# SauersML/genomic_pca

Measured on AMD Instinct MI355X. Metric: SNPs x samples / sec through rSVD at k=20; max|dPC| vs ref, higher is better.
Workload: dtype i8 (exact: int8 dosages x 4 signed 7-bit fixed-point digit planes of the skinny operand, i32 accumulate, f64 recombination; accuracy >= f32)

## Files before the change

genomic_pca_amd/_lib.py:

```python
from __future__ import annotations

import ctypes as C
import os
import subprocess

_PKG = os.path.dirname(os.path.abspath(__file__))
LIB_PATH = os.path.join(_PKG, "libgpca.so")
CSRC = os.path.join(_PKG, "csrc")

GPCA_OK = 0
GPCA_ERR_BAD_ARG = -1
GPCA_ERR_OOM = -2
GPCA_ERR_HIP = -3
GPCA_ERR_RCCL = -4
GPCA_ERR_MISSING_GENOTYPE = -5
GPCA_ERR_NOT_CONVERGED = -6
GPCA_ERR_STATE = -7
GPCA_ERR_NO_DEVICE = -8
GPCA_ERR_INVALID_GENOTYPE = -9
GPCA_UNIQUE_ID_BYTES = 128
PREC_DEFAULT = 0
PREC_I8_EXACT = 1
PREC_F32_MFMA = 2
STORE_AUTO = 0
STORE_2BIT = 1
STORE_INT8 = 2
GRM_STANDARDIZED = 0
GRM_CENTRED = 1
CFG_SIMPLE_KERNELS = 1
CFG_NO_COMPACT = 2
CFG_NO_NARROW = 4
CFG_NO_SPIN_SYNC = 8


class GpcaLibraryError(RuntimeError):
    pass


class GpcaError(RuntimeError):
    def __init__(self, status: int, message: str):
        super().__init__(f"[gpca status {status}] {message}")
        self.status = status
        self.message = message


class gpca_config(C.Structure):
    _fields_ = [("device", C.c_int32), ("precision", C.c_int32), ("storage", C.c_int32), ("digit_planes", C.c_int32),
                ("reserved", C.c_int32 * 4)]


class gpca_qc_config(C.Structure):
    _fields_ = [("min_snp_call_rate", C.c_double), ("min_snp_maf", C.c_double), ("max_snp_hwe_p_value", C.c_double)]


class gpca_kernel_timing(C.Structure):
    _fields_ = [("name", C.c_char * 32), ("launches", C.c_int64), ("total_ms", C.c_double), ("flops", C.c_double),
                ("bytes", C.c_double)]


ALLREDUCE_FN = C.CFUNCTYPE(C.c_int, C.c_void_p, C.POINTER(C.c_double), C.c_int64)
PANEL_FN = C.CFUNCTYPE(C.c_int, C.c_void_p, C.c_int64, C.c_int64, C.c_void_p, C.c_int64)
PANEL_HOST_I8 = 0
PANEL_HOST_BED = 1
PANEL_SYNTH = 2
PANEL_SYNTH16 = 3
PANEL_MAPPED_I8 = 4
PANEL_MAPPED_BED = 5
SOURCE_REGISTER = 1
SOURCE_BENCH_HOLD = 2


class gpca_panel_source(C.Structure):
    _fields_ = [("kind", C.c_int32), ("n_pop", C.c_int32), ("fill", PANEL_FN), ("user", C.c_void_p),
                ("thresh", C.c_void_p), ("seed", C.c_uint64), ("snp_offset", C.c_int64), ("host_ld", C.c_int64), ("flags", C.c_int64)]


class gpca_stream_info(C.Structure):
    _fields_ = [("panel_rows", C.c_int64), ("n_panels", C.c_int32), ("ring_slots", C.c_int32), ("n_cached", C.c_int32),
                ("staging_buffers", C.c_int32), ("zero_staging", C.c_int32), ("copy_threads", C.c_int32), ("fills", C.c_int64),
                ("fill_host_ms", C.c_double), ("fill_wait_ms", C.c_double), ("register_ms", C.c_double), ("reserved", C.c_int64 * 4)]


_H = C.c_void_p
PROTOTYPES = {
    "gpca_version": (C.c_int, []),
    "gpca_status_string": (C.c_char_p, [C.c_int]),
    "gpca_create": (C.c_int, [C.POINTER(gpca_config), C.POINTER(_H)]),
    "gpca_destroy": (C.c_int, [_H]),
    "gpca_last_error": (C.c_char_p, [_H]),
    "gpca_upload_genotypes_i8": (C.c_int, [_H, C.c_void_p, C.c_int64, C.c_int64, C.c_int64]),
    "gpca_upload_bed2bit": (C.c_int, [_H, C.c_void_p, C.c_int64, C.c_int64]),
    "gpca_synth_genotypes": (C.c_int, [_H, C.c_int64, C.c_int64, C.c_uint64, C.c_void_p, C.c_int32, C.c_int64]),
    "gpca_download_genotypes_i8": (C.c_int, [_H, C.c_void_p, C.c_int64]),
    "gpca_load_from_source": (C.c_int, [_H, C.POINTER(gpca_panel_source), C.c_int64, C.c_int64]),
    "gpca_stream_open": (C.c_int, [_H, C.POINTER(gpca_panel_source), C.c_int64, C.c_int64, C.c_int64, C.c_int32]),
    "gpca_stream_set_fused": (C.c_int, [_H, C.c_int32]),
    "gpca_stream_set_cache": (C.c_int, [_H, C.c_int64, C.POINTER(C.c_int32)]),
    "gpca_stream_get_info": (C.c_int, [_H, C.POINTER(gpca_stream_info)]),
    "gpca_get_device_memory": (C.c_int, [_H, C.POINTER(C.c_int64), C.POINTER(C.c_int64)]),
    "gpca_copy_rows": (C.c_int, [_H, _H, C.c_int64, C.c_int64]),
    "gpca_set_sample_mask": (C.c_int, [_H, C.c_void_p]),
    "gpca_set_condensed_basis": (C.c_int, [_H, C.c_void_p, C.c_void_p, C.c_int32, C.c_int64]),
    "gpca_rsvd_condensed": (C.c_int, [_H, C.c_int32, C.c_int32, C.c_int32, C.c_uint64]),
    "gpca_refine": (C.c_int, [_H, C.c_void_p, C.c_int32]),
    "gpca_dims": (C.c_int, [_H, C.POINTER(C.c_int64), C.POINTER(C.c_int64)]),
    "gpca_get_storage": (C.c_int, [_H, C.POINTER(C.c_int32), C.POINTER(C.c_int32)]),
    "gpca_snp_stats": (C.c_int, [_H, C.POINTER(gpca_qc_config), C.c_void_p, C.c_void_p, C.c_void_p]),
    "gpca_get_snp_qc_detail": (C.c_int, [_H, C.c_void_p, C.c_void_p]),
    "gpca_set_standardization": (C.c_int, [_H, C.c_void_p, C.c_void_p, C.c_void_p]),
    "gpca_get_standardization": (C.c_int, [_H, C.c_void_p, C.c_void_p, C.c_void_p]),
    "gpca_hwe_chi_squared_p_value": (C.c_double, [C.c_uint64, C.c_uint64, C.c_uint64]),
    "gpca_host_eigh_desc": (C.c_int, [C.c_void_p, C.c_int32, C.c_void_p, C.c_void_p]),
    "gpca_device_eigh_desc": (C.c_int, [_H, C.c_void_p, C.c_int32, C.c_void_p, C.c_void_p]),
    "gpca_device_orth": (C.c_int, [_H, C.c_void_p, C.c_int32, C.c_int32, C.c_void_p, C.c_void_p, C.POINTER(C.c_int32)]),
    "gpca_device_tail": (C.c_int, [_H, C.c_void_p, C.c_void_p, C.c_int32, C.c_int32, C.c_int32]),
    "gpca_standardize_block": (C.c_int, [_H, C.c_void_p, C.c_int64, C.c_void_p, C.c_int64, C.c_void_p]),
    "gpca_num_pca_snps": (C.c_int64, [_H]),
    "gpca_num_qc_samples": (C.c_int64, [_H]),
    "gpca_get_pca_snp_rows": (C.c_int, [_H, C.c_void_p]),
    "gpca_rsvd": (C.c_int, [_H, C.c_int32, C.c_int32, C.c_int32, C.c_uint64]),
    "gpca_get_scores": (C.c_int, [_H, C.c_void_p]),
    "gpca_get_scores_f64": (C.c_int, [_H, C.c_void_p]),
    "gpca_get_eigenvalues": (C.c_int, [_H, C.c_void_p]),
    "gpca_get_singular_values": (C.c_int, [_H, C.c_void_p]),
    "gpca_get_loadings": (C.c_int, [_H, C.c_void_p]),
    "gpca_transform": (C.c_int, [_H, C.c_void_p]),
    "gpca_project": (C.c_int, [_H, C.c_void_p, C.c_void_p, C.c_void_p, C.c_int32, C.c_void_p, C.c_void_p]),
    "gpca_grm": (C.c_int, [_H, C.c_int32, C.c_int64, C.c_int64, C.c_void_p, C.c_void_p]),
    "gpca_king": (C.c_int, [_H, C.c_int64, C.c_int64, C.c_void_p, C.c_void_p]),
    "gpca_ld_window": (C.c_int, [_H, C.c_int64, C.c_int64, C.c_void_p, C.c_int32, C.c_double, C.c_void_p, C.c_void_p, C.c_void_p]),
    "gpca_pcrelate_isaf": (C.c_int, [_H, C.c_void_p, C.c_int32, C.c_void_p, C.c_int64, C.c_int64, C.c_void_p, C.c_void_p]),
    "gpca_pcrelate": (C.c_int, [_H, C.c_void_p, C.c_int32, C.c_void_p, C.c_double, C.c_int64, C.c_int64, C.c_void_p, C.c_void_p]),
    "gpca_assoc_linear": (C.c_int, [_H, C.c_void_p, C.c_int32, C.c_void_p, C.c_int32, C.c_void_p, C.c_double, C.c_int64, C.c_int64, C.c_void_p,
                                    C.c_void_p, C.c_void_p]),
    "gpca_student_t_log10p": (C.c_double, [C.c_double, C.c_double]),
    "gpca_logistic_null": (C.c_int, [C.c_void_p, C.c_void_p, C.c_int32, C.c_void_p, C.c_int64, C.c_void_p, C.c_void_p, C.POINTER(C.c_int32)]),
    "gpca_assoc_logistic_score": (C.c_int, [_H, C.c_void_p, C.c_int32, C.c_void_p, C.c_int32, C.c_void_p, C.c_double, C.c_int64, C.c_int64,
                                            C.c_void_p, C.c_void_p, C.c_void_p]),
    "gpca_normal_log10p": (C.c_double, [C.c_double]),
    "gpca_assoc_logistic_spa": (C.c_int, [_H, C.c_void_p, C.c_int32, C.c_void_p, C.c_int32, C.c_void_p, C.c_double, C.c_double, C.c_int64,
                                          C.c_int64, C.c_void_p, C.c_void_p, C.c_void_p, C.c_void_p]),
    "gpca_spa_log10p": (C.c_int, [C.c_void_p, C.c_void_p, C.c_int64, C.c_double, C.POINTER(C.c_double), C.c_void_p, C.POINTER(C.c_int32)]),
    "gpca_comm_get_unique_id": (C.c_int, [C.c_void_p]),
    "gpca_comm_init": (C.c_int, [_H, C.c_int32, C.c_int32, C.c_void_p, C.c_int64]),
    "gpca_set_allreduce_hook": (C.c_int, [_H, ALLREDUCE_FN, C.c_void_p, C.c_int32, C.c_int32, C.c_int64]),
    "gpca_comm_count_ranks": (C.c_int, [_H, C.POINTER(C.c_int32)]),
    "gpca_get_timings": (C.c_int, [_H, C.POINTER(gpca_kernel_timing), C.c_int32, C.POINTER(C.c_int32)]),
    "gpca_reset_timings": (C.c_int, [_H]),
    "gpca_enable_timings": (C.c_int, [_H, C.c_int32]),
    "gpca_synchronize": (C.c_int, [_H]),
}


def build(force: bool = False) -> str:
    cmd = ["make", "-C", CSRC, "-s"] + (["-B"] if force else [])
    subprocess.check_call(cmd)
    return LIB_PATH


_lib = None


def load() -> C.CDLL:
    global _lib
    if _lib is not None:
        return _lib
    if not os.path.exists(LIB_PATH):
        raise GpcaLibraryError(
            f"{LIB_PATH} not found: build it with `python -c 'import __graft_entry__ as g; g.build()'` "
            "(hipcc --offload-arch=gfx950).  genomic_pca_amd has no CPU fallback.")
    try:
        lib = C.CDLL(LIB_PATH)
    except OSError as e:
        raise GpcaLibraryError(f"could not load {LIB_PATH}: {e}") from e
    for name, (res, args) in PROTOTYPES.items():
        try:
            fn = getattr(lib, name)
        except AttributeError as e:
            raise GpcaLibraryError(f"{LIB_PATH} does not export {name} (stale build?)") from e
        fn.restype = res
        fn.argtypes = args
    _lib = lib
    return lib
```

genomic_pca_amd/csrc/gemm_i8.hip:

```cpp
#include "gemm_i8_common.h"

namespace gpca {

template <int NSU>
struct GqnG { i32x4 g[4 * NSU]; float r, b; };
template <int NSU>
__device__ __forceinline__ void gqn_load(GqnG<NSU>& b, const int8_t* __restrict__ G, int64_t ldg, int64_t unit, int c, int h,
                                         const float* __restrict__ rv, const float* __restrict__ bv) {
    const __amdgpu_buffer_rsrc_t rg = make_rsrc8(G + unit * 32 * ldg);
    const uint32_t vo = (uint32_t)(c * ldg + 16 * h);
#pragma unroll
    for (int j = 0; j < 4 * NSU; ++j) b.g[j] = __builtin_amdgcn_raw_buffer_load_b128(rg, vo, 32u * j, 2);
    b.r = rv[unit * 32 + c]; b.b = bv[unit * 32 + c];
}
template <int NSU, int PF>
__global__ __launch_bounds__(256, 1) void k_gq_n(const int8_t* __restrict__ G, int64_t ldg, int64_t units,
                                                  const int8_t* __restrict__ Qd, const double* __restrict__ qscale,
                                                  const float* __restrict__ rv, const float* __restrict__ bv,
                                                  const float* __restrict__ sv, float* __restrict__ Tout,
                                                  float* __restrict__ cunit, double* __restrict__ apart, int scale_out, int64_t ldt) {
    const int lane = threadIdx.x & 63;
    const int wv = __builtin_amdgcn_readfirstlane(threadIdx.x >> 6);
    const int c = lane & 31, h = lane >> 5;
    const int64_t wave = (int64_t)blockIdx.x * 4 + wv, waves = (int64_t)gridDim.x * 4;
// ... 383 lines not shown
        else *dst = vv;
    }
    __builtin_amdgcn_fence(__ATOMIC_ACQ_REL, "wavefront");
    __builtin_amdgcn_sched_barrier(0);
}

struct GqdRound { int64_t unit0; int nv; int R; };

template <int NT, int R>
__device__ __forceinline__ void gqd_round(const int8_t* __restrict__ G, int64_t ldg, int64_t nstage,
                                          const int8_t* __restrict__ Qd, GqdSmem* sm, int wv, int lane, int c, int h,
                                          int64_t unit0, int nvalid, bool prologue, bool chain, GqdRound nx, uint32_t& rslot, int round_ix, uint32_t ph,
                                          int64_t rows_total, double qs, const float* __restrict__ rv,
                                          const float* __restrict__ bv, float sj, float* __restrict__ Tout, int scale_out, int64_t ldt,
                                          float* __restrict__ cunit, float& amax) {
    constexpr int S = kGqdSlots;
    static_assert(R >= 1 && R <= 4, "tiles per wave");
    auto phys = [&](uint32_t st_) -> uint32_t { const uint32_t p_ = st_ + ph; return p_ >= (uint32_t)nstage ? p_ - (uint32_t)nstage : p_; };
    const int64_t row0 = unit0 * 32;
    const i32x4 rg = gqd_rsrc(G + row0 * ldg);
    const i32x4 rgn = gqd_rsrc(G + nx.unit0 * 32 * ldg);
    const i32x4 rq = gqd_rsrc(Qd + wv * 1024);
    const uint32_t ld32 = (uint32_t)ldg;
    const uint32_t gvo_e = (uint32_t)(lane >> 3) * ld32 + 16u * (uint32_t)((lane & 7) ^ (lane >> 4));
    const uint32_t gvo_o = (uint32_t)(lane >> 3) * ld32 + 16u * (uint32_t)((lane & 7) ^ (lane >> 4) ^ 4);
    const uint32_t qvo = (uint32_t)(lane * 16);
    uint32_t toff[R];
#pragma unroll
    for (int t = 0; t < R; ++t) toff[t] = (uint32_t)(t < nvalid ? 32 * t : 0) * ld32;
    {
        const uint32_t lds_rb = (uint32_t)(uintptr_t)(__attribute__((address_space(3))) void*)&sm->rb[wv][0][0];
        i32x4 rr_ = gqd_rsrc(rv + row0), rb_ = gqd_rsrc(bv + row0);
        rr_.z = rb_.z = (int)((rows_total - row0) * 4);
        asm volatile("s_waitcnt lgkmcnt(0)" ::: "memory");
#pragma unroll
        for (int j = 0; j < (R + 1) / 2; ++j) {
            gqd_dma_dword(lds_rb + 256u * j, qvo >> 2, rr_, 256u * j);
            gqd_dma_dword(lds_rb + 512u + 256u * j, qvo >> 2, rb_, 256u * j);
        }
    }
    constexpr uint32_t QCH = kDigits * 1024;
    const uint32_t lds_q = (uint32_t)(uintptr_t)(__attribute__((address_space(3))) void*)&sm->q[0][0][0][0] + (uint32_t)wv * 1024u;
    const uint32_t lds_g = (uint32_t)(uintptr_t)(__attribute__((address_space(3))) void*)&sm->g[0][0][0] + (uint32_t)wv * (S * 4096u);
    const char* gl = reinterpret_cast<const char*>(&sm->g[wv][0][0]);
    uint32_t loff[4];
#pragma unroll
    for (int s4 = 0; s4 < 4; ++s4) loff[s4] = (uint32_t)(c * 128 + (((2 * s4 + h) ^ ((c >> 1) & 7)) * 16));

    i32x16 acc[R][kDigits];
#pragma unroll
    for (int t = 0; t < R; ++t)
#pragma unroll
        for (int d = 0; d < kDigits; ++d)
#pragma unroll
            for (int e = 0; e < 16; ++e) acc[t][d][e] = 0;

#define GQD_ISSUE_G(RSRC, SO, SLOT)                                                                       \
    {                                                                                                     \
        const uint32_t so_ = (SO);                                                                        \
        const uint32_t la_ = lds_g + (uint32_t)(SLOT) * 4096u;                                            \
        _Pragma("unroll") for (int i = 0; i < 4; ++i) gqd_dma<NT>(la_ + 1024u * i, (i & 1) ? gvo_o : gvo_e, RSRC, so_ + 8u * i * ld32); \
    }
#define GQD_ISSUE_Q(ST, QS)                                                                               \
    {                                                                                                     \
        _Pragma("unroll") for (int j = 0; j < 4; ++j)                                                     \
            gqd_dma(lds_q + (uint32_t)(((QS) * 4 + j) * kDigits) * 1024u, qvo, rq, (phys((uint32_t)(ST)) * 4u + j) * QCH); \
    }
    int64_t ist = 0;
    int it = 0;
    bool in_next = false;
    uint32_t pst = 0; int pt = 0;
#define GQD_ISSUE_NEXT(SLOT)                                                                              \
    {                                                                                                     \
        if (!in_next) {                                                                                   \
            GQD_ISSUE_G(rg, toff[it] + phys((uint32_t)ist) * 128u, SLOT)                                  \
            if (++it == R) { it = 0; if (++ist == nstage) { if (chain) in_next = true; else ist = 0; } }  \
        } else {                                                                                          \
            const uint32_t tn_ = (uint32_t)(pt < nx.nv ? 32 * pt : 0) * ld32;                             \
            GQD_ISSUE_G(rgn, tn_ + phys(pst) * 128u, SLOT)                                                \
            if (++pt == nx.R) { pt = 0; ++pst; }                                                          \
        }                                                                                                 \
    }
    if (prologue) {
        rslot = 0;
        GQD_ISSUE_NEXT(0) GQD_ISSUE_NEXT(1)
        GQD_ISSUE_Q(0, 0)
#pragma unroll
        for (int sl = S - 4; sl < S; ++sl) GQD_ISSUE_NEXT(sl)
    } else {
        ist = S / R; it = S % R;
    }
    i32x4 gcur, gnxt;

    for (int64_t st = 0; st < nstage; ++st) {
        if constexpr (R == 4) asm volatile("s_waitcnt vmcnt(16)\n\ts_barrier" ::: "memory");
        else if constexpr (R == 3) asm volatile("s_waitcnt vmcnt(12)\n\ts_barrier" ::: "memory");
        else if constexpr (R == 2) asm volatile("s_waitcnt vmcnt(8)\n\ts_barrier" ::: "memory");
        else asm volatile("s_waitcnt vmcnt(4)\n\ts_barrier" ::: "memory");
        GQD_STAGE_STAMP(round_ix, st)
        GQD_ISSUE_Q(st + 1 < nstage ? st + 1 : 0, (int)((st + 1) & 1))
        i32x4 q[4][kDigits];
#pragma unroll
        for (int s4 = 0; s4 < 4; ++s4)
#pragma unroll
            for (int d = 0; d < kDigits; ++d) q[s4][d] = sm->q[st & 1][s4][d][lane];
        if (st == 0) {
            gcur = *reinterpret_cast<const i32x4*>(gl + rslot * 4096u + loff[0]);
            gnxt = *reinterpret_cast<const i32x4*>(gl + rslot * 4096u + loff[1]);
        }
#pragma unroll
        for (int t = 0; t < R; ++t) {
            const char* ub = gl + rslot * 4096u;
            const uint32_t nslot = rslot == S - 1 ? 0u : rslot + 1u;
#pragma unroll
            for (int s4 = 0; s4 < 4; ++s4) {
                i32x4 gfar;
                if (s4 < 2) {
                    gfar = *reinterpret_cast<const i32x4*>(ub + loff[s4 + 2]);
                } else {
                    if (s4 == 2) {
                        if constexpr (R == 4) {
                            if (t == 0) gqd_wait_vm<24>(); else gqd_wait_vm<20>();
                        } else {
                            if (st < gqd_early_stages(R)) gqd_wait_young(gqd_q_young_early(R));
                            else gqd_wait_young(gqd_q_young(R, t));
                        }
                    }
                    gfar = *reinterpret_cast<const i32x4*>(gl + nslot * 4096u + loff[s4 - 2]);
                }
#pragma unroll
                for (int d = 0; d < kDigits; ++d)
                    acc[t][d] = __builtin_amdgcn_mfma_i32_32x32x32_i8(gcur, q[s4][d], acc[t][d], 0, 0, 0);
                if (s4 == 3) {
                    asm volatile("" :: "v"(gcur));
                    GQD_ISSUE_NEXT(rslot)
                }
                gcur = gnxt; gnxt = gfar;
            }
            rslot = nslot;
        }
    }
    if (!chain) asm volatile("s_waitcnt vmcnt(0)\n\ts_barrier" ::: "memory");
    GQD_STAMP(1 + 2 * round_ix)
#undef GQD_ISSUE_NEXT
#undef GQD_ISSUE_G
#undef GQD_ISSUE_Q
    float* tile = sm->tile[wv];
#pragma unroll
    for (int t = 0; t < R; ++t)
        if (t < nvalid) gq_tile_out<7, true>(acc[t], 0.f, 0.f, &sm->rb[wv][0][32 * t], &sm->rb[wv][1][32 * t], qs, sj, scale_out, tile, Tout, ldt, unit0 + t, cunit, amax, lane, nx.unit0 != unit0);
    GQD_STAMP(2 + 2 * round_ix)
}

template <int NT>
__global__ __launch_bounds__(256, 1) void k_gq_d(const int8_t* __restrict__ G, int64_t ldg, int64_t units, int64_t nstage,
                                                  const int8_t* __restrict__ Qd, const double* __restrict__ qscale,
                                                  const float* __restrict__ rv, const float* __restrict__ bv,
                                                  const float* __restrict__ sv, float* __restrict__ Tout,
                                                  float* __restrict__ cpart, double* __restrict__ apart, int scale_out, int64_t ldt,
                                                  int chain_ok, int phase_mul) {
    extern __shared__ __attribute__((aligned(16))) char gqd_smem[];
    GqdSmem* sm = reinterpret_cast<GqdSmem*>(gqd_smem);
    __builtin_assume(nstage >= 2 && (nstage & 1) == 0);
    const int lane = threadIdx.x & 63;
    const int wv = __builtin_amdgcn_readfirstlane(threadIdx.x >> 6);
    const int c = lane & 31, h = lane >> 5;
    const uint32_t ph = (uint32_t)(((int64_t)(blockIdx.x & 7) * (phase_mul & 0xffff) + (int64_t)(blockIdx.x >> 3) * (phase_mul >> 16)) % nstage);
    const int64_t u0 = (units * (int64_t)blockIdx.x) / gridDim.x;
    const int64_t u1 = (units * ((int64_t)blockIdx.x + 1)) / gridDim.x;
    float amax = 0.f;
    const float sj = sv[c];
    const double qs = qscale[c];
    asm volatile("" :: "v"(sj), "v"(qs));
    auto round_at = [&](int64_t u) -> GqdRound {
        const int64_t rem = u1 - u, take = rem < 16 ? rem : 16;
        const int64_t base = take >> 2, extra = take & 3;
        const int nv = (int)(base + (wv < extra ? 1 : 0));
        GqdRound r;
        r.nv = nv; r.R = nv ? nv : 1;
        r.unit0 = nv ? u + wv * base + (wv < extra ? wv : extra) : u;
        return r;
    };
    const bool chain_all = chain_ok && nstage > kGqdSlots;
    uint32_t rslot = 0;
    int round_ix = 0;
    GQD_STAMP(0)
    int64_t u = u0;
    while (u < u1) {
        const int64_t un = u + (u1 - u < 16 ? u1 - u : 16);
        const GqdRound cur = round_at(u);
        const bool chain = chain_all && un < u1;
        const bool prologue = !chain_all || u == u0;
        GqdRound nx = cur;
        if (chain) nx = round_at(un);
#define GPCA_GQD_ROUND(RR) gqd_round<NT, RR>(G, ldg, nstage, Qd, sm, wv, lane, c, h, cur.unit0, cur.nv, prologue, chain, nx, rslot, round_ix, ph, units * 32, qs, rv, bv, sj, Tout, scale_out, ldt, cpart, amax)
        if (cur.R == 4) GPCA_GQD_ROUND(4);
        else if (cur.R == 3) GPCA_GQD_ROUND(3);
        else if (cur.R == 2) GPCA_GQD_ROUND(2);
        else GPCA_GQD_ROUND(1);
#undef GPCA_GQD_ROUND
        u = un;
        ++round_ix;
    }
#if GPCA_STAMP
    if (threadIdx.x == 0 && blockIdx.x == 0) g_gqd_stamp_n = round_ix;
#endif
    float am_lo, am_hi; halves_pair(amax, am_lo, am_hi);
    const float am = fmaxf(am_lo, am_hi);
    if (h == 0) apart[((int64_t)blockIdx.x * 4 + wv) * 32 + c] = (double)am;
}

int launch_gq_d(hipStream_t st, const int8_t* G, int64_t ldg, const GqPlan& plan, int64_t Npad, const int8_t* Qd,
                const double* qscale, const float* r, const float* b, const float* s, float* Tout, float* cpart, double* apart,
                int scale_out, int64_t ldt, const KernelOpts& ko) {
    if (!dma_shape_ok(Npad, 256, plan.units * 32, 32) || ldg < Npad) return (int)hipErrorInvalidValue;
    const dim3 grid((unsigned)(plan.waves / 4)), blk(256);
    const int64_t nstage = Npad / 128;
    int phase = ko.gq_phase;
    if (phase < 0) phase = (nstage >= 16 && nstage <= 400) ? (int)((nstage / 8) << 16) : 0;
    hipLaunchKernelGGL((k_gq_d<1>), grid, blk, sizeof(GqdSmem), st, G, ldg, plan.units, nstage, Qd, qscale, r, b, s, Tout, cpart, apart, scale_out, ldt, ko.gq_chain, phase);
    return 0;
}

template <bool PACKED>
struct GttXG { unsigned g[16]; };

#ifndef GPCA_GTTX_AUX
#define GPCA_GTTX_AUX 2
#endif
template <bool PACKED>
__device__ __forceinline__ void gttx_load_g(GttXG<PACKED>& b, __amdgpu_buffer_rsrc_t rg, uint32_t gvo, uint32_t row_off, uint32_t ldr) {
#pragma unroll
    for (int i = 0; i < 16; ++i) b.g[i] = (unsigned)__builtin_amdgcn_raw_buffer_load_b32(rg, gvo, row_off + (uint32_t)i * ldr, PACKED ? 0 : GPCA_GTTX_AUX);
}
template <bool PACKED, int ABL = 0>
__device__ __forceinline__ void gttx_decode_step(const GttXG<PACKED>& bn, Gtt2Ops& on, unsigned (&x)[4], unsigned (&y)[4], int m, unsigned bsh) {
    const int w = m >> 2, ph = m & 3;
    if (ABL & 1) { on.bt[ph][w] = (int)bn.g[4 * w + ph]; return; }
    if (PACKED) {
        if (ph == 0) x[w] = ((bn.g[4 * w] >> bsh) & 0xffu) | (((bn.g[4 * w + 1] >> bsh) & 0xffu) << 8) |
                            (((bn.g[4 * w + 2] >> bsh) & 0xffu) << 16) | ((bn.g[4 * w + 3] >> bsh) << 24);
        if (ph == 1) { on.bt[0][w] = (int)(x[w] & 0x03030303u); on.bt[1][w] = (int)((x[w] >> 2) & 0x03030303u); }
        if (ph == 2) on.bt[2][w] = (int)((x[w] >> 4) & 0x03030303u);
        if (ph == 3) on.bt[3][w] = (int)((x[w] >> 6) & 0x03030303u);
    } else {
        const int r0 = (int)bn.g[4 * w], r1 = (int)bn.g[4 * w + 1], r2 = (int)bn.g[4 * w + 2], r3 = (int)bn.g[4 * w + 3];
        if (ph == 0) { x[w] = (unsigned)permb(r1, r0, 0x05010400u); y[w] = (unsigned)permb(r1, r0, 0x07030602u); }
        if (ph == 1) { x[w] = x[w]; }
        if (ph == 2) {
            const int y0 = permb(r3, r2, 0x05010400u);
            on.bt[0][w] = permb(y0, (int)x[w], 0x05040100u); on.bt[1][w] = permb(y0, (int)x[w], 0x07060302u);
        }
        if (ph == 3) {
            const int y1 = permb(r3, r2, 0x07030602u);
            on.bt[2][w] = permb(y1, (int)y[w], 0x05040100u); on.bt[3][w] = permb(y1, (int)y[w], 0x07060302u);
        }
    }
}
template <bool PACKED>
__device__ __forceinline__ void gttx_decode(const GttXG<PACKED>& b, Gtt2Ops& o, unsigned bsh) {
    unsigned x[4], y[4];
#pragma unroll
    for (int m = 0; m < 16; ++m) gttx_decode_step<PACKED>(b, o, x, y, m, bsh);
}
struct GttXT { i32x4 t[kDigits]; };
template <bool PACKED, int ND = kDigits, int ABL = 0, bool ZERO = false>
__device__ __forceinline__ void gttx_phase(const GttXT& tc, const Gtt2Ops& oc, i32x16 (&acc)[4][kDigits],
                                           const GttXG<PACKED>& gn, Gtt2Ops& on, GttXT& tn, const i32x4* lds_next, unsigned bsh) {
    unsigned x[4], y[4];
    const i32x16 zero16 = {0, 0, 0, 0, 0, 0, 0, 0, 0, 0, 0, 0, 0, 0, 0, 0};
#pragma unroll
    for (int d = 0; d < kDigits; ++d)
#pragma unroll
        for (int t = 0; t < 4; ++t) {
            if (ABL & 8) { if (d < ND) { if (ZERO) acc[t][d] = zero16; acc[t][d][0] ^= tc.t[d][t] ^ oc.bt[t][d]; } }
            else if (d < ND) acc[t][d] = __builtin_amdgcn_mfma_i32_32x32x32_i8(tc.t[d], oc.bt[t], ZERO ? zero16 : acc[t][d], 0, 0, 0);
            const int m = d * 4 + t;
            if (m < ND) tn.t[m] = lds_next[m * 64];
            gttx_decode_step<PACKED, ABL>(gn, on, x, y, m, bsh);
            __builtin_amdgcn_sched_barrier(0);
        }
}

template <int NT>
__device__ __forceinline__ void gtd_issue_g(const uint8_t* gp, int64_t ldr, int64_t blk, int64_t kblocks, uint32_t lds_slot, uint32_t gvo) {
    const int64_t ub = blk < kblocks ? blk : 0;
    const i32x4 rg = gqd_rsrc(gp + ub * 32 * ldr);
    asm volatile("s_waitcnt lgkmcnt(0)" ::: "memory");
#pragma unroll
    for (int i = 0; i < 4; ++i) gqd_dma<NT>(lds_slot + 1024u * i, gvo, rg, 8u * i * (uint32_t)ldr);
}
__device__ __forceinline__ void gtd_issue_t(const int8_t* tp, int64_t st, int64_t nstage, uint32_t lds_t_slot, uint32_t tvo) {
    constexpr uint32_t TKB = kDigits * 1024;
    const int64_t us = st < nstage ? st : 0;
    const i32x4 rt = gqd_rsrc(tp + us * 4 * TKB);
#pragma unroll
    for (int j = 0; j < 4; ++j) gqd_dma<0>(lds_t_slot + (uint32_t)(j * kDigits) * 1024u, tvo, rt, j * TKB);
}
__device__ __forceinline__ void gtd_read_g(GttXG<false>& b, const char* unit) {
#pragma unroll
    for (int i = 0; i < 16; ++i) b.g[i] = *reinterpret_cast<const unsigned*>(unit + i * 128);
}

#if GPCA_STAMP
__device__ unsigned long long g_gtd_stamp[2 * 4096];
#endif
__device__ __forceinline__ int64_t k2_virtual_wg(int xcd_remap) {
    int64_t vb = blockIdx.x;
    if (xcd_remap) {
        const int64_t q = gridDim.x / 8, r = gridDim.x % 8, x = blockIdx.x % 8;
        vb = x * q + (x < r ? x : r) + blockIdx.x / 8;
    }
    return vb;
}

struct GtdTask { const uint8_t* gp; const int8_t* tp; int64_t kblocks; int64_t n0; int64_t slice; bool live; };

template <int BITS>
__device__ __forceinline__ void gtt_tiles_out(const i32x16 (&acc)[4][kDigits], double* __restrict__ Ypart, int64_t slice, int64_t Npad, int64_t n0,
                                              char* stage = nullptr, int piece_stride = 1024) {
    __builtin_amdgcn_sched_barrier(0);
    unsigned all = ~0u;
    asm volatile("" : "+s"(all));
    const int lane = (int)__builtin_amdgcn_mbcnt_hi(all, __builtin_amdgcn_mbcnt_lo(all, 0u));
    const int c = lane & 31, h = lane >> 5;
#ifndef GPCA_YPART_DIRECT
    if (stage) {
        double* ybase = Ypart + (slice * Npad + n0) * 32;
#pragma unroll
        for (int t = 0; t < 4; ++t) {
#pragma unroll
            for (int half = 0; half < 2; ++half) {
#pragma unroll
                for (int q = 0; q < 2; ++q)
#pragma unroll
                    for (int ip = 0; ip < 2; ++ip) {
                        const int e = 8 * half + 4 * q + 2 * ip;
                        double2 o;
                        o.x = combine_digits<BITS>(acc[t], e); o.y = combine_digits<BITS>(acc[t], e + 1);
                        const int ch = 4 * q + 2 * h + ip;
                        *reinterpret_cast<double2*>(stage + (c >> 3) * piece_stride + (c & 7) * 128 + ((ch ^ (c & 7)) << 4)) = o;
                    }
                __builtin_amdgcn_fence(__ATOMIC_ACQ_REL, "wavefront");
#pragma unroll
                for (int i = 0; i < 4; ++i) {
                    const int line = (lane >> 3) + 8 * i, ch = lane & 7;
                    const double2 v = *reinterpret_cast<const double2*>(stage + i * piece_stride + (lane >> 3) * 128 + ((ch ^ (line & 7)) << 4));
                    typedef double d2v __attribute__((ext_vector_type(2)));
                    const d2v vv = {v.x, v.y};
                    __builtin_nontemporal_store(vv, reinterpret_cast<d2v*>(ybase + (4 * line + t) * 32 + 16 * half + 2 * ch));
                }
                __builtin_amdgcn_fence(__ATOMIC_ACQ_REL, "wavefront");
                __builtin_amdgcn_sched_barrier(0);
            }
        }
        return;
    }
#endif
    double* yp = Ypart + (slice * Npad + n0 + 4 * c) * 32 + 4 * h;
#pragma unroll
    for (int t = 0; t < 4; ++t) {
#pragma unroll
        for (int e = 0; e < 16; e += 2) {
            const int j = acc_row(0, e, 0);
            double2 o;
            o.x = combine_digits<BITS>(acc[t], e); o.y = combine_digits<BITS>(acc[t], e + 1);
            *reinterpret_cast<double2*>(yp + t * 32 + j) = o;
            if (e == 6) __builtin_amdgcn_sched_barrier(0);
        }
        __builtin_amdgcn_sched_barrier(0);
    }
}

struct K2Walk {
    int64_t wch, g, wch_step, g_step, ngroups;
    int ntask;
    __device__ __forceinline__ void init(int64_t vwg, int64_t T, int64_t ngroups_, int tasks_per_wg, int strided) {
        ngroups = ngroups_;
        const int64_t t_first = strided ? vwg : vwg * tasks_per_wg, t_step = strided ? (int64_t)gridDim.x : 1;
        ntask = 0;
        if (t_first < T) { const int64_t left = (T - 1 - t_first) / t_step + 1; ntask = (int)(left < tasks_per_wg ? left : tasks_per_wg); }
        wch = t_first / ngroups; g = t_first - wch * ngroups;
        wch_step = t_step / ngroups; g_step = t_step - wch_step * ngroups;
    }
    __device__ __forceinline__ void advance() { wch += wch_step; g += g_step; if (g >= ngroups) { g -= ngroups; ++wch; } }
};

template <int NT, int ABL = 0>
__global__ __launch_bounds__(256, 1) void k_gtt_d(const uint8_t* __restrict__ Gb, int64_t ldr, int64_t Npad,
                                                   const int8_t* __restrict__ Td, double* __restrict__ Ypart,
                                                   int64_t S, int64_t C, int64_t ngroups, int W, int tasks_per_wg, int strided, int xcd_remap) {
    extern __shared__ __attribute__((aligned(16))) char gqd_smem[];
    GqdSmem* sm = reinterpret_cast<GqdSmem*>(gqd_smem);
    const int lane = threadIdx.x & 63;
    const int wv = __builtin_amdgcn_readfirstlane(threadIdx.x >> 6);
    const int c = lane & 31, h = lane >> 5;
#if GPCA_STAMP
    if (threadIdx.x == 0 && blockIdx.x < 4096) g_gtd_stamp[2 * blockIdx.x] = __builtin_amdgcn_s_memrealtime();
#endif
    constexpr uint32_t TKB = kDigits * 1024;
    K2Walk cw;
    cw.init(k2_virtual_wg(xcd_remap), (int64_t)W * ngroups, ngroups, tasks_per_wg, strided);
    const int ntask = cw.ntask;
    if (ntask == 0) return;
    auto task_of = [&](const K2Walk& w) -> GtdTask {
        const int64_t s0 = w.wch * C, s1 = (s0 + C < S) ? s0 + C : S;
        GtdTask k;
        k.n0 = (w.g * 4 + wv) * 128;
        k.live = k.n0 < Npad;
        if (!k.live) k.n0 = 0;
        k.gp = Gb + (s0 * 128) * ldr + k.n0;
        k.tp = Td + (s0 * 4) * TKB + wv * 1024;
        k.kblocks = (s1 - s0) * 4;
        k.slice = w.wch;
        return k;
    };

    const uint32_t gvo = (uint32_t)(lane >> 3) * (uint32_t)ldr + 16u * (uint32_t)(lane & 7);
    const uint32_t tvo = (uint32_t)(lane * 16);
    const uint32_t lds_t = (uint32_t)(uintptr_t)(__attribute__((address_space(3))) void*)&sm->q[0][0][0][0] + (uint32_t)wv * 1024u;
    const uint32_t lds_g = (uint32_t)(uintptr_t)(__attribute__((address_space(3))) void*)&sm->g[0][0][0] + (uint32_t)wv * (kGqdSlots * 4096u);
    const char* gl = reinterpret_cast<const char*>(&sm->g[wv][0][0]) + (16 * h) * 128 + 4 * c;
    i32x4 (*tds)[4][kDigits][64] = sm->q;

    K2Walk gw = cw, tw = cw;
    int gi = 0; GtdTask gk = task_of(gw); int64_t gblk = 0;
    int ti = 0; GtdTask tk = gk; int64_t tst = 0;
    auto issue_g = [&](uint32_t slot) {
        const i32x4 rg = gqd_rsrc(gk.gp + gblk * 32 * ldr);
        asm volatile("s_waitcnt lgkmcnt(0)" ::: "memory");
#pragma unroll
        for (int i = 0; i < 4; ++i) gqd_dma<NT>(lds_g + slot * 4096u + 1024u * i, gvo, rg, 8u * i * (uint32_t)ldr);
        if (++gblk == gk.kblocks) { gblk = 0; if (gi + 1 < ntask) { ++gi; gw.advance(); gk = task_of(gw); } }
    };
    auto issue_t = [&](uint32_t tslot) {
        const i32x4 rt = gqd_rsrc(tk.tp + tst * 4 * TKB);
#pragma unroll
        for (int j = 0; j < 4; ++j) gqd_dma<0>(lds_t + tslot * 4u * TKB + (uint32_t)(j * kDigits) * 1024u, tvo, rt, j * TKB);
        if (++tst == (tk.kblocks >> 2)) { tst = 0; if (ti + 1 < ntask) { ++ti; tw.advance(); tk = task_of(tw); } }
    };

    i32x16 acc[4][kDigits];
    GttXG<false> GA, GB;
    Gtt2Ops OA, OB;
    GttXT TA, TB;
    issue_g(0); issue_g(1);
    issue_t(0);
    issue_g(2); issue_g(3); issue_g(4); issue_g(5);
    issue_t(1);
    asm volatile("s_waitcnt vmcnt(20)\n\ts_barrier" ::: "memory");
    gtd_read_g(GA, gl);
    gtd_read_g(GB, gl + 4096);
#pragma unroll
    for (int d = 0; d < kDigits; ++d) TA.t[d] = tds[0][0][d][lane];
    gttx_decode<false>(GA, OA, 0u);
    asm volatile("" :: "v"(GB.g[15]));
    issue_g(0);
    uint32_t s1 = 1;
    uint32_t slot = 0;

#define GTD_PHASE(TC, OC, GN, ON, TN, GR, WV, TSLOT, TBLK, ZERO)                                           \
    {                                                                                                    \
        const uint32_t s2_ = s1 == kGqdSlots - 1 ? 0u : s1 + 1u;                                         \
        gqd_wait_vm<WV>();                                                                               \
        gtd_read_g(GR, gl + s2_ * 4096u);                                                                \
        __builtin_amdgcn_sched_barrier(0);                                                               \
        gttx_phase<false, kDigits, ABL, ZERO>(TC, OC, acc, GN, ON, TN, &tds[(TSLOT)][(TBLK)][0][lane], 0u); \
        __builtin_amdgcn_sched_barrier(0);                                                               \
        if (!(ABL & 4)) issue_g(s1);                                                                     \
        s1 = s2_;                                                                                        \
    }
#define GTD_STAGE(ZERO)                                                                                  \
    {                                                                                                    \
        GTD_PHASE(TA, OA, GB, OB, TB, GA, 20, slot, 1, ZERO)                                             \
        GTD_PHASE(TB, OB, GA, OA, TA, GB, 20, slot, 2, false)                                            \
        GTD_PHASE(TA, OA, GB, OB, TB, GA, 20, slot, 3, false)                                            \
        asm volatile("s_waitcnt vmcnt(16)\n\ts_barrier" ::: "memory");    \
        if (!(ABL & 2)) issue_t(slot);                                                                   \
        GTD_PHASE(TB, OB, GA, OA, TA, GB, 24, slot ^ 1u, 0, false)                                       \
        slot ^= 1u;                                                                                      \
    }
    for (int i = 0; i < ntask; ++i) {
        if (i) cw.advance();
        const GtdTask k = task_of(cw);
        const int64_t nstage = k.kblocks >> 2;
        GTD_STAGE(true)
        for (int64_t st = 1; st < nstage; ++st) GTD_STAGE(false)
        if (k.live && !((ABL & 16) && acc[0][0][0] != 0x7fffffff)) gtt_tiles_out<7>(acc, Ypart, k.slice, Npad, k.n0, reinterpret_cast<char*>(&sm->tile[wv][0]));
    }
#undef GTD_STAGE
#undef GTD_PHASE
    asm volatile("s_waitcnt vmcnt(0)" ::: "memory");
#if GPCA_STAMP
    if (threadIdx.x == 0 && blockIdx.x < 4096) g_gtd_stamp[2 * blockIdx.x + 1] = __builtin_amdgcn_s_memrealtime();
#endif
}

struct GtpStage { i32x4 t[4][kDigits][64]; char g[4][4096]; };
struct GtpSmem { GtpStage stg[4]; };

template <int ND>
__device__ __forceinline__ void gtp_segment(const uint8_t* __restrict__ G2, int64_t ld2, int64_t Npad, const int8_t* __restrict__ Td,
                                            double* __restrict__ Ypart, GtpSmem* sm, int wv, int lane, int c, int h,
                                            int64_t g, int64_t s0, int64_t nstage, int64_t slice) {
    const int64_t n0 = (g * 4 + wv) * 128;
    const int64_t m_begin = s0 * 128;

    i32x16 acc[4][kDigits];
#pragma unroll
    for (int t = 0; t < 4; ++t)
#pragma unroll
        for (int d = 0; d < kDigits; ++d)
#pragma unroll
            for (int e = 0; e < 16; ++e) acc[t][d][e] = 0;

    constexpr uint32_t TKB = kDigits * 1024;
    const uint8_t* gp = G2 + m_begin * ld2 + g * 128;
    const int8_t* tp = Td + (m_begin >> 5) * TKB + wv * 1024;
    const uint32_t gvo = (uint32_t)(8 * wv + (lane >> 3)) * (uint32_t)ld2 + 16u * (uint32_t)(lane & 7);
    const uint32_t tvo = (uint32_t)(lane * 16);
    const uint32_t lds0 = (uint32_t)(uintptr_t)(__attribute__((address_space(3))) void*)&sm->stg[0];
    const unsigned bsh = 8u * (unsigned)(c & 3);
    const uint32_t rdo = (uint32_t)((16 * h) * 128 + 32 * wv + (c & ~3));

    auto issue_stage = [&](int64_t st, uint32_t slot) {
        const int64_t us = st < nstage ? st : 0;
        const i32x4 rg = gqd_rsrc(gp + us * 128 * ld2);
        const i32x4 rt = gqd_rsrc(tp + us * 4 * TKB);
        const uint32_t base = lds0 + slot * (uint32_t)sizeof(GtpStage);
#pragma unroll
        for (int bb = 0; bb < 4; ++bb)
            gqd_dma<0>(base + 4u * TKB + (uint32_t)bb * 4096u + (uint32_t)wv * 1024u, gvo, rg, (uint32_t)(32 * bb) * (uint32_t)ld2);
#pragma unroll
        for (int j = 0; j < 4; ++j)
            gqd_dma<0>(base + (uint32_t)(j * kDigits) * 1024u + (uint32_t)wv * 1024u, tvo, rt, j * TKB);
    };
    auto read_g = [&](GttXG<true>& b, uint32_t slot, int bb) {
        const char* unit = &sm->stg[slot].g[bb][0] + rdo;
#pragma unroll
        for (int i = 0; i < 16; ++i) b.g[i] = *reinterpret_cast<const unsigned*>(unit + i * 128);
    };

    GttXG<true> GA, GB;
    Gtt2Ops OA, OB;
    GttXT TA, TB;
    issue_stage(0, 0); issue_stage(1, 1); issue_stage(2, 2);
    asm volatile("s_waitcnt vmcnt(8)\n\ts_barrier" ::: "memory");
    issue_stage(3, 3);
    read_g(GA, 0, 0);
    read_g(GB, 0, 1);
#pragma unroll
    for (int d = 0; d < ND; ++d) TA.t[d] = sm->stg[0].t[0][d][lane];
    gttx_decode<true>(GA, OA, bsh);

#define GTP_PHASE(TC, OC, GN, ON, TN, GR, TSLOT, TBLK, RS, RB)                                             \
    {                                                                                                    \
        read_g(GR, (RS), (RB));                                                                          \
        __builtin_amdgcn_sched_barrier(0);                                                               \
        gttx_phase<true, ND>(TC, OC, acc, GN, ON, TN, &sm->stg[(TSLOT)].t[(TBLK)][0][lane], bsh);            \
        __builtin_amdgcn_sched_barrier(0);                                                               \
    }
    for (int64_t st = 0; st < nstage; ++st) {
        const uint32_t q0 = (uint32_t)(st & 3), qn = (uint32_t)((st + 1) & 3);
        if (st > 0) {
            asm volatile("s_waitcnt vmcnt(8) lgkmcnt(0)\n\ts_barrier" ::: "memory");
            issue_stage(st + 3, (uint32_t)((st + 3) & 3));
        }
        GTP_PHASE(TA, OA, GB, OB, TB, GA, q0, 1, q0, 2)
        GTP_PHASE(TB, OB, GA, OA, TA, GB, q0, 2, q0, 3)
        GTP_PHASE(TA, OA, GB, OB, TB, GA, q0, 3, qn, 0)
        GTP_PHASE(TB, OB, GA, OA, TA, GB, qn, 0, qn, 1)
    }
#undef GTP_PHASE
    asm volatile("s_waitcnt vmcnt(0)\n\ts_barrier" ::: "memory");
    gtt_tiles_out<ND == 3 ? 8 : 7>(acc, Ypart, slice, Npad, n0, &sm->stg[3].g[0][1024 * wv], (int)sizeof(sm->stg[3].g[0]));
}

template <int ND>
__global__ __launch_bounds__(256, 1) void k_gtt_p(const uint8_t* __restrict__ G2, int64_t ld2, int64_t Npad,
                                                   const int8_t* __restrict__ Td, double* __restrict__ Ypart,
                                                   int64_t S, int64_t C, int64_t ngroups, int W, int tasks_per_wg, int strided, int xcd_remap) {
    extern __shared__ __attribute__((aligned(16))) char gqd_smem[];
    GtpSmem* sm = reinterpret_cast<GtpSmem*>(gqd_smem);
    const int lane = threadIdx.x & 63;
    const int wv = __builtin_amdgcn_readfirstlane(threadIdx.x >> 6);
    const int c = lane & 31, h = lane >> 5;
    K2Walk cw;
    cw.init(k2_virtual_wg(xcd_remap), (int64_t)W * ngroups, ngroups, tasks_per_wg, strided);
    for (int i = 0; i < cw.ntask; ++i) {
        if (i) cw.advance();
        const int64_t s0 = cw.wch * C, s1 = (s0 + C < S) ? s0 + C : S;
        gtp_segment<ND>(G2, ld2, Npad, Td, Ypart, sm, wv, lane, c, h, cw.g, s0, s1 - s0, cw.wch);
    }
}

int launch_gtt_p(hipStream_t st, const uint8_t* G2, int64_t ld2, int64_t Mpad, int64_t Npad, const int8_t* Td, double* Ypart,
                 const Gtt8Plan& plan, int nd, const KernelOpts& ko) {
    if (plan.tasks_per_wg < 1 || plan.S * 128 != Mpad || !dma_shape_ok(Npad, kSamplePad2bit, Mpad, kGQRowsPerWave) || ld2 * 4 < Npad) return (int)hipErrorInvalidValue;
    const int remap = ko.gtt_xcd;
    if (nd == 3) hipLaunchKernelGGL(k_gtt_p<3>, dim3((unsigned)plan.grid), dim3(256), sizeof(GtpSmem), st, G2, ld2, Npad, Td, Ypart, plan.S, plan.C, plan.ngroups, plan.W, plan.tasks_per_wg, plan.strided, remap);
    else hipLaunchKernelGGL(k_gtt_p<kDigits>, dim3((unsigned)plan.grid), dim3(256), sizeof(GtpSmem), st, G2, ld2, Npad, Td, Ypart, plan.S, plan.C, plan.ngroups, plan.W, plan.tasks_per_wg, plan.strided, remap);
    return 0;
}

int launch_gtt_d(hipStream_t st, const int8_t* G, int64_t ldg, int64_t Mpad, int64_t Npad, const int8_t* Td, double* Ypart,
                 const Gtt8Plan& plan, const KernelOpts& ko) {
    if (plan.tasks_per_wg < 1 || plan.S * 128 != Mpad || !dma_shape_ok(Npad, 256, Mpad, kGQRowsPerWave) || ldg < Npad) return (int)hipErrorInvalidValue;
    const dim3 grid((unsigned)plan.grid), blk(256);
    const int remap = ko.gtt_xcd;
    hipLaunchKernelGGL((k_gtt_d<1>), grid, blk, sizeof(GqdSmem), st, (const uint8_t*)G, ldg, Npad, Td, Ypart, plan.S, plan.C, plan.ngroups, plan.W, plan.tasks_per_wg, plan.strided, remap);
    return 0;
}

int init_device_kernels_i8() {
    int e = 0;
#define GPCA_OPT_IN(KERNEL, BYTES) \
    if (e == 0) e = (int)hipFuncSetAttribute(reinterpret_cast<const void*>(KERNEL), hipFuncAttributeMaxDynamicSharedMemorySize, (int)(BYTES));
    GPCA_OPT_IN((k_gq_d<1>), sizeof(GqdSmem))
    GPCA_OPT_IN((k_gtt_p<kDigits>), sizeof(GtpSmem)) GPCA_OPT_IN((k_gtt_p<3>), sizeof(GtpSmem))
    GPCA_OPT_IN((k_gtt_d<1>), sizeof(GqdSmem))
#undef GPCA_OPT_IN
    return e;
}

}
```

genomic_pca_amd/csrc/gpca_api.cpp:

```cpp
#include "gpca_internal.h"

using namespace gpca;

RcclApi g_rccl;
thread_local std::string g_last_global_err;

static thread_local uint64_t g_tls_err_gen = 0;
static thread_local std::string g_tls_err;
static std::atomic<uint64_t> g_next_gen{1};
int fail(gpca_handle* h, int code, const std::string& msg) {
    if (h) { h->err = msg; g_tls_err_gen = h->gen; g_tls_err = msg; } else g_last_global_err = msg;
    return code;
}

void fold_timings(gpca_handle* h) {
    for (auto& r : h->recs) {
        float ms = 0.f;
        if (hipEventSynchronize(r.b) == hipSuccess && hipEventElapsedTime(&ms, r.a, r.b) == hipSuccess) {
            size_t i = 0;
            for (; i < h->agg.size(); ++i) if (r.name == h->agg[i].name) break;
            if (i == h->agg.size()) { gpca_kernel_timing t{}; snprintf(t.name, sizeof t.name, "%s", r.name.c_str()); h->agg.push_back(t); }
            h->agg[i].launches++; h->agg[i].total_ms += ms; h->agg[i].flops += r.flops; h->agg[i].bytes += r.bytes;
        }
        h->ev_pool.push_back(r.a); h->ev_pool.push_back(r.b);
    }
    h->recs.clear();
}

extern "C" int gpca_version(void) { return GPCA_VERSION; }

extern "C" const char* gpca_status_string(int s) {
    switch (s) {
        case GPCA_OK: return "ok";
        case GPCA_ERR_BAD_ARG: return "bad argument";
        case GPCA_ERR_OOM: return "out of device memory";
        case GPCA_ERR_HIP: return "HIP runtime error";
        case GPCA_ERR_RCCL: return "RCCL error";
        case GPCA_ERR_MISSING_GENOTYPE: return "missing genotype in a PCA SNP";
        case GPCA_ERR_NOT_CONVERGED: return "sketch lost rank";
        case GPCA_ERR_STATE: return "call out of order";
        case GPCA_ERR_NO_DEVICE: return "no HIP device";
        case GPCA_ERR_INVALID_GENOTYPE: return "genotype outside {0,1,2} in a PCA SNP";
        default: return "unknown status";
    }
}

extern "C" const char* gpca_last_error(gpca_handle* h) {
    if (!h) return g_last_global_err.c_str();
    if (g_tls_err_gen == h->gen) return g_tls_err.c_str();
    return h->err.c_str();
}

extern "C" int gpca_create(const gpca_config* cfg, gpca_handle** out) {
    if (!out) return fail(nullptr, GPCA_ERR_BAD_ARG, "gpca_create: out is NULL");
    *out = nullptr;
    int ndev = 0;
    if (hipGetDeviceCount(&ndev) != hipSuccess || ndev <= 0)
        return fail(nullptr, GPCA_ERR_NO_DEVICE, "gpca_create: no HIP device visible (this engine has no CPU fallback)");
    gpca_handle* h = new gpca_handle();
    h->gen = g_next_gen.fetch_add(1, std::memory_order_relaxed);
    int dev = cfg ? cfg->device : -1;
    if (dev < 0) { if (hipGetDevice(&dev) != hipSuccess) dev = 0; }
    if (dev >= ndev) { delete h; return fail(nullptr, GPCA_ERR_BAD_ARG, "gpca_create: device ordinal out of range"); }
    h->device = dev;
    h->precision = (!cfg || cfg->precision == GPCA_PREC_DEFAULT) ? GPCA_PREC_I8_EXACT : cfg->precision;
    h->storage_cfg = cfg ? cfg->storage : GPCA_STORE_AUTO;
    if (h->storage_cfg != GPCA_STORE_AUTO && h->storage_cfg != GPCA_STORE_INT8 && h->storage_cfg != GPCA_STORE_2BIT) { delete h; return fail(nullptr, GPCA_ERR_BAD_ARG, "gpca_create: unknown storage mode"); }
    if (h->precision != GPCA_PREC_F32_MFMA && h->precision != GPCA_PREC_I8_EXACT) { delete h; return fail(nullptr, GPCA_ERR_BAD_ARG, "gpca_create: unknown precision mode"); }
    h->storage = h->storage_cfg == GPCA_STORE_2BIT ? GPCA_STORE_2BIT : GPCA_STORE_INT8;
    {
        const int dp = cfg ? cfg->digit_planes : 0;
        if (dp != 0 && dp != 3 && dp != 4) { delete h; return fail(nullptr, GPCA_ERR_BAD_ARG, "gpca_create: digit_planes must be 0, 3 or 4"); }
        if (dp == 3 && !(h->precision == GPCA_PREC_I8_EXACT && h->storage_cfg == GPCA_STORE_2BIT)) { delete h; return fail(nullptr, GPCA_ERR_BAD_ARG, "gpca_create: digit_planes = 3 is implemented for GPCA_PREC_I8_EXACT with GPCA_STORE_2BIT"); }
        h->nd_cfg = dp;
        h->nd = dp == 3 ? 3 : ((dp == 0 && h->precision == GPCA_PREC_I8_EXACT && h->storage == GPCA_STORE_2BIT) ? 3 : 4);
    }
    {
        const int32_t flags = cfg ? cfg->reserved[0] : 0, gqw = cfg ? cfg->reserved[1] : 0, gtw = cfg ? cfg->reserved[2] : 0;
        if ((flags & ~GPCA_CFG_ALL) != 0 || gqw < 0 || gtw < 0 || (cfg && cfg->reserved[3] != 0)) { delete h; return fail(nullptr, GPCA_ERR_BAD_ARG, "gpca_create: unknown bits in gpca_config.reserved"); }
        h->simple_kernels = (flags & GPCA_CFG_SIMPLE_KERNELS) != 0;
        h->compact_ok = (flags & GPCA_CFG_NO_COMPACT) == 0;
        h->narrow_ok = (flags & GPCA_CFG_NO_NARROW) == 0;
        h->spin_sync = (flags & GPCA_CFG_NO_SPIN_SYNC) == 0;
        if (gqw) h->gq_waves_target = std::max(4, (int)gqw);
        if (gtw) h->gtt_waves_target = std::max(4, (int)gtw);
    }
    if (hipSetDevice(dev) != hipSuccess || hipStreamCreateWithFlags(&h->st, hipStreamNonBlocking) != hipSuccess) {
        delete h; return fail(nullptr, GPCA_ERR_HIP, "gpca_create: hipSetDevice/hipStreamCreate failed");
    }
    hipDeviceProp_t prop;
    if (hipGetDeviceProperties(&prop, dev) == hipSuccess) {
        if (strncmp(prop.gcnArchName, "gfx950", 6) != 0) {
            std::string m = std::string("gpca_create: device is ") + prop.gcnArchName + ", this library only carries gfx950 code";
            (void)hipStreamDestroy(h->st); delete h; return fail(nullptr, GPCA_ERR_NO_DEVICE, m);
        }
    }
    int e = init_device_kernels_i8();
    if (e == 0) e = init_device_kernels_common();
    if (e == 0) e = init_device_kernels_eig();
    if (e != 0) {
        std::string m = std::string("gpca_create: cannot reserve the LDS the DMA kernels need (hipFuncSetAttribute: ") + hipGetErrorString((hipError_t)e) + ")";
        (void)hipStreamDestroy(h->st); delete h; return fail(nullptr, GPCA_ERR_HIP, m);
    }
    *out = h;
    return GPCA_OK;
}

void drop_child(gpca_handle* h) {
    h->child_valid = false; h->rsvd_on_child = false;
    if (!h->child) return;
    gpca_handle* c = h->child;
    h->child = nullptr;
    c->d_row_ids = nullptr;
    if (h->timing_on || !c->agg.empty() || !c->recs.empty()) {
        (void)hipStreamSynchronize(h->st);
        fold_timings(c);
        for (const gpca_kernel_timing& t : c->agg) {
            size_t i = 0;
            for (; i < h->agg.size(); ++i) if (strcmp(h->agg[i].name, t.name) == 0) break;
            if (i == h->agg.size()) h->agg.push_back(t);
            else { h->agg[i].launches += t.launches; h->agg[i].total_ms += t.total_ms; h->agg[i].flops += t.flops; h->agg[i].bytes += t.bytes; }
        }
    }
    (void)gpca_destroy(c);
}

extern "C" int gpca_destroy(gpca_handle* h) {
    if (!h) return GPCA_OK;
    { LOCK(h);
      (void)hipSetDevice(h->device);
      (void)hipStreamSynchronize(h->st);
      drop_child(h);
      stream_close(h);
      for (auto& r : h->recs) { (void)hipEventDestroy(r.a); (void)hipEventDestroy(r.b); }
      for (auto e : h->ev_pool) (void)hipEventDestroy(e);
      if (h->ev_status) (void)hipEventDestroy(h->ev_status);
      if (h->comm && g_rccl.CommDestroy) g_rccl.CommDestroy(h->comm);
      free_stats(h); free_ws(h); dfree(h->dG); dfree(h->dG2);
      for (auto* ln : h->lanes_free) {
          (void)hipStreamDestroy(ln->st); (void)hipEventDestroy(ln->dep); dfree(ln->d_rows); dfree(ln->d_cols); dfree(ln->d_out); dfree(ln->d_err); delete ln;
      }
      h->lanes_free.clear(); h->lanes_total = 0;
      dfree(h->d_status); if (h->h_status) { (void)hipHostFree(h->h_status); h->h_status = nullptr; }
      if (!h->is_child) (void)hipStreamDestroy(h->st);
    }
    { std::lock_guard<std::mutex> lk(h->pull_mu); }
    delete h;
    return GPCA_OK;
}

extern "C" int gpca_synchronize(gpca_handle* h) {
    if (!h) return GPCA_ERR_BAD_ARG;
    LOCK(h);
    if (h->sm.st_fill) HIPCHK(hipStreamSynchronize(h->sm.st_fill));
    HIPCHK(hipStreamSynchronize(h->st));
    return GPCA_OK;
}

int alloc_stats(gpca_handle* h) {
    const size_t M = (size_t)h->Mpad;
    if (h->d_mu && h->cap_stats_pad >= h->Mpad) return GPCA_OK;
    if (h->d_mu) free_stats(h);
    h->cap_stats_pad = h->Mpad;
    HIPCHK(hipMalloc((void**)&h->d_mu, M * 4)); HIPCHK(hipMalloc((void**)&h->d_sigma, M * 4));
    HIPCHK(hipMalloc((void**)&h->d_r, M * 4)); HIPCHK(hipMalloc((void**)&h->d_b, M * 4));
    HIPCHK(hipMalloc((void**)&h->d_keep, M)); HIPCHK(hipMalloc((void**)&h->d_reason, M));
    HIPCHK(hipMalloc((void**)&h->d_counts, M * 16)); HIPCHK(hipMalloc((void**)&h->d_flags, 16));
    HIPCHK(hipMemsetAsync(h->d_counts, 0, M * 16, h->st)); HIPCHK(hipMemsetAsync(h->d_r, 0, M * 4, h->st)); HIPCHK(hipMemsetAsync(h->d_b, 0, M * 4, h->st));
    HIPCHK(hipMemsetAsync(h->d_mu, 0, M * 4, h->st)); HIPCHK(hipMemsetAsync(h->d_sigma, 0, M * 4, h->st)); HIPCHK(hipMemsetAsync(h->d_keep, 0, M, h->st));
    return GPCA_OK;
}

int refresh_pca_rows(gpca_handle* h) {
    std::vector<uint8_t> keep((size_t)h->M);
    HIPCHK(hipMemcpy(keep.data(), h->d_keep, (size_t)h->M, hipMemcpyDeviceToHost));
    h->pca_rows.clear();
    for (int64_t i = 0; i < h->M; ++i) if (keep[(size_t)i]) h->pca_rows.push_back(i);
    h->n_pca = (int64_t)h->pca_rows.size();
    dfree(h->d_pca_rows);
    if (h->n_pca) {
        HIPCHK(hipMalloc((void**)&h->d_pca_rows, (size_t)h->n_pca * 8));
        HIPCHK(hipMemcpy(h->d_pca_rows, h->pca_rows.data(), (size_t)h->n_pca * 8, hipMemcpyHostToDevice));
    }
    return GPCA_OK;
}

extern "C" int gpca_snp_stats(gpca_handle* h, const gpca_qc_config* qc, float* mu, float* sigma, uint8_t* keep) {
    if (!h) return GPCA_ERR_BAD_ARG;
    LOCK(h);
    if (!have_genotypes(h)) return fail(h, GPCA_ERR_STATE, "gpca_snp_stats: no genotypes resident and no panel stream open");
    HIPCHK(hipSetDevice(h->device));
    CHK(alloc_stats(h));
    QcParams q{0.0, 0.0, 1.0};
    if (qc) { q.min_call_rate = qc->min_snp_call_rate; q.min_maf = qc->min_snp_maf; q.max_hwe_p = qc->max_snp_hwe_p_value; }
    HIPCHK(hipMemsetAsync(h->d_flags, 0, 16, h->st));
    {
        ScopedTimer t(h, "snp_stats", 0.0, (double)h->M * (double)h->N);
        CHK(for_each_panel(h, [&](const PanelView& pv) -> int {
            const int64_t o = pv.row0;
            if (h->storage == GPCA_STORE_2BIT)
                launch_snp_stats_2bit(h->st, pv.g2, pv.rows, h->N, h->ld2, q, h->d_mu + o, h->d_sigma + o, h->d_r + o, h->d_b + o, h->d_keep + o,
                                      h->d_reason + o, h->d_counts + 4 * o, h->d_flags);
            else
                launch_snp_stats(h->st, pv.g8, pv.rows, h->N, h->ld8, q, h->d_mu + o, h->d_sigma + o, h->d_r + o, h->d_b + o, h->d_keep + o,
                                 h->d_reason + o, h->d_counts + 4 * o, h->d_flags);
            HIPCHK(hipGetLastError());
            return GPCA_OK;
        }));
    }
    HIPCHK(hipMemcpyAsync(&h->flags, h->d_flags, 4, hipMemcpyDeviceToHost, h->st));
    HIPCHK(hipStreamSynchronize(h->st));
    if (h->sm.on && h->sm.fl.d_flags) CHK(finish_pack_flags(h, h->sm.fl.d_flags, h->sm.st_fill));
    h->flags |= h->pack_flags;
    CHK(refresh_pca_rows(h));
    h->have_stats = true; h->have_rsvd = false; h->rmax_valid = false; drop_child(h);
    if (mu) HIPCHK(hipMemcpy(mu, h->d_mu, (size_t)h->M * 4, hipMemcpyDeviceToHost));
    if (sigma) HIPCHK(hipMemcpy(sigma, h->d_sigma, (size_t)h->M * 4, hipMemcpyDeviceToHost));
    if (keep) HIPCHK(hipMemcpy(keep, h->d_keep, (size_t)h->M, hipMemcpyDeviceToHost));
    return GPCA_OK;
}

extern "C" int gpca_get_snp_qc_detail(gpca_handle* h, uint32_t* counts, uint8_t* reason) {
    if (!h) return GPCA_ERR_BAD_ARG;
    LOCK(h);
    if (!h->have_stats) return fail(h, GPCA_ERR_STATE, "gpca_get_snp_qc_detail: run gpca_snp_stats first");
    if (counts) HIPCHK(hipMemcpy(counts, h->d_counts, (size_t)h->M * 16, hipMemcpyDeviceToHost));
    if (reason) HIPCHK(hipMemcpy(reason, h->d_reason, (size_t)h->M, hipMemcpyDeviceToHost));
    return GPCA_OK;
}

extern "C" int gpca_get_standardization(gpca_handle* h, float* mu, float* sigma, uint8_t* keep) {
    if (!h) return GPCA_ERR_BAD_ARG;
    LOCK(h);
    if (!h->have_stats) return fail(h, GPCA_ERR_STATE, "gpca_get_standardization: run gpca_snp_stats or gpca_set_standardization first");
    HIPCHK(hipStreamSynchronize(h->st));
    if (mu) HIPCHK(hipMemcpy(mu, h->d_mu, (size_t)h->M * 4, hipMemcpyDeviceToHost));
// ... 327 lines not shown
```

genomic_pca_amd/csrc/gpca_internal.h:

```cpp
#pragma once
#include "../../include/gpca.h"
#include "kernels.h"

#include <dlfcn.h>
#include <hip/hip_runtime.h>

#include <algorithm>
#include <atomic>
#include <chrono>
#include <condition_variable>
#include <deque>
#include <thread>
#include <cmath>
#include <cstdio>
#include <cstdlib>
#include <cstring>
#include <map>
#include <mutex>
#include <string>
#include <vector>

using namespace gpca;

typedef struct ncclComm* ncclComm_t;
typedef struct { char internal[128]; } ncclUniqueId_t;
typedef int (*pfn_ncclGetUniqueId)(ncclUniqueId_t*);
typedef int (*pfn_ncclCommInitRank)(ncclComm_t*, int, ncclUniqueId_t, int);
typedef int (*pfn_ncclAllReduce)(const void*, void*, size_t, int, int, ncclComm_t, hipStream_t);
typedef int (*pfn_ncclCommDestroy)(ncclComm_t);
typedef const char* (*pfn_ncclGetErrorString)(int);
struct RcclApi {
    void* lib = nullptr;
    pfn_ncclGetUniqueId GetUniqueId = nullptr;
    pfn_ncclCommInitRank CommInitRank = nullptr;
    pfn_ncclAllReduce AllReduce = nullptr;
    pfn_ncclCommDestroy CommDestroy = nullptr;
    pfn_ncclGetErrorString GetErrorString = nullptr;
    bool load() {
        if (lib) return true;
        const char* names[] = {"librccl.so.1", "librccl.so", "/opt/rocm/lib/librccl.so.1"};
        for (const char* n : names) { lib = dlopen(n, RTLD_NOW | RTLD_LOCAL); if (lib) break; }
        if (!lib) return false;
        GetUniqueId = (pfn_ncclGetUniqueId)dlsym(lib, "ncclGetUniqueId");
        CommInitRank = (pfn_ncclCommInitRank)dlsym(lib, "ncclCommInitRank");
        AllReduce = (pfn_ncclAllReduce)dlsym(lib, "ncclAllReduce");
        CommDestroy = (pfn_ncclCommDestroy)dlsym(lib, "ncclCommDestroy");
        GetErrorString = (pfn_ncclGetErrorString)dlsym(lib, "ncclGetErrorString");
        return GetUniqueId && CommInitRank && AllReduce && CommDestroy;
    }
};
extern RcclApi g_rccl;
enum { kNcclFloat64 = 8, kNcclSum = 0 };

struct TimingRec { std::string name; hipEvent_t a, b; double flops, bytes; };

struct PanelView { const int8_t* g8; const uint8_t* g2; int64_t row0, rows, rows_pad; int index; };

struct Filler {
    gpca_panel_source src{};
    int64_t chunk_rows = 0;
    int64_t stage_ld = 0;
    uint32_t* d_thresh = nullptr;
    int8_t* d_scratch8 = nullptr;
    uint8_t* d_raw = nullptr;
    unsigned* d_flags = nullptr;
    bool open = false;
    bool host = false, mapped = false, registered = false;
    const uint8_t* map_base = nullptr; int64_t map_ld = 0; size_t reg_bytes = 0;
    int device = 0, copy_threads = 1;
    int n_stage = 0;
    std::vector<void*> h_stage;
    std::vector<hipEvent_t> ev_stage;
    enum { kFree = 0, kReady = 1, kInFlight = 2 };
    std::vector<int> st_state, st_rc;
    std::vector<int64_t> st_row0;
    std::deque<std::pair<int64_t, int64_t>> jobs;
    uint64_t posted = 0, produced = 0, consumed = 0;
    bool busy = false, quit = false;
    std::mutex m; std::condition_variable cv; std::thread worker;
    int64_t fills = 0; double fill_host_ms = 0.0, fill_wait_ms = 0.0, register_ms = 0.0;
    std::map<void*, int64_t> held;
};

struct StreamState {
    bool on = false;
    Filler fl;
    int64_t panel_rows = 0;
    int n_panels = 0, ring = 0;
    std::vector<void*> slot;
    std::vector<hipEvent_t> ev_filled, ev_free;
    std::vector<char> free_pending;
    hipStream_t st_fill = nullptr;
    int64_t seq = 0;
    int fused = 1;
    std::vector<void*> cache;
    std::vector<hipEvent_t> ev_cache;
    std::vector<char> cache_filled;
};

struct gpca_handle {
    std::recursive_mutex mu;
    KernelOpts ko;
    StreamState sm;
    int device = 0;
    int precision = GPCA_PREC_I8_EXACT;
    int storage = GPCA_STORE_INT8;
    int storage_cfg = GPCA_STORE_AUTO;
    int nd_cfg = 0;
    int auto_pin = 0;
    hipStream_t st = nullptr;
    std::string err;

    int64_t M = 0, N = 0, ldg = 0, Mpad = 0;
    int64_t ld8 = 0;
    int64_t cap_rows_pad = 0;
    int64_t cap_stats_pad = 0;
    int8_t* dG = nullptr;
    uint8_t* dG2 = nullptr;
    int64_t ld2 = 0;
    uint32_t pack_flags = 0;

    bool have_stats = false;
    float *d_mu = nullptr, *d_sigma = nullptr, *d_r = nullptr, *d_b = nullptr;
    uint8_t *d_keep = nullptr, *d_reason = nullptr;
    uint32_t *d_counts = nullptr, *d_flags = nullptr;
    int64_t n_pca = 0;
    std::vector<int64_t> pca_rows;
    int64_t* d_pca_rows = nullptr;
    uint32_t flags = 0;

    int k = 0, l = 0, L = 0;
    bool have_rsvd = false;
    float *dQ = nullptr, *dT = nullptr, *dTb = nullptr, *dYpart = nullptr, *d_cpart = nullptr, *d_s32 = nullptr;
    double* h_pin = nullptr;
    int spin_sync = 1;
    int* d_cholflag = nullptr;
    double *d_scratch64 = nullptr, *dY = nullptr, *d_c = nullptr, *d_part64 = nullptr, *dW = nullptr, *dZ = nullptr, *d_s64 = nullptr;
    double* d_tr64 = nullptr; size_t cap_tr64 = 0;
    double* d_scores64 = nullptr; float* d_scores32 = nullptr; float* d_load32 = nullptr; int* d_sign = nullptr;
    double* d_eigres = nullptr;
    double* d_cand_val = nullptr; int64_t* d_cand_idx = nullptr;
    size_t cap_Q = 0, cap_T = 0, cap_Tb = 0, cap_Ypart = 0, cap_cpart = 0, cap_Y = 0, cap_part64 = 0, cap_scores = 0, cap_load = 0;
    std::vector<double> eig, sv;
    GttPlan plan{};
    GqPlan gqplan{};
    Gtt8Plan plan8{};
    int8_t *dQd = nullptr, *dTd = nullptr;
    bool c_fold_pending = false;
    double* d_apart = nullptr; size_t cap_apart = 0; bool apart_valid = false; int64_t apart_parts = 0;
    const double* apart_src[4] = {nullptr, nullptr, nullptr, nullptr};
    float* d_rmax = nullptr; bool rmax_valid = false;
    double* d_amax_run = nullptr;
    double* d_yint = nullptr; size_t cap_yint = 0;
    uint8_t* d_smask = nullptr;
    int64_t n_smask = 0;
    float* d_cw = nullptr; int32_t* d_cfeat0 = nullptr; int c_cmax = 0; int64_t c_R = 0; int c_B = 0;
    int64_t *d_cblk_row0 = nullptr, *d_cblk_row1 = nullptr; int32_t *d_cblk_feat0 = nullptr, *d_cblk_c = nullptr;
    double* dP = nullptr; size_t cap_P = 0;
    float* d_lqr = nullptr; size_t cap_lqr = 0;
    float *d_ones = nullptr, *d_zeros = nullptr; size_t cap_ones = 0, cap_zeros = 0;
    bool loadings_valid = true;
    double* d_status = nullptr;
    double* h_status = nullptr;
    hipEvent_t ev_status = nullptr;
    std::string status_own;
    struct PullLane {
        hipStream_t st = nullptr;
        hipEvent_t dep = nullptr;
        int64_t *d_rows = nullptr, *d_cols = nullptr; float* d_out = nullptr; unsigned long long* d_err = nullptr;
        size_t cap_rows = 0, cap_cols = 0, cap_out = 0;
    };
    std::mutex pull_mu;
    std::condition_variable pull_cv;
    std::vector<PullLane*> lanes_free;
    int lanes_total = 0;
    std::atomic<int> pulls_in_flight{0};
    double *dYpart64 = nullptr, *d_qscale = nullptr, *d_qinv = nullptr, *d_tscale = nullptr, *d_tinv = nullptr;
    size_t cap_Qd = 0, cap_Td = 0, cap_Ypart64 = 0;
    int nd = 4;
    uint64_t gen = 0;
    int simple_kernels = 0;
    int narrow_ok = 1;
    int gq_waves_target = 1024, gtt_waves_target = 2048;

    gpca_handle* child = nullptr;
    bool child_valid = false, rsvd_on_child = false;
    bool is_child = false;
    const int64_t* d_row_ids = nullptr;
    int compact_ok = 1;

    int world = 1, rank = 0;
    int64_t snp_offset = 0;
    ncclComm_t comm = nullptr;
    gpca_allreduce_fn hook = nullptr;
    void* hook_user = nullptr;
    std::vector<double> hook_buf;

    bool timing_on = false;
    int timing_every = 1;
    int64_t timing_calls = 0;
    bool timing_skip = false;
    int open_timers = 0;
    std::vector<TimingRec> recs;
    std::vector<hipEvent_t> ev_pool;
    std::vector<gpca_kernel_timing> agg;
};
constexpr size_t kMaxTimingRecs = 32768;
#define LOCK(h) std::lock_guard<std::recursive_mutex> lock_guard_(h->mu); (void)hipSetDevice(h->device); drain_pulls(h)
#define LOCK_SHARED(h) std::lock_guard<std::recursive_mutex> lock_guard_(h->mu); (void)hipSetDevice(h->device)
constexpr int kMaxPullLanes = 16;
inline void drain_pulls(gpca_handle* h) {
    if (h->pulls_in_flight.load(std::memory_order_acquire) == 0) return;
    std::unique_lock<std::mutex> lk(h->pull_mu);
    h->pull_cv.wait(lk, [&] { return h->pulls_in_flight.load(std::memory_order_acquire) == 0; });
}

extern thread_local std::string g_last_global_err;
int fail(gpca_handle* h, int code, const std::string& msg);
#define HIPCHK(call)                                                                                   \
    do {                                                                                               \
        hipError_t e_ = (call);                                                                        \
        if (e_ != hipSuccess) {                                                                        \
            char buf_[512];                                                                            \
            snprintf(buf_, sizeof buf_, "%s failed: %s (%s:%d)", #call, hipGetErrorString(e_), __FILE__, __LINE__); \
            return fail(h, e_ == hipErrorOutOfMemory ? GPCA_ERR_OOM : GPCA_ERR_HIP, buf_);             \
        }                                                                                              \
    } while (0)
#define CHK(x) do { int rc_ = (x); if (rc_ != GPCA_OK) return rc_; } while (0)

template <typename T>
inline int ensure(gpca_handle* h, T*& p, size_t& cap, size_t need_elems) {
    if (cap >= need_elems && p) return GPCA_OK;
    if (p) { HIPCHK(hipFree(p)); p = nullptr; cap = 0; }
    HIPCHK(hipMalloc((void**)&p, need_elems * sizeof(T)));
    cap = need_elems;
    return GPCA_OK;
}
template <typename T>
inline void dfree(T*& p) { if (p) { (void)hipFree(p); p = nullptr; } }
template <typename T>
inline hipError_t dalloc(T*& p, size_t elems) { return hipMalloc((void**)&p, std::max<size_t>(elems, 1) * sizeof(T)); }
inline int preflight_device_memory(gpca_handle* h, const char* name, const char* what, double need_bytes) {
    size_t fr = 0, tot = 0;
    HIPCHK(hipMemGetInfo(&fr, &tot));
    if (need_bytes > (double)fr) {
        char buf[256];
        snprintf(buf, sizeof buf, "%s: %s %.3g GB of device memory, %.3g GB are free: ask for fewer rows", name, what, need_bytes * 1e-9, (double)fr * 1e-9);
        return fail(h, GPCA_ERR_OOM, buf);
    }
    return GPCA_OK;
}

inline hipError_t malloc_genotypes(const gpca_handle*, void** p, size_t bytes) { return hipMalloc(p, bytes); }

inline int64_t round_up(int64_t x, int64_t m) { return (x + m - 1) / m * m; }
static_assert(gpca::kMaxSketchCols == 128, "kernels.h");
constexpr int kMaxSketch = gpca::kMaxSketchCols;

void fold_timings(gpca_handle* h);
struct ScopedTimer {
    gpca_handle* h; bool on; size_t idx = 0; hipStream_t st;
    ScopedTimer(gpca_handle* h_, const char* name, double flops, double bytes, hipStream_t st_ = nullptr, bool enable = true)
        : h(h_), on(h_->timing_on && !h_->timing_skip && enable), st(st_ ? st_ : h_->st) {
        if (!on) return;
        if (h->recs.size() >= kMaxTimingRecs && h->open_timers == 0) fold_timings(h);
        TimingRec r; r.name = name; r.flops = flops; r.bytes = bytes; r.a = r.b = nullptr;
        for (hipEvent_t* e : {&r.a, &r.b}) {
            if (!h->ev_pool.empty()) { *e = h->ev_pool.back(); h->ev_pool.pop_back(); }
            else if (hipEventCreateWithFlags(e, hipEventDisableSystemFence) != hipSuccess) { on = false; return; }
        }
        (void)hipEventRecord(r.a, st);
        h->recs.push_back(r); idx = h->recs.size() - 1; h->open_timers++;
    }
    ~ScopedTimer() { if (on) { (void)hipEventRecord(h->recs[idx].b, st); h->open_timers--; } }
};


inline bool have_genotypes(const gpca_handle* h) { return h->dG || h->dG2 || h->sm.on; }
inline bool multi_rank(const gpca_handle* h) { return h->world > 1 || h->hook != nullptr; }
constexpr size_t kPlaneBytesPerBlock = (size_t)gpca::kDigits * 1024;
void free_stats(gpca_handle* h);
int alloc_stats(gpca_handle* h);
int refresh_pca_rows(gpca_handle* h);
void free_eigensnp(gpca_handle* h);
void free_ws(gpca_handle* h);
void stream_close(gpca_handle* h);
int finish_pack_flags(gpca_handle* h, unsigned* d_flags, hipStream_t st);
int filler_fill(gpca_handle* h, Filler& f, int64_t row0, int64_t rows, void* dst, hipStream_t st);
void filler_post(Filler& f, int64_t row0, int64_t rows);
void filler_cancel(Filler& f);
int allreduce_f64(gpca_handle* h, double* dbuf, int64_t count);
hipError_t stream_wait(gpca_handle* h);
int agree_status(gpca_handle* h, int local_rc, const char* where);
int agree_status_begin(gpca_handle* h, int local_rc);
int agree_status_end(gpca_handle* h, int local_rc, const char* where);
void status_histogram(double* slots16, int local_rc);
int status_verdict(gpca_handle* h, const double* v, int local_rc, const std::string& own, const char* where);
void drop_child(gpca_handle* h);
struct XBuf {
    double* p = nullptr; bool pinned = false;
    hipError_t alloc(size_t n) {
        if (hipMalloc((void**)&p, std::max<size_t>(n, 1) * 8) == hipSuccess) return hipSuccess;
        (void)hipGetLastError();
        p = nullptr; pinned = true;
        return hipHostMalloc((void**)&p, std::max<size_t>(n, 1) * 8, hipHostMallocDefault);
    }
    ~XBuf() { if (p) { if (pinned) (void)hipHostFree(p); else (void)hipFree(p); } }
};
#define LOCAL(x) do { if (lrc == GPCA_OK) lrc = (x); if (lrc != GPCA_OK && !mr) return lrc; } while (0)
int exchange_with_status(gpca_handle* h, const char* fn, double* buf, size_t n, int& lrc, double* tail, size_t ntail = 16);
inline void set_row_bit(std::vector<uint32_t>& mask, int64_t i) { mask[(size_t)(i >> 5)] |= 1u << (i & 31); }
int64_t kept_row_mask(const std::vector<uint8_t>& keep, int64_t Mpad, std::vector<uint32_t>& mask);
int check_genotype_flag(gpca_handle* h, const char* fn, const char* whose, const unsigned* d_bad);
struct PanelRows { const void* G; int64_t ldr; };
inline PanelRows panel_rows(const gpca_handle* h, const PanelView& pv) {
    return h->storage == GPCA_STORE_2BIT ? PanelRows{pv.g2, h->ld2} : PanelRows{pv.g8, h->ld8};
}
inline PanelView resident_view(const gpca_handle* h) { return PanelView{h->dG, h->dG2, 0, h->M, h->Mpad, 0}; }
int asc_check_call(gpca_handle* h, const std::string& f, bool cols_ok, const std::string& cols_rule, const double* Y, const double* C, int Pc,
                   const char* out_err, int64_t row0, int64_t row1, double max_vif, const char* late_err = nullptr);
void asc_sample_set(const uint8_t* include, int64_t N, std::vector<int64_t>& S, std::vector<unsigned>* incw);
int asc_standardise(const double* C, int Pc, const std::vector<int64_t>& S, double* X, std::string& msg);
int asc_cholesky(const double* X, int P, int64_t ns, const double* w, bool (*accept)(double d, double diag), std::vector<double>& A,
                 std::string& msg);
void asc_solve_lt(const std::vector<double>& A, int P, int64_t ns, const double* X, const double* w, double* out);
int asc_check_genotypes(gpca_handle* h, const std::string& f, const unsigned long long* d_bad, hipStream_t st);
struct AscOutput { double* host; const double* dev; int64_t elems; };
int asc_copy_outputs(gpca_handle* h, hipStream_t st, std::initializer_list<AscOutput> outs);

template <class F>
inline int for_each_panel_walk(gpca_handle* h, F&& fn) {
    StreamState& sm = h->sm;
    const bool packed = h->storage == GPCA_STORE_2BIT;
    const int64_t row_bytes = packed ? h->ld2 : h->ld8;
    for (int p = 0; p < sm.n_panels; ++p) {
// ... 49 lines not shown
```

genomic_pca_amd/csrc/gpca_rsvd.cpp:

```cpp
#include "gpca_internal.h"

using namespace gpca;

static void tred2(int n, double* V, double* d, double* e) {
    for (int j = 0; j < n; ++j) d[j] = V[(n - 1) * n + j];
    for (int i = n - 1; i > 0; --i) {
        double scale = 0.0, h = 0.0;
        for (int k = 0; k < i; ++k) scale += std::fabs(d[k]);
        if (scale == 0.0) {
            e[i] = d[i - 1];
            for (int j = 0; j < i; ++j) { d[j] = V[(i - 1) * n + j]; V[i * n + j] = 0.0; V[j * n + i] = 0.0; }
        } else {
            for (int k = 0; k < i; ++k) { d[k] /= scale; h += d[k] * d[k]; }
            double f = d[i - 1];
            double g = std::sqrt(h);
            if (f > 0) g = -g;
            e[i] = scale * g; h -= f * g; d[i - 1] = f - g;
            for (int j = 0; j < i; ++j) e[j] = 0.0;
            for (int j = 0; j < i; ++j) {
                f = d[j]; V[j * n + i] = f; g = e[j] + V[j * n + j] * f;
                for (int k = j + 1; k <= i - 1; ++k) { g += V[k * n + j] * d[k]; e[k] += V[k * n + j] * f; }
                e[j] = g;
            }
            f = 0.0;
            for (int j = 0; j < i; ++j) { e[j] /= h; f += e[j] * d[j]; }
            const double hh = f / (h + h);
            for (int j = 0; j < i; ++j) e[j] -= hh * d[j];
            for (int j = 0; j < i; ++j) {
                f = d[j]; g = e[j];
                for (int k = j; k <= i - 1; ++k) V[k * n + j] -= (f * e[k] + g * d[k]);
                d[j] = V[(i - 1) * n + j]; V[i * n + j] = 0.0;
            }
        }
        d[i] = h;
    }
    for (int i = 0; i < n - 1; ++i) {
        V[(n - 1) * n + i] = V[i * n + i]; V[i * n + i] = 1.0;
        const double h = d[i + 1];
        if (h != 0.0) {
            for (int k = 0; k <= i; ++k) d[k] = V[k * n + (i + 1)] / h;
            for (int j = 0; j <= i; ++j) {
                double g = 0.0;
                for (int k = 0; k <= i; ++k) g += V[k * n + (i + 1)] * V[k * n + j];
                for (int k = 0; k <= i; ++k) V[k * n + j] -= g * d[k];
            }
        }
        for (int k = 0; k <= i; ++k) V[k * n + (i + 1)] = 0.0;
    }
    for (int j = 0; j < n; ++j) { d[j] = V[(n - 1) * n + j]; V[(n - 1) * n + j] = 0.0; }
    V[(n - 1) * n + (n - 1)] = 1.0; e[0] = 0.0;
}
static void tql2(int n, double* V, double* d, double* e) {
    for (int i = 1; i < n; ++i) e[i - 1] = e[i];
    e[n - 1] = 0.0;
    double f = 0.0, tst1 = 0.0;
    const double eps = 2.220446049250313e-16;
    for (int l = 0; l < n; ++l) {
        tst1 = std::max(tst1, std::fabs(d[l]) + std::fabs(e[l]));
        int m = l;
        while (m < n - 1 && std::fabs(e[m]) > eps * tst1) ++m;
        if (m > l) {
            int iter = 0;
            do {
                ++iter;
                double g = d[l];
                double p = (d[l + 1] - g) / (2.0 * e[l]);
                double r = std::hypot(p, 1.0);
                if (p < 0) r = -r;
                d[l] = e[l] / (p + r); d[l + 1] = e[l] * (p + r);
                const double dl1 = d[l + 1];
                double h = g - d[l];
                for (int i = l + 2; i < n; ++i) d[i] -= h;
                f += h;
                p = d[m];
                double c = 1.0, c2 = c, c3 = c, s = 0.0, s2 = 0.0;
                const double el1 = e[l + 1];
                for (int i = m - 1; i >= l; --i) {
                    c3 = c2; c2 = c; s2 = s;
                    g = c * e[i]; h = c * p;
                    r = std::hypot(p, e[i]);
                    e[i + 1] = s * r; s = e[i] / r; c = p / r;
                    p = c * d[i] - s * g;
                    d[i + 1] = h + s * (c * g + s * d[i]);
                    for (int k = 0; k < n; ++k) {
                        h = V[k * n + i + 1];
                        V[k * n + i + 1] = s * V[k * n + i] + c * h;
                        V[k * n + i] = c * V[k * n + i] - s * h;
                    }
                }
                p = -s * s2 * c3 * el1 * e[l] / dl1;
                e[l] = s * p; d[l] = c * p;
            } while (std::fabs(e[l]) > eps * tst1 && iter < 200);
        }
        d[l] += f; e[l] = 0.0;
    }
}
static void host_eigh_desc(std::vector<double>& A, std::vector<double>& V, std::vector<double>& w, int n) {
    std::vector<double> e((size_t)n);
    V = A;
    if (n == 1) { w[0] = A[0]; V[0] = 1.0; return; }
    tred2(n, V.data(), w.data(), e.data());
    tql2(n, V.data(), w.data(), e.data());
    for (int i = 0; i < n - 1; ++i) {
        int m = i;
        for (int j = i + 1; j < n; ++j) if (w[j] > w[m]) m = j;
        if (m != i) { std::swap(w[i], w[m]); for (int k = 0; k < n; ++k) std::swap(V[k * n + i], V[k * n + m]); }
    }
}
extern "C" int gpca_host_eigh_desc(const double* a_sym, int32_t n, double* w, double* v) {
    if (!a_sym || !w || !v || n < 1 || n > kMaxSketch) return GPCA_ERR_BAD_ARG;
    std::vector<double> A(a_sym, a_sym + (size_t)n * n), V((size_t)n * n), W((size_t)n);
    host_eigh_desc(A, V, W, n);
    std::copy(W.begin(), W.end(), w); std::copy(V.begin(), V.end(), v);
    return GPCA_OK;
}

extern "C" int gpca_device_eigh_desc(gpca_handle* h, const double* a_sym, int32_t n, double* w, double* v) {
    if (!h || !a_sym || !w || !v || n < 1 || n > kMaxSketch) return GPCA_ERR_BAD_ARG;
    LOCK(h);
    const int L = n <= 32 ? 32 : (n <= 64 ? 64 : kMaxSketch);
    double *dA = nullptr, *dZz = nullptr, *dR = nullptr, *dV = nullptr;
    std::vector<double> A((size_t)L * L, 0.0), R((size_t)kEigResCount);
    for (int a = 0; a < n; ++a) for (int c = 0; c < n; ++c) A[(size_t)a * L + c] = a_sym[(size_t)a * n + c];
    int rc = GPCA_OK;
    auto run = [&]() -> int {
        HIPCHK(hipMalloc((void**)&dA, A.size() * 8)); HIPCHK(hipMalloc((void**)&dZz, 2 * (size_t)L * n * 8));
        HIPCHK(hipMalloc((void**)&dR, R.size() * 8)); HIPCHK(hipMalloc((void**)&dV, (size_t)n * n * 8));
        HIPCHK(hipMemcpyAsync(dA, A.data(), A.size() * 8, hipMemcpyHostToDevice, h->st));
        launch_small_eigh(h->st, dA, 0, n, L, n, 1, 1.0, nullptr, dZz, dR, dV);
        HIPCHK(hipGetLastError());
        HIPCHK(hipMemcpyAsync(R.data(), dR, R.size() * 8, hipMemcpyDeviceToHost, h->st));
        HIPCHK(hipMemcpyAsync(v, dV, (size_t)n * n * 8, hipMemcpyDeviceToHost, h->st));
        HIPCHK(hipStreamSynchronize(h->st));
        return GPCA_OK;
    };
    rc = run();
    dfree(dA); dfree(dZz); dfree(dR); dfree(dV);
    if (rc != GPCA_OK) return rc;
    std::copy(R.begin() + kEigResW, R.begin() + kEigResW + n, w);
    if (R[kEigResFlag + 1] != 0.0) return fail(h, GPCA_ERR_NOT_CONVERGED, "gpca_device_eigh_desc: the QL sweeps hit their cap");
    return GPCA_OK;
}

static int stage_sum_c(gpca_handle* h, int64_t parts) {
    launch_sum_partials_f32(h->st, h->d_cpart, parts, h->L, h->d_c, h->d_scratch64);
    HIPCHK(hipGetLastError());
    return GPCA_OK;
}


static inline bool narrow_shape(const gpca_handle* h) {
    return h->narrow_ok && h->precision == GPCA_PREC_I8_EXACT && h->storage == GPCA_STORE_INT8 && h->N <= kNarrowSamples;
}
static inline bool k2_batched(const gpca_handle* h) {
    return !narrow_shape(h) && !h->simple_kernels;
}
static inline Gtt8Plan k2_plan(const gpca_handle* h, int64_t rows_pad) {
    return narrow_shape(h) ? gtt8_plan_narrow(rows_pad, h->N, std::min(h->gtt_waves_target, 1024)) :
           k2_batched(h) ? gtt8_plan_batched(rows_pad, h->ldg, h->gtt_waves_target) : gtt8_plan(rows_pad, h->ldg, h->gtt_waves_target);
}

static inline GqPlan k1_plan(const gpca_handle* h, int64_t rows_pad) { return gq_plan(rows_pad, h->gq_waves_target); }

static int k2_panel(gpca_handle* h, const PanelView& pv, const int8_t* Td_half, const Gtt8Plan& plan) {
    const int8_t* Td = Td_half + (size_t)(pv.row0 >> 5) * kPlaneBytesPerBlock;
    const bool packed = h->storage == GPCA_STORE_2BIT;
    if (narrow_shape(h)) launch_gtt_n(h->st, pv.g8, h->ld8, pv.rows_pad, h->ldg, Td, h->dYpart64, plan);
    else if (h->simple_kernels) {
        if (packed) launch_gtt_2bit(h->st, pv.g2, h->ld2, pv.rows_pad, h->ldg, Td, h->dYpart64, plan, h->nd);
        else launch_gtt_i8(h->st, pv.g8, h->ld8, pv.rows_pad, h->ldg, Td, h->dYpart64, plan, h->ko);
    } else if (packed) {
        const int e = launch_gtt_p(h->st, pv.g2, h->ld2, pv.rows_pad, h->ldg, Td, h->dYpart64, plan, h->nd, h->ko);
        if (e != 0) return fail(h, GPCA_ERR_HIP, "k_gtt_p launch failed (hip error " + std::to_string(e) + ")");
    } else {
        const int e = launch_gtt_d(h->st, pv.g8, h->ld8, pv.rows_pad, h->ldg, Td, h->dYpart64, plan, h->ko);
        if (e != 0) return fail(h, GPCA_ERR_HIP, "k_gtt_d launch failed (hip error " + std::to_string(e) + ")");
    }
    HIPCHK(hipGetLastError());
    return GPCA_OK;
}

static int stage_AtT_local(gpca_handle* h, bool planes_ready = false) {
    const double elems = (double)h->M * (double)h->N;
    if (h->precision == GPCA_PREC_I8_EXACT) {
        const int L = h->L, halves = L / 32;
        const size_t td_half = (size_t)h->Mpad * 32 * kDigits;
        for (int hf = 0; hf < halves && !planes_ready; ++hf) {
            const float* Th = h->dT + 32 * hf;
            double* tsc = h->d_tscale + 32 * hf; double* tin = h->d_tinv + 32 * hf;
            if (h->c_fold_pending) launch_quantize_f32_cfold(h->st, Th, h->Mpad, h->Mpad, tin, h->dTd + hf * td_half, 0, h->nd, L, h->d_scratch64 + (size_t)hf * kPostK1Scratch,
                                                             post_k1_slices(h->Mpad / 32), h->d_c + 32 * hf);
            else if (h->apart_valid) launch_quantize_f32_premax(h->st, Th, h->Mpad, h->Mpad, h->apart_src[hf], h->apart_parts, tsc, tin, h->dTd + hf * td_half, 0, h->nd, L);
            else launch_quantize_f32(h->st, Th, h->Mpad, h->Mpad, h->d_part64, tsc, tin, h->dTd + hf * td_half, 0, h->nd, L);
            HIPCHK(hipGetLastError());
        }
        h->apart_valid = false; h->c_fold_pending = false;
        const bool streamed = h->sm.on;
        const size_t yint_half = (size_t)h->N * 32;
        {
            const double by = h->storage == GPCA_STORE_2BIT ? elems / 4 : elems;
            ScopedTimer sweep(h, "gemm_GtT", 2.0 * elems * h->l, by * halves, nullptr, streamed);
            CHK(for_each_panel(h, [&](const PanelView& pv) -> int {
                const Gtt8Plan plan = streamed ? k2_plan(h, pv.rows_pad) : h->plan8;
                for (int hf = 0; hf < halves; ++hf) {
                    {
                        ScopedTimer t(h, "gemm_GtT", 2.0 * elems * h->l / halves, by, nullptr, !streamed);
                        CHK(k2_panel(h, pv, h->dTd + hf * td_half, plan));
                    }
                    if (streamed) launch_accum_y_i8(h->st, h->dYpart64, plan.W, h->ldg, h->N, h->d_yint + hf * yint_half, pv.index == 0);
                    else launch_reduce_y_i8(h->st, h->dYpart64, plan.W, h->ldg, h->N, h->d_c + 32 * hf, h->d_tscale + 32 * hf, h->dY + 32 * hf, L);
                    HIPCHK(hipGetLastError());
                }
                return GPCA_OK;
            }));
        }
        if (streamed)
            for (int hf = 0; hf < halves; ++hf) {
                launch_finish_y_i8(h->st, h->d_yint + hf * yint_half, h->N, h->d_c + 32 * hf, h->d_tscale + 32 * hf, h->dY + 32 * hf, L);
                HIPCHK(hipGetLastError());
            }
        return GPCA_OK;
    }
    {
        const bool packed = h->storage == GPCA_STORE_2BIT;
        ScopedTimer t(h, "gemm_GtT", 2.0 * elems * h->l, packed ? elems / 4 : elems);
        launch_gtt_f32(h->st, packed ? (const void*)h->dG2 : (const void*)h->dG, packed, packed ? h->ld2 : h->ld8, h->Mpad, h->ldg, h->dTb, h->L, h->dYpart, h->plan);
    }
    HIPCHK(hipGetLastError());
    launch_reduce_y(h->st, h->dYpart, h->plan.W, h->ldg, h->N, h->L, h->d_c, h->dY);
    HIPCHK(hipGetLastError());
    return GPCA_OK;
}

static int stage_AQ(gpca_handle* h, int scale_out) {
    const double elems = (double)h->M * (double)h->N;
    if (h->precision == GPCA_PREC_I8_EXACT) {
        const int L = h->L, halves = L / 32;
        const bool packed = h->storage == GPCA_STORE_2BIT, streamed = h->sm.on;
        const size_t qhalf = (size_t)h->ldg * 32 * kDigits;
        const size_t chalf = (size_t)h->Mpad;
        const size_t ahalf = (size_t)h->gqplan.waves * 32;
        if (streamed && scale_out) HIPCHK(hipMemsetAsync(h->d_amax_run, 0, kMaxSketch * 8, h->st));
        {
            const double by = packed ? elems / 4 : elems;
            ScopedTimer sweep(h, "gemm_GQ", 2.0 * elems * h->l, by * halves, nullptr, streamed);
            CHK(for_each_panel(h, [&](const PanelView& pv) -> int {
                const GqPlan plan = streamed ? k1_plan(h, pv.rows_pad) : h->gqplan;
                for (int hf = 0; hf < halves; ++hf) {
                    const int8_t* Qd = h->dQd + hf * qhalf;
                    const double* qsc = h->d_qscale + 32 * hf;
                    const float* s32 = h->d_s32 + 32 * hf;
                    const float* rr = h->d_r + pv.row0; const float* bb = h->d_b + pv.row0;
                    float* Th = h->dT + (size_t)pv.row0 * L + 32 * hf;
                    float* cp = h->d_cpart + hf * chalf + (size_t)pv.row0;
                    double* ap = h->d_apart + hf * ahalf;
                    ScopedTimer t(h, "gemm_GQ", 2.0 * elems * h->l / halves, by, nullptr, !streamed);
                    if (packed) launch_gq_2bit(h->st, pv.g2, h->ld2, plan, h->ldg, Qd, qsc, rr, bb, s32, Th, cp, ap, scale_out, h->nd, L);
                    else if (narrow_shape(h)) {
                        const int e = launch_gq_n(h->st, pv.g8, h->ld8, plan, h->N, Qd, qsc, rr, bb, s32, Th, cp, ap, scale_out, L);
                        if (e != 0) return fail(h, GPCA_ERR_HIP, "k_gq_n launch failed (hip error " + std::to_string(e) + ")");
                    }
                    else if (!h->simple_kernels) {
                        const int e = launch_gq_d(h->st, pv.g8, h->ld8, plan, h->ldg, Qd, qsc, rr, bb, s32, Th, cp, ap, scale_out, L, h->ko);
                        if (e != 0) return fail(h, GPCA_ERR_HIP, "k_gq_d launch failed (hip error " + std::to_string(e) + ")");
                    }
                    else launch_gq_i8(h->st, pv.g8, h->ld8, plan, h->N, Qd, qsc, rr, bb, s32, Th, cp, scale_out, L, h->ko);
                    HIPCHK(hipGetLastError());
                    if (streamed && scale_out && (packed || !h->simple_kernels || narrow_shape(h))) {
                        launch_absmax_fold(h->st, ap, plan.waves, h->d_amax_run + 32 * hf);
                        HIPCHK(hipGetLastError());
                    }
                }
                return GPCA_OK;
            }));
        }
        h->apart_valid = scale_out != 0 && (packed || !h->simple_kernels || narrow_shape(h));
        h->c_fold_pending = scale_out != 0 && !streamed && h->apart_valid;
        if (scale_out)
            for (int hf = 0; hf < halves; ++hf) {
                if (h->c_fold_pending)
                    launch_post_k1(h->st, h->d_cpart + hf * chalf, h->Mpad / 32, h->d_scratch64 + (size_t)hf * kPostK1Scratch, h->d_apart + hf * ahalf, h->gqplan.waves,
                                   h->d_tscale + 32 * hf, h->d_tinv + 32 * hf, h->nd);
                else launch_sum_partials_f32(h->st, h->d_cpart + hf * chalf, h->Mpad / 32, 32, h->d_c + 32 * hf, h->d_scratch64);
                HIPCHK(hipGetLastError());
            }
        for (int hf = 0; hf < kMaxSketch / 32; ++hf) h->apart_src[hf] = streamed ? h->d_amax_run + 32 * hf : h->d_apart + hf * ahalf;
        h->apart_parts = streamed ? 1 : h->gqplan.waves;
        return GPCA_OK;
    }
    {
        const bool packed = h->storage == GPCA_STORE_2BIT;
        ScopedTimer t(h, "gemm_GQ", 2.0 * elems * h->l, packed ? elems / 4 : elems);
        launch_gq_f32(h->st, packed ? (const void*)h->dG2 : (const void*)h->dG, packed, packed ? h->ld2 : h->ld8, h->gqplan, h->ldg, h->dQ, h->L, h->d_r, h->d_b,
                      h->d_s32, h->dT, scale_out ? h->dTb : nullptr, h->d_cpart);
    }
    HIPCHK(hipGetLastError());
    if (scale_out) CHK(stage_sum_c(h, h->gqplan.waves));
    return GPCA_OK;
}

static int stage_power_fused(gpca_handle* h) {
    const double elems = (double)h->M * (double)h->N;
    const int L = h->L, halves = L / 32;
    const bool packed = h->storage == GPCA_STORE_2BIT;
    const size_t qhalf = (size_t)h->ldg * 32 * kDigits, chalf = (size_t)h->Mpad, ahalf = (size_t)h->gqplan.waves * 32;
    const size_t td_half = (size_t)h->Mpad * 32 * kDigits, yint_half = (size_t)h->N * 32;
    {
        const double by = packed ? elems / 4 : elems;
        ScopedTimer sweep(h, "gemm_fused", 4.0 * elems * h->l, by * halves);
        CHK(for_each_panel(h, [&](const PanelView& pv) -> int {
            const GqPlan plan1 = k1_plan(h, pv.rows_pad);
            const Gtt8Plan plan2 = k2_plan(h, pv.rows_pad);
            const float* rr = h->d_r + pv.row0; const float* bb = h->d_b + pv.row0;
            for (int hf = 0; hf < halves; ++hf) {
                const int8_t* Qd = h->dQd + hf * qhalf;
                float* Th = h->dT + (size_t)pv.row0 * L + 32 * hf;
                float* cp = h->d_cpart + hf * chalf + (size_t)pv.row0;
                double* ap = h->d_apart + hf * ahalf;
                if (packed) launch_gq_2bit(h->st, pv.g2, h->ld2, plan1, h->ldg, Qd, h->d_qscale + 32 * hf, rr, bb, h->d_s32 + 32 * hf, Th, cp, ap, 1, h->nd, L);
                else if (narrow_shape(h)) {
                    const int e = launch_gq_n(h->st, pv.g8, h->ld8, plan1, h->N, Qd, h->d_qscale + 32 * hf, rr, bb, h->d_s32 + 32 * hf, Th, cp, ap, 1, L);
                    if (e != 0) return fail(h, GPCA_ERR_HIP, "k_gq_n launch failed (hip error " + std::to_string(e) + ")");
                }
                else {
                    const int e = launch_gq_d(h->st, pv.g8, h->ld8, plan1, h->ldg, Qd, h->d_qscale + 32 * hf, rr, bb, h->d_s32 + 32 * hf, Th, cp, ap, 1, L, h->ko);
                    if (e != 0) return fail(h, GPCA_ERR_HIP, "k_gq_d launch failed (hip error " + std::to_string(e) + ")");
                }
                HIPCHK(hipGetLastError());
                launch_quantize_f32_premax(h->st, Th, pv.rows_pad, pv.rows_pad, ap, plan1.waves, h->d_tscale + 32 * hf, h->d_tinv + 32 * hf,
                                           h->dTd + hf * td_half + (size_t)(pv.row0 >> 5) * kPlaneBytesPerBlock, 0, h->nd, L);
                HIPCHK(hipGetLastError());
            }
            for (int hf = 0; hf < halves; ++hf) {
                CHK(k2_panel(h, pv, h->dTd + hf * td_half, plan2));
                launch_accum_y_scaled(h->st, h->dYpart64, plan2.W, h->ldg, h->N, h->d_tscale + 32 * hf, h->d_yint + hf * yint_half, pv.index == 0);
                HIPCHK(hipGetLastError());
            }
            return GPCA_OK;
        }));
    }
    for (int hf = 0; hf < halves; ++hf) {
        launch_sum_partials_f32(h->st, h->d_cpart + hf * chalf, h->Mpad / 32, 32, h->d_c + 32 * hf, h->d_scratch64);
        HIPCHK(hipGetLastError());
        launch_finish_y_sum(h->st, h->d_yint + hf * yint_half, h->N, h->d_c + 32 * hf, h->dY + 32 * hf, L);
        HIPCHK(hipGetLastError());
    }
    h->apart_valid = false;
    return GPCA_OK;
}

static int stage_orth(gpca_handle* h, int rounds = 2) {
    const int L = h->L, l = h->l;
    if (h->d_smask) {
        launch_mask_rows(h->st, h->dY, h->N, L, h->d_smask);
        HIPCHK(hipGetLastError());
    }
    for (int round = 0; round < rounds; ++round) {
        const int64_t parts = gram_num_parts(h->N);
        launch_gram_f64(h->st, h->dY, h->N, L, h->d_part64);
        HIPCHK(hipGetLastError());
        if (L == 32 && parts <= 64) launch_chol_inv_fold(h->st, h->d_part64, (int)parts, l, L, h->dZ, h->d_cholflag);
        else {
            launch_sum_partials_f64(h->st, h->d_part64, parts, (int64_t)L * L, h->dW, h->d_scratch64);
            HIPCHK(hipGetLastError());
            const int e = launch_chol_inv(h->st, h->dW, l, L, h->dZ, h->d_cholflag);
            if (e != 0) return fail(h, GPCA_ERR_HIP, "CholeskyQR: the factorisation was not launched (hip error " + std::to_string(e) + ")");
        }
        HIPCHK(hipGetLastError());
        if (round + 1 < rounds) launch_apply_right_inplace(h->st, h->dY, h->N, L, h->dZ, nullptr, h->ldg);
        else launch_apply_right_tail(h->st, h->dY, h->N, L, h->dZ, h->dQ, h->ldg, h->d_part64, h->d_part64 + tail_num_parts(h->ldg) * L);
        HIPCHK(hipGetLastError());
    }
    const bool i8 = h->precision == GPCA_PREC_I8_EXACT;
    const int64_t tparts = tail_num_parts(h->ldg);
    const double* csum_part = h->d_part64;
    const double* amax_part = h->d_part64 + tparts * L;
    if (i8 && tparts <= kFinishQFoldMax) {
        for (int hf = 0; hf < L / 32; ++hf) {
            launch_quantize_f64_finishq(h->st, h->dY + 32 * hf, h->N, h->ldg, h->dQd + (size_t)hf * h->ldg * 32 * kDigits, h->storage == GPCA_STORE_2BIT ? 1 : 0, h->nd, L,
                                        csum_part + 32 * hf, amax_part + 32 * hf, tparts, L, h->d_s64 + 32 * hf, h->d_s32 + 32 * hf, h->d_qscale + 32 * hf, h->d_qinv + 32 * hf);
            HIPCHK(hipGetLastError());
        }
        return GPCA_OK;
    }
    launch_finish_q(h->st, csum_part, amax_part, tparts, L, h->d_s64, h->d_s32, i8 ? h->d_qscale : nullptr, i8 ? h->d_qinv : nullptr, h->nd);
    HIPCHK(hipGetLastError());
    if (i8) {
        for (int hf = 0; hf < L / 32; ++hf) {
            launch_quantize_f64_prescaled(h->st, h->dY + 32 * hf, h->N, h->ldg, h->d_qinv + 32 * hf, h->dQd + (size_t)hf * h->ldg * 32 * kDigits,
                                          h->storage == GPCA_STORE_2BIT ? 1 : 0, h->nd, L);
            HIPCHK(hipGetLastError());
        }
    }
    return GPCA_OK;
}

static int ensure_workspace(gpca_handle* h) {
    const int L = h->L;
    const int64_t Npad = h->ldg, M = h->M, N = h->N;
    const int64_t gemm_rows = h->sm.on ? h->sm.panel_rows : h->Mpad;
    h->plan = gtt_plan(h->Mpad, Npad, L, h->gtt_waves_target);
    h->gqplan = k1_plan(h, gemm_rows);
    CHK(ensure(h, h->dQ, h->cap_Q, (size_t)Npad * L));
    CHK(ensure(h, h->dT, h->cap_T, (size_t)h->Mpad * L));
    if (h->precision == GPCA_PREC_F32_MFMA) CHK(ensure(h, h->dTb, h->cap_Tb, (size_t)h->Mpad * L));
    if (h->Mpad > M) HIPCHK(hipMemsetAsync(h->dT + (size_t)M * L, 0, (size_t)(h->Mpad - M) * L * 4, h->st));
    if (h->precision == GPCA_PREC_F32_MFMA) CHK(ensure(h, h->dYpart, h->cap_Ypart, (size_t)h->plan.W * (size_t)Npad * L));
    const int64_t cparts = cpart_capacity(h->gqplan.waves, h->Mpad, L);
    CHK(ensure(h, h->d_cpart, h->cap_cpart, (size_t)cparts));
    CHK(ensure(h, h->dY, h->cap_Y, (size_t)N * L + 16));
    const int64_t p64 = part64_capacity(M, h->Mpad, N, Npad, L);
    CHK(ensure(h, h->d_part64, h->cap_part64, (size_t)p64));
    if (!h->d_c) {
        constexpr size_t LL = (size_t)kMaxSketch * kMaxSketch;
        HIPCHK(hipMalloc((void**)&h->d_c, kMaxSketch * 8)); HIPCHK(hipMalloc((void**)&h->d_s64, kMaxSketch * 8));
        HIPCHK(hipMalloc((void**)&h->d_s32, kMaxSketch * 4)); HIPCHK(hipMalloc((void**)&h->dW, (LL + 16) * 8));
        HIPCHK(hipMalloc((void**)&h->dZ, 2 * LL * 8));
        HIPCHK(hipHostMalloc((void**)&h->h_pin, (3 * LL + 16) * 8, hipHostMallocDefault)); HIPCHK(hipMalloc((void**)&h->d_sign, kMaxSketch * 4));
        HIPCHK(hipMalloc((void**)&h->d_scratch64, (size_t)sum_scratch_capacity(kMaxSketch) * 8));
        HIPCHK(hipMalloc((void**)&h->d_eigres, kEigResCount * 8));
        HIPCHK(hipMalloc((void**)&h->d_cand_val, (size_t)scores_cand_capacity() * 8)); HIPCHK(hipMalloc((void**)&h->d_cand_idx, (size_t)scores_cand_capacity() * 8));
        HIPCHK(hipMalloc((void**)&h->d_cholflag, 4));
    }
    if (h->precision == GPCA_PREC_I8_EXACT) {
        h->plan8 = k2_plan(h, gemm_rows);
        CHK(ensure(h, h->dQd, h->cap_Qd, (size_t)Npad * 32 * kDigits * (size_t)(L / 32)));
        CHK(ensure(h, h->dTd, h->cap_Td, (size_t)h->Mpad * 32 * kDigits * (size_t)(L / 32)));
        int64_t yslices = h->plan8.W;
        if (h->sm.on && h->M % h->sm.panel_rows) yslices = std::max<int64_t>(yslices, k2_plan(h, round_up(h->M % h->sm.panel_rows, kGQRowsPerWave)).W);
        CHK(ensure(h, h->dYpart64, h->cap_Ypart64, (size_t)yslices * (size_t)Npad * 32));
        CHK(ensure(h, h->d_apart, h->cap_apart, (size_t)h->gqplan.waves * 32 * (size_t)(L / 32)));
        if (h->sm.on) CHK(ensure(h, h->d_yint, h->cap_yint, (size_t)N * 32 * (size_t)(L / 32)));
        if (!h->d_qscale) {
            HIPCHK(hipMalloc((void**)&h->d_qscale, kMaxSketch * 8)); HIPCHK(hipMalloc((void**)&h->d_qinv, kMaxSketch * 8));
            HIPCHK(hipMalloc((void**)&h->d_tscale, kMaxSketch * 8)); HIPCHK(hipMalloc((void**)&h->d_tinv, kMaxSketch * 8));
            HIPCHK(hipMalloc((void**)&h->d_amax_run, kMaxSketch * 8));
            HIPCHK(hipMalloc((void**)&h->d_rmax, 4));
        }
    }
    size_t cap2 = h->cap_scores;
    CHK(ensure(h, h->d_scores64, h->cap_scores, (size_t)N * h->k));
    CHK(ensure(h, h->d_scores32, cap2, (size_t)N * h->k));
    CHK(ensure(h, h->d_load32, h->cap_load, (size_t)std::max<int64_t>(h->n_pca, 1) * h->k));
    return GPCA_OK;
}

static int rsvd_preflight(gpca_handle* h, int32_t k, int32_t oversample, int32_t power_iters) {
    if (!have_genotypes(h)) return fail(h, GPCA_ERR_STATE, "gpca_rsvd: no genotypes resident and no panel stream open");
    if (!h->have_stats) return fail(h, GPCA_ERR_STATE, "gpca_rsvd: run gpca_snp_stats or gpca_set_standardization first");
    if (k <= 0) return fail(h, GPCA_ERR_BAD_ARG, "Number of components (-k) must be > 0.");
    if (oversample < 0 || power_iters < 0) return fail(h, GPCA_ERR_BAD_ARG, "gpca_rsvd: negative oversample/power_iters");
    if (h->N < 2) return fail(h, GPCA_ERR_BAD_ARG, "PCA requires at least 2 samples.");
    if (!multi_rank(h) && h->n_pca == 0) return fail(h, GPCA_ERR_BAD_ARG, "PCA requires at least 1 variant (feature), found 0.");
    const int l = k + oversample;
    if (l > kMaxSketch) return fail(h, GPCA_ERR_BAD_ARG, "gpca_rsvd: k + oversample must be <= 128");
    if (l > 64 && h->precision != GPCA_PREC_I8_EXACT)
        return fail(h, GPCA_ERR_BAD_ARG, "gpca_rsvd: sketches wider than 64 columns (k + oversample > 64) run on GPCA_PREC_I8_EXACT; GPCA_PREC_F32_MFMA holds up to 64");
    if (l > h->N || (!multi_rank(h) && l > h->n_pca)) return fail(h, GPCA_ERR_BAD_ARG, "gpca_rsvd: k + oversample exceeds min(samples, PCA SNPs)");
    if (h->flags & 1u) return fail(h, GPCA_ERR_MISSING_GENOTYPE,
        "Unexpected missing genotype (-127i8) in a PCA SNP. This should have been filtered by QC.");
    if (h->flags & 2u) return fail(h, GPCA_ERR_INVALID_GENOTYPE, "a PCA SNP holds a dosage outside {0,1,2}");
    if (h->sm.on && h->precision != GPCA_PREC_I8_EXACT) return fail(h, GPCA_ERR_STATE, "gpca_rsvd: streamed panels need GPCA_PREC_I8_EXACT");
    if (h->precision == GPCA_PREC_I8_EXACT && h->N > ((int64_t)1 << 22))
        return fail(h, GPCA_ERR_BAD_ARG, "gpca_rsvd: the exact-integer path holds up to 4 194 304 samples per matrix (i32 accumulators); use GPCA_PREC_F32_MFMA beyond");
    HIPCHK(hipSetDevice(h->device));
    h->k = k; h->l = l; h->L = l <= 32 ? 32 : (l <= 64 ? 64 : kMaxSketch);
    h->have_rsvd = false;
    CHK(ensure_workspace(h));
    HIPCHK(hipMemsetAsync(h->d_cholflag, 0, 4, h->st));
    return GPCA_OK;
}

static int enqueue_small_eigh(gpca_handle* h, const double* src, int nslices, int zmode, double denom) {
    launch_small_eigh(h->st, src, nslices, h->l, h->L, h->k, zmode, denom, h->d_cholflag, h->dZ, h->d_eigres, nullptr);
    HIPCHK(hipGetLastError());
    return GPCA_OK;
}
static int enqueue_scores_loadings(gpca_handle* h, const float* Xload, bool loadings) {
    const int L = h->L, k = h->k;
    const size_t zk = (size_t)L * k;
    if (L <= 64) {
        launch_scores(h->st, h->dY, h->N, L, h->dZ, k, h->d_scores64, h->d_cand_val, h->d_cand_idx);
        HIPCHK(hipGetLastError());
        launch_scores_sign(h->st, h->d_scores64, h->d_scores32, h->N, k, h->d_cand_val, h->d_cand_idx, scores_num_parts(h->N), h->d_sign);
        HIPCHK(hipGetLastError());
        if (loadings) launch_rightmul_gather_f32(h->st, Xload, h->d_pca_rows, h->n_pca, L, h->dZ + zk, k, h->d_load32, h->d_sign);
    } else {
        launch_rightmul_f64(h->st, h->dY, h->N, L, h->dZ, k, h->d_scores64, (float*)nullptr);
        HIPCHK(hipGetLastError());
        launch_col_sign(h->st, h->d_scores64, h->N, k, h->d_sign);
        launch_scale_cols(h->st, h->d_scores64, h->d_scores32, h->N, k, h->d_sign);
        HIPCHK(hipGetLastError());
        if (loadings) {
            launch_scale_cols(h->st, h->dZ + zk, (float*)nullptr, L, k, h->d_sign);
            launch_rightmul_gather_f32(h->st, Xload, h->d_pca_rows, h->n_pca, L, h->dZ + zk, k, h->d_load32);
        }
    }
    HIPCHK(hipGetLastError());
    return GPCA_OK;
}
static int finish_small_eigh(gpca_handle* h, bool take) {
    double* res = h->h_pin;
    HIPCHK(hipMemcpyAsync(res, h->d_eigres, sizeof(double) * kEigResCount, hipMemcpyDeviceToHost, h->st));
    HIPCHK(stream_wait(h));
    if (!take) return GPCA_OK;
    static_assert(kEigNotConverged == GPCA_ERR_NOT_CONVERGED, "eig_result.h restates the status code");
    const EigVerdict verdict = eig_result_verdict(res, h->l);
    if (verdict.status != 0) return fail(h, verdict.status, verdict.msg);
    h->sv.assign(res + kEigResSv, res + kEigResSv + h->l);
    h->eig.assign(res + kEigResEig, res + kEigResEig + h->k);
    return GPCA_OK;
}

static int call_tail(gpca_handle* h, int zmode, double denom, const float* Xload, int lrc) {
    const bool mr = multi_rank(h);
    const int L = h->L;
    const double* gsrc = h->dW; int gslices = 0;
    auto gram = [&]() -> int {
        const int64_t rows = zmode == 0 ? h->M : h->N;
        const int64_t parts = gram_num_parts(rows);
        if (zmode == 0) launch_gram_f32(h->st, h->dT, rows, L, h->d_part64);
        else launch_gram_f64(h->st, h->dY, rows, L, h->d_part64);
        HIPCHK(hipGetLastError());
        if (mr) launch_sum_partials_f64(h->st, h->d_part64, parts, (int64_t)L * L, h->dW, h->d_scratch64);
        else launch_sum_partials_f64_stage1(h->st, h->d_part64, parts, (int64_t)L * L, h->d_scratch64, &gsrc, &gslices);
        HIPCHK(hipGetLastError());
        return GPCA_OK;
    };
    LOCAL(gram());
    if (mr) {
        h->status_own = h->err;
        status_histogram(h->h_status, lrc);
        if (hipMemcpyAsync(h->dW + (size_t)L * L, h->h_status, 16 * sizeof(double), hipMemcpyHostToDevice, h->st) != hipSuccess && lrc == GPCA_OK)
            lrc = fail(h, GPCA_ERR_HIP, "gpca_rsvd: status copy failed");
        const int xrc = allreduce_f64(h, h->dW, (int64_t)L * L + 16);
        if (xrc != GPCA_OK) return xrc;
    }
    auto tail = [&]() -> int {
        CHK(enqueue_small_eigh(h, gsrc, gslices, zmode, denom));
        return enqueue_scores_loadings(h, Xload, true);
    };
    LOCAL(tail());
    if (mr && hipMemcpyAsync(h->h_status + 16, h->dW + (size_t)L * L, 16 * sizeof(double), hipMemcpyDeviceToHost, h->st) != hipSuccess)
        return lrc != GPCA_OK ? lrc : fail(h, GPCA_ERR_HIP, "gpca_rsvd: status fetch failed");
    {
        const int frc = finish_small_eigh(h, lrc == GPCA_OK);
        if (lrc == GPCA_OK) lrc = frc;
    }
    if (mr) {
        const std::string own_now = h->err;
        const int agreed = status_verdict(h, h->h_status + 16, lrc, h->status_own, "gpca_rsvd (after the last exchange)");
        if (agreed != GPCA_OK) return agreed;
        h->err = own_now;
    }
    return lrc;
}

static bool wants_child(gpca_handle* h, int32_t k, int32_t oversample) {
    if (!h->compact_ok || h->is_child || h->sm.on || multi_rank(h) || h->d_smask || !h->have_stats || (!h->dG && !h->dG2)) return false;
    if (h->n_pca < 1 || k + oversample > h->n_pca) return false;
    if ((h->flags & 3u) != 0) return false;
    const int64_t npad = round_up(h->n_pca, kGQRowsPerWave), dropped = h->Mpad - npad;
    const int64_t pitch = h->storage == GPCA_STORE_2BIT ? h->ld2 : h->ld8;
    if (dropped < 32768 || dropped * pitch < ((int64_t)8 << 20)) return false;
    return 2 * npad <= h->Mpad;
}
static int ensure_child(gpca_handle* h) {
    if (h->child && h->child_valid) return GPCA_OK;
    drop_child(h);
    const bool packed = h->storage == GPCA_STORE_2BIT;
    const int64_t n = h->n_pca, npad = round_up(n, kGQRowsPerWave), pitch = packed ? h->ld2 : h->ld8;
    size_t free_b = 0, total_b = 0;
    HIPCHK(hipMemGetInfo(&free_b, &total_b));
    const double need = (double)npad * (double)pitch + (double)npad * 1024.0 + (double)h->ldg * 8192.0 + 1073741824.0;
    if (need > (double)free_b) return GPCA_ERR_OOM;
    gpca_handle* c = new gpca_handle();
    c->is_child = true; c->compact_ok = 0;
    c->device = h->device; c->precision = h->precision; c->storage = h->storage; c->nd = h->nd; c->ko = h->ko;
    c->st = h->st;
    c->simple_kernels = h->simple_kernels; c->narrow_ok = h->narrow_ok; c->spin_sync = h->spin_sync;
    c->gq_waves_target = h->gq_waves_target; c->gtt_waves_target = h->gtt_waves_target;
    c->timing_on = h->timing_on;
    c->M = n; c->N = h->N; c->Mpad = npad; c->ldg = h->ldg; c->ld8 = h->ld8; c->ld2 = h->ld2; c->cap_rows_pad = npad; c->pack_flags = h->pack_flags;
    h->child = c;
    auto build = [&]() -> int {
        gpca_handle* hh = h;
        (void)hh;
        if (packed) { HIPCHK(malloc_genotypes(h, (void**)&c->dG2, (size_t)npad * (size_t)pitch)); }
        else { HIPCHK(malloc_genotypes(h, (void**)&c->dG, (size_t)npad * (size_t)pitch)); }
        char* gdst = packed ? (char*)c->dG2 : (char*)c->dG;
        if (npad > n) HIPCHK(hipMemsetAsync(gdst + (size_t)n * pitch, 0, (size_t)(npad - n) * pitch, h->st));
        launch_gather_rows(h->st, packed ? (const void*)h->dG2 : (const void*)h->dG, pitch, h->d_pca_rows, n, gdst);
        HIPCHK(hipGetLastError());
        {
            gpca_handle* h = c;
            CHK(alloc_stats(h));
        }
        launch_gather_elems(h->st, h->d_mu, 4, h->d_pca_rows, n, c->d_mu); launch_gather_elems(h->st, h->d_sigma, 4, h->d_pca_rows, n, c->d_sigma);
        launch_gather_elems(h->st, h->d_r, 4, h->d_pca_rows, n, c->d_r); launch_gather_elems(h->st, h->d_b, 4, h->d_pca_rows, n, c->d_b);
        launch_gather_elems(h->st, h->d_counts, 16, h->d_pca_rows, n, c->d_counts);
        HIPCHK(hipGetLastError());
        HIPCHK(hipMemsetAsync(c->d_keep, 1, (size_t)n, h->st)); HIPCHK(hipMemsetAsync(c->d_reason, 0, (size_t)npad, h->st));
        c->pca_rows.resize((size_t)n);
        for (int64_t i = 0; i < n; ++i) c->pca_rows[(size_t)i] = i;
        c->n_pca = n;
        HIPCHK(hipMalloc((void**)&c->d_pca_rows, (size_t)n * 8));
        HIPCHK(hipMemcpyAsync(c->d_pca_rows, c->pca_rows.data(), (size_t)n * 8, hipMemcpyHostToDevice, h->st));
        HIPCHK(hipStreamSynchronize(h->st));
        c->d_row_ids = h->d_pca_rows;
        c->snp_offset = h->snp_offset;
        c->flags = 0; c->have_stats = true;
        return GPCA_OK;
    };
    const int rc = build();
    if (rc != GPCA_OK) { const std::string keep = c->err.empty() ? h->err : c->err; drop_child(h); h->err = keep; return rc; }
    h->child_valid = true;
    return GPCA_OK;
}

extern "C" int gpca_rsvd(gpca_handle* h, int32_t k, int32_t oversample, int32_t power_iters, uint64_t seed) {
    if (!h) return GPCA_ERR_BAD_ARG;
    LOCK(h);
    h->rsvd_on_child = false;
    struct SkipGuard { gpca_handle* h; ~SkipGuard() { h->timing_skip = false; } } skip_guard{h};
    if (!h->is_child) h->timing_skip = h->timing_on && h->timing_every > 1 && (h->timing_calls++ % h->timing_every) != 0;
    if (wants_child(h, k, oversample) && ensure_child(h) == GPCA_OK) {
        gpca_handle* c = h->child;
        c->timing_on = h->timing_on; c->timing_skip = h->timing_skip;
        const int rc = gpca_rsvd(c, k, oversample, power_iters, seed);
        if (rc != GPCA_OK) { h->err = c->err; h->have_rsvd = false; return rc; }
        h->k = c->k; h->l = c->l; h->L = c->L; h->eig = c->eig; h->sv = c->sv;
        h->have_rsvd = true; h->loadings_valid = true; h->rsvd_on_child = true;
        return GPCA_OK;
    }
    const bool mr = multi_rank(h);
    const int pre = rsvd_preflight(h, k, oversample, power_iters);
    if (!mr) { if (pre != GPCA_OK) return pre; }
    else {
        CHK(agree_status_begin(h, pre));
        if (pre != GPCA_OK) return agree_status_end(h, pre, "gpca_rsvd (before the sketch)");
    }
    bool agreement_pending = mr;
    int lrc = GPCA_OK;
    const int l = h->l, L = h->L;
#define EXCHANGE(buf, count) do { \
        if (agreement_pending) { \
            agreement_pending = false; \
            const int arc_ = agree_status_end(h, GPCA_OK, "gpca_rsvd (before the sketch)"); \
            if (arc_ != GPCA_OK) { (void)hipStreamSynchronize(h->st); return arc_; }    \
        } \
        const int xrc_ = allreduce_f64(h, (buf), (count)); if (xrc_ != GPCA_OK) return xrc_; } while (0)
    auto omega = [&]() -> int {
        ScopedTimer t(h, "omega", 0.0, (double)h->M * L * 4.0);
        if (h->precision == GPCA_PREC_I8_EXACT) {
            if (!h->rmax_valid) {
                HIPCHK(hipMemsetAsync(h->d_rmax, 0, 4, h->st));
                launch_max_f32(h->st, h->d_r, h->Mpad, h->d_rmax);
                HIPCHK(hipGetLastError());
                h->rmax_valid = true;
            }
            launch_omega_planes(h->st, h->M, h->Mpad, l, L, h->snp_offset, seed, h->d_r, h->d_b, h->d_cpart, h->dTd, h->d_rmax, h->d_tscale, h->d_tinv, h->nd, h->d_row_ids);
            h->apart_valid = false;
        } else launch_omega(h->st, h->M, h->Mpad, l, L, h->snp_offset, seed, h->d_r, h->d_b, h->dTb, h->d_cpart, nullptr, 1, h->d_row_ids);
        HIPCHK(hipGetLastError());
        return GPCA_OK;
    };
    LOCAL(omega());
    LOCAL(stage_sum_c(h, omega_num_parts(h->Mpad)));
    LOCAL(stage_AtT_local(h, h->precision == GPCA_PREC_I8_EXACT));
    EXCHANGE(h->dY, h->N * (int64_t)L);
    LOCAL(stage_orth(h, power_iters == 0 ? 2 : 1));
    const bool fused = h->sm.on && h->sm.fused && (h->storage == GPCA_STORE_2BIT || !h->simple_kernels || narrow_shape(h));
    for (int it = 0; it < power_iters; ++it) {
        if (fused) LOCAL(stage_power_fused(h));
        else { LOCAL(stage_AQ(h, 1)); LOCAL(stage_AtT_local(h)); }
        EXCHANGE(h->dY, h->N * (int64_t)L);
        LOCAL(stage_orth(h, it + 1 == power_iters ? 2 : 1));
    }
    LOCAL(stage_AQ(h, 0));
    const double n_eff = h->d_smask ? (double)h->n_smask : (double)h->N;
    lrc = call_tail(h, 0, n_eff - 1.0, h->dT, lrc);
    if (lrc != GPCA_OK) return lrc;
#undef EXCHANGE
    h->have_rsvd = true; h->loadings_valid = true;
    return GPCA_OK;
}

#define NEED_RSVD(name) \
    if (!h || !out) return GPCA_ERR_BAD_ARG; \
    LOCK(h); \
    if (!h->have_rsvd) return fail(h, GPCA_ERR_STATE, name ": run gpca_rsvd first")
#define ON_CHILD(call) \
    if (h->rsvd_on_child && h->child) { const int rc_ = (call); if (rc_ != GPCA_OK) h->err = h->child->err; return rc_; }

extern "C" int gpca_get_scores(gpca_handle* h, float* out) {
    NEED_RSVD("gpca_get_scores");
    ON_CHILD(gpca_get_scores(h->child, out));
    HIPCHK(hipMemcpy(out, h->d_scores32, (size_t)h->N * h->k * 4, hipMemcpyDeviceToHost));
    return GPCA_OK;
}
extern "C" int gpca_get_scores_f64(gpca_handle* h, double* out) {
    NEED_RSVD("gpca_get_scores_f64");
    ON_CHILD(gpca_get_scores_f64(h->child, out));
    HIPCHK(hipMemcpy(out, h->d_scores64, (size_t)h->N * h->k * 8, hipMemcpyDeviceToHost));
    return GPCA_OK;
}
extern "C" int gpca_get_eigenvalues(gpca_handle* h, double* out) {
    NEED_RSVD("gpca_get_eigenvalues");
    std::copy(h->eig.begin(), h->eig.end(), out);
    return GPCA_OK;
}
extern "C" int gpca_get_singular_values(gpca_handle* h, double* out) {
    NEED_RSVD("gpca_get_singular_values");
    std::copy(h->sv.begin(), h->sv.end(), out);
    return GPCA_OK;
}
extern "C" int gpca_get_loadings(gpca_handle* h, float* out) {
    NEED_RSVD("gpca_get_loadings");
    ON_CHILD(gpca_get_loadings(h->child, out));
    if (!h->loadings_valid) return fail(h, GPCA_ERR_STATE, "gpca_get_loadings: the last call (gpca_rsvd_condensed) produced sample scores only");
    if (h->n_pca) HIPCHK(hipMemcpy(out, h->d_load32, (size_t)h->n_pca * h->k * 4, hipMemcpyDeviceToHost));
    return GPCA_OK;
}

extern "C" int gpca_transform(gpca_handle* h, double* out) {
    NEED_RSVD("gpca_transform");
    ON_CHILD(gpca_transform(h->child, out));
    if (!h->loadings_valid) return fail(h, GPCA_ERR_STATE, "gpca_transform: the last call (gpca_rsvd_condensed) produced sample scores only");
    HIPCHK(hipSetDevice(h->device));
    const int L = h->L, k = h->k;
    const bool mr = multi_rank(h);
    int lrc = GPCA_OK;
    auto prep = [&]() -> int {
// ... 236 lines not shown
```

genomic_pca_amd/csrc/kernels.h:

```cpp
#pragma once
#include <hip/hip_runtime.h>
#include <stdint.h>
#include "eig_result.h"
#include "plan_math.h"

namespace gpca {

struct QcParams { double min_call_rate, min_maf, max_hwe_p; };

struct KernelOpts {
    int gq_phase = -1;
    int gq_chain = 1;
    int gtt_xcd = 1;
};
int init_device_kernels_i8();
int init_device_kernels_common();
int init_device_kernels_eig();

void launch_small_eigh(hipStream_t st, const double* src, int nslices, int n, int L, int k, int zmode, double denom, const int* cholflag,
                       double* Z, double* res, double* Vout);

template <class T>
__host__ __device__ inline constexpr T acc_row(T row0, int e, int h) { return row0 + (e & 3) + 8 * (e >> 2) + 4 * h; }

__host__ __device__ inline int64_t blocked_t_index(int64_t row, int col, int LT) {
    const int64_t group = row >> 4;
    const int w = (int)(row & 15), lt = col >> 5, cc = col & 31;
    return ((group * LT + lt) * 64 + ((w & 1) * 32 + cc)) * 8 + (w >> 1);
}
__host__ __device__ inline int64_t blocked_q_index(int64_t n, int col, int LT) {
    const int64_t chunk = n >> 5;
    const int w = (int)(n & 31), lt = col >> 5, cc = col & 31;
    return ((chunk * LT + lt) * 64 + ((w >> 4) * 32 + cc)) * 16 + (w & 15);
}

void launch_synth(hipStream_t st, int8_t* G, int64_t M, int64_t N, int64_t ld, int64_t snp_offset,
                  uint64_t seed, const uint32_t* d_thresh, int P);
void launch_synth16(hipStream_t st, void* G, int packed, int64_t rows, int64_t N, int64_t ld, int64_t snp0, uint64_t seed,
                    const uint32_t* d_thresh16, int P);
void launch_bed_decode(hipStream_t st, const uint8_t* bed, int64_t bytes_per_row, int8_t* G, int64_t M,
                       int64_t N, int64_t ld);
void launch_snp_stats(hipStream_t st, const int8_t* G, int64_t M, int64_t N, int64_t ld, QcParams qc,
                      float* mu, float* sigma, float* r, float* b, uint8_t* keep, uint8_t* reason,
                      uint32_t* counts, uint32_t* flags);
void launch_set_scale(hipStream_t st, int64_t M, const float* mu, const float* sigma, const uint8_t* keep,
                      float* r, float* b);
void launch_standardize_block(hipStream_t st, const int8_t* G, int64_t ld, const float* mu,
                              const float* sigma, const int64_t* rows, int64_t ns, const int64_t* cols,
                              int64_t nj, float* out, unsigned long long* err_idx);

void launch_omega(hipStream_t st, int64_t M, int64_t Mpad, int l, int L, int64_t snp_offset, uint64_t seed,
                  const float* r, const float* b, float* Tb, float* cpart, double* apart, int blocked = 1, const int64_t* row_ids = nullptr);
void launch_gather_rows(hipStream_t st, const void* src, int64_t pitch, const int64_t* ids, int64_t n, void* dst);
void launch_gather_elems(hipStream_t st, const void* src, int elem_bytes, const int64_t* ids, int64_t n, void* dst);

void launch_omega_planes(hipStream_t st, int64_t M, int64_t Mpad, int l, int L, int64_t snp_offset, uint64_t seed, const float* r,
                         const float* b, float* cpart, int8_t* Td, const float* rmax, double* tscale, double* tinv, int nd,
                         const int64_t* row_ids = nullptr);
void launch_max_f32(hipStream_t st, const float* r, int64_t n, float* out);

void launch_gq_f32(hipStream_t st, const void* G, int packed, int64_t ldr, const GqPlan& plan, int64_t Npad, const float* Qb,
                   int L, const float* r, const float* b, const float* s, float* Tout, float* Tb, float* cpart);
void launch_gtt_f32(hipStream_t st, const void* G, int packed, int64_t ldr, int64_t Mpad, int64_t Npad, const float* Tb,
                    int L, float* Ypart, const GttPlan& plan);
void launch_reduce_y(hipStream_t st, const float* Ypart, int W, int64_t Npad, int64_t N, int L, const double* c,
                     double* Y);

void launch_sum_partials_f32(hipStream_t st, const float* part, int64_t P, int64_t E, double* out, double* scratch);
void launch_sum_partials_f64(hipStream_t st, const double* part, int64_t P, int64_t E, double* out, double* scratch);
#ifdef __HIPCC__
template <typename T>
__device__ __forceinline__ void sum_partials_body(const T* __restrict__ part, int64_t P, int64_t E, double* __restrict__ out, int S, int bx, int by,
                                                  double (*red)[64]) {
    const int lane = threadIdx.x & 63, wv = threadIdx.x >> 6;
    const int64_t e = (int64_t)bx * 64 + lane;
    const int64_t per = (P + S - 1) / S;
    const int64_t p0 = by * per, p1 = (p0 + per < P) ? p0 + per : P;
    double a0 = 0.0, a1 = 0.0, a2 = 0.0, a3 = 0.0;
    if (e < E) {
        int64_t p = p0 + wv;
        for (; p + 12 < p1; p += 16) {
            a0 += (double)part[p * E + e]; a1 += (double)part[(p + 4) * E + e];
            a2 += (double)part[(p + 8) * E + e]; a3 += (double)part[(p + 12) * E + e];
        }
        for (; p < p1; p += 4) a0 += (double)part[p * E + e];
    }
    red[wv][lane] = (a0 + a1) + (a2 + a3);
    __syncthreads();
    if (wv == 0 && e < E) out[(int64_t)by * E + e] = ((red[0][lane] + red[1][lane]) + red[2][lane]) + red[3][lane];
}
#endif
void launch_sum_partials_f64_stage1(hipStream_t st, const double* part, int64_t P, int64_t E, double* scratch, const double** src, int* slices);
void launch_gram_f64(hipStream_t st, const double* X, int64_t rows, int L, double* part);
void launch_gram_f32(hipStream_t st, const float* X, int64_t rows, int L, double* part);
constexpr double kDigitScale = 0.49 * 268435456.0;
constexpr double kDigitScale3 = 0.49 * 16777216.0;
inline double digit_scale(int nd) { return nd == 3 ? kDigitScale3 : kDigitScale; }
void launch_apply_right_tail(hipStream_t st, double* X, int64_t rows, int L, const double* Z, float* Qout, int64_t rows_pad,
                             double* csum_part, double* amax_part);
void launch_finish_q(hipStream_t st, const double* csum_part, const double* amax_part, int64_t P, int L, double* s64, float* s32,
                     double* scale, double* inv, int nd = 4);
int launch_chol_inv(hipStream_t st, const double* W, int n, int ld, double* Z, int* flag);
void launch_chol_inv_fold(hipStream_t st, const double* part, int P, int n, int ld, double* Z, int* flag);
void launch_apply_right_inplace(hipStream_t st, double* X, int64_t rows, int L, const double* Z, float* Qb,
                                int64_t rows_pad);
void launch_rightmul_f64(hipStream_t st, const double* X, int64_t rows, int L, const double* Z, int K, double* out64,
                         float* out32);
void launch_rightmul_gather_f32(hipStream_t st, const float* X, const int64_t* row_ids, int64_t nrows, int L,
                                const double* Z, int K, float* out32, const int* sign = nullptr);
void launch_scores(hipStream_t st, const double* X, int64_t rows, int L, const double* Z, int K, double* out64, double* cand_val, int64_t* cand_idx);
void launch_scores_sign(hipStream_t st, double* out64, float* out32, int64_t rows, int K, const double* cand_val, const int64_t* cand_idx,
                        int64_t parts, int* sign);
void launch_colsum_f64(hipStream_t st, const double* X, int64_t rows, int L, double* part);
void launch_col_sign(hipStream_t st, const double* X, int64_t rows, int K, int* sign);
void launch_scale_cols(hipStream_t st, double* X64, float* X32, int64_t rows, int K, const int* sign);
void launch_f64_to_f32(hipStream_t st, const double* in, float* out, int64_t n);
void launch_fill_f32(hipStream_t st, float* p, int64_t n, float v);
void launch_expand_loadings(hipStream_t st, const float* load, const int64_t* rows, int64_t n_pca, int k, int L, float* Tp);
void launch_scale_rows(hipStream_t st, const float* X, int64_t M, int64_t Mpad, int L, const float* r, const float* b,
                       float* Tb, float* cpart, int blocked = 1);


void launch_bd_expand(hipStream_t st, const float* W, const int32_t* feat0, int cmax, const double* P, int64_t M, int L, float* out);
void launch_bd_reduce(hipStream_t st, const float* W, const int32_t* feat0, int cmax, const float* T, int L, const int64_t* blk_row0,
                      const int64_t* blk_row1, const int32_t* blk_feat0, const int32_t* blk_c, int B, double* P);
void launch_rightmul_inplace_f32(hipStream_t st, float* X, int64_t rows, int L, const double* Z);
void launch_mask_rows(hipStream_t st, double* Y, int64_t N, int L, const uint8_t* mask);
void launch_f32_to_f64(hipStream_t st, const float* in, double* out, int64_t n);

constexpr int kDigits = 4;
void launch_gq_i8(hipStream_t st, const int8_t* G, int64_t ldg, const GqPlan& plan, int64_t N, const int8_t* Qd,
                  const double* qscale, const float* r, const float* b, const float* s, float* Tout, float* cpart,
                  int scale_out, int64_t ldt = 32, const KernelOpts& ko = KernelOpts());
void launch_gtt_i8(hipStream_t st, const int8_t* G, int64_t ldg, int64_t Mpad, int64_t Npad, const int8_t* Td,
                   double* Ypart, const Gtt8Plan& plan, const KernelOpts& ko = KernelOpts());
void launch_gtt_n(hipStream_t st, const int8_t* G, int64_t ldg, int64_t Mpad, int64_t Npad, const int8_t* Td, double* Ypart,
                  const Gtt8Plan& plan);
int launch_gq_n(hipStream_t st, const int8_t* G, int64_t ldg, const GqPlan& plan, int64_t N, const int8_t* Qd,
                const double* qscale, const float* r, const float* b, const float* s, float* Tout, float* cpart, double* apart,
                int scale_out, int64_t ldt = 32);
void launch_reduce_y_i8(hipStream_t st, const double* Ypart, int W, int64_t Npad, int64_t N, const double* c,
                        const double* tscale, double* Y, int64_t ldy = 32);
void launch_accum_y_i8(hipStream_t st, const double* Ypart, int W, int64_t Npad, int64_t N, double* Yint, int first);
void launch_finish_y_i8(hipStream_t st, const double* Yint, int64_t N, const double* c, const double* tscale, double* Y, int64_t ldy = 32);
void launch_absmax_fold(hipStream_t st, const double* apart, int64_t P, double* run);
void launch_accum_y_scaled(hipStream_t st, const double* Ypart, int W, int64_t Npad, int64_t N, const double* tscale, double* Yacc, int first);
void launch_finish_y_sum(hipStream_t st, const double* Yacc, int64_t N, const double* c, double* Y, int64_t ldy = 32);
void launch_quantize_f32(hipStream_t st, const float* X, int64_t rows, int64_t rows_pad, double* part, double* scale,
                         double* inv, int8_t* Xd, int layout = 0, int nd = 4, int64_t ldx = 32);
void launch_quantize_f64(hipStream_t st, const double* X, int64_t rows, int64_t rows_pad, double* part, double* scale,
                         double* inv, int8_t* Xd, int layout = 0, int nd = 4, int64_t ldx = 32);

constexpr int64_t kSamplePad2bit = 1024;
void launch_bed_to_codes(hipStream_t st, const uint8_t* bed, int64_t bpr, uint8_t* G2, int64_t M, int64_t N, int64_t ld2);
void launch_pack_i8(hipStream_t st, const int8_t* G8, int64_t ld8, uint8_t* G2, int64_t rows, int64_t N, int64_t ld2,
                    unsigned* flags);
void launch_snp_stats_2bit(hipStream_t st, const uint8_t* G2, int64_t M, int64_t N, int64_t ld2, QcParams qc, float* mu,
                           float* sigma, float* r, float* b, uint8_t* keep, uint8_t* reason, uint32_t* counts, uint32_t* flags);
void launch_standardize_block_2bit(hipStream_t st, const uint8_t* G2, int64_t ld2, const float* mu, const float* sigma,
                                   const int64_t* rows, int64_t ns, const int64_t* cols, int64_t nj, float* out,
                                   unsigned long long* err_idx);
void launch_gq_2bit(hipStream_t st, const uint8_t* G2, int64_t ld2, const GqPlan& plan, int64_t Npad, const int8_t* Qd,
                    const double* qscale, const float* r, const float* b, const float* s, float* Tout, float* cpart,
                    double* apart, int scale_out, int nd = 4, int64_t ldt = 32);
void launch_quantize_f64_prescaled(hipStream_t st, const double* X, int64_t rows, int64_t rows_pad, const double* inv, int8_t* Xd, int layout, int nd = 4, int64_t ldx = 32);
void launch_quantize_f64_finishq(hipStream_t st, const double* X, int64_t rows, int64_t rows_pad, int8_t* Xd, int layout, int nd, int64_t ldx,
                                 const double* csum_part, const double* amax_part, int64_t P, int ldp, double* s64, float* s32, double* scale, double* inv);
void launch_quantize_f32_premax(hipStream_t st, const float* X, int64_t rows, int64_t rows_pad, const double* apart, int64_t P,
                                double* scale, double* inv, int8_t* Xd, int layout, int nd = 4, int64_t ldx = 32);
void launch_post_k1(hipStream_t st, const float* cpart, int64_t units, double* cscratch, const double* apart, int64_t P, double* scale, double* inv, int nd);
void launch_quantize_f32_cfold(hipStream_t st, const float* X, int64_t rows, int64_t rows_pad, const double* inv, int8_t* Xd, int layout, int nd,
                               int64_t ldx, const double* cscratch, int cslices, double* c);
int launch_gtt_p(hipStream_t st, const uint8_t* G2, int64_t ld2, int64_t Mpad, int64_t Npad, const int8_t* Td, double* Ypart,
                 const Gtt8Plan& plan, int nd = 4, const KernelOpts& ko = KernelOpts());
int launch_gtt_d(hipStream_t st, const int8_t* G, int64_t ldg, int64_t Mpad, int64_t Npad, const int8_t* Td, double* Ypart,
                 const Gtt8Plan& plan, const KernelOpts& ko = KernelOpts());
int launch_gq_d(hipStream_t st, const int8_t* G, int64_t ldg, const GqPlan& plan, int64_t Npad, const int8_t* Qd,
                const double* qscale, const float* r, const float* b, const float* s, float* Tout, float* cpart, double* apart,
                int scale_out, int64_t ldt = 32, const KernelOpts& ko = KernelOpts());
void launch_gtt_2bit(hipStream_t st, const uint8_t* G2, int64_t ld2, int64_t Mpad, int64_t Npad, const int8_t* Td,
                     double* Ypart, const Gtt8Plan& plan, int nd = 4);


void launch_project(hipStream_t st, const void* G, int packed, int64_t ldr, int64_t Mpad, int64_t Npad, const int8_t* Ta, const int8_t* Tb,
                    const uint32_t* rmask, double* Ypa, double* Ypb, unsigned* cnt, unsigned* bad, const PrjPlan& plan, int nd, int lazy_b);
void launch_project_correct(hipStream_t st, const double* Yint_b, int64_t N, const double* tscale_b, const unsigned* cnt, int64_t n_model,
                            double* Y, int64_t ldy);
void launch_project_colmax(hipStream_t st, const float* X, int64_t rows, int L, unsigned long long* out);
void launch_project_used(hipStream_t st, const unsigned* cnt, int64_t N, double n_model, double* used);

constexpr int kGrmDigits = 6;
constexpr int kGrmFlushRows = 4096;
constexpr int kGrmTabBytes = 4 * kGrmDigits * 32;
void launch_grm(hipStream_t st, const void* G, int packed, int64_t ldr, int64_t rows_pad, const int8_t* tab, const uint32_t* kmask,
                const int2* tiles, int64_t ntiles, int64_t row0, int64_t row1, int64_t N, double* R, int* Q, int first);
void launch_grm_vec(hipStream_t st, const void* G, int packed, int64_t ldr, int64_t rows, int64_t Npad, const uint8_t* keep,
                    const int64_t* qc, const int64_t* qe, double* Up, double* Vp, unsigned* cnt, unsigned* bad);
void launch_grm_vec_fold(hipStream_t st, const double* Up, const double* Vp, int64_t rows, int64_t Npad, double* u, double* v);
void launch_grm_finish(hipStream_t st, const double* R, const int* Q, const double* u, const double* v, const unsigned* cnt, double S,
                       double beta, double K, int64_t row0, int64_t row1, double* out, double* npairs);

void launch_king(hipStream_t st, const void* G, int packed, int64_t ldr, int64_t rows_pad, const uint32_t* kmask, const int2* tiles,
                 int64_t ntiles, int64_t row0, int64_t row1, int64_t N, double* R, int64_t E, int first);
void launch_king_vec(hipStream_t st, const void* G, int packed, int64_t ldr, int64_t rows, int64_t Npad, const uint8_t* keep,
                     unsigned* het, unsigned* miss, unsigned* bad);
void launch_king_vec_f64(hipStream_t st, const unsigned* het, const unsigned* miss, int64_t Npad, double* het_f, double* miss_f);
void launch_king_finish(hipStream_t st, const double* R, int64_t E, const double* het, const double* miss, double K, int64_t row0,
                        int64_t row1, double* kin, int* counts);

void launch_ld(hipStream_t st, const void* G, int packed, int64_t ldr, const int64_t* krows, int64_t K, int64_t N, int64_t row0,
               int64_t row1, const int64_t* win_end, int wmax, int weff, int* W);
void launch_ld_vec(hipStream_t st, const void* G, int packed, int64_t ldr, const int64_t* krows, int64_t N, int64_t row0, int64_t hi,
                   unsigned* stat, unsigned long long* bad);
void launch_ld_finish(hipStream_t st, const int* W, const unsigned* stat, int64_t N, int64_t row0, int64_t row1, const int64_t* win_end,
                      int wmax, double threshold, double* r2, int* counts, unsigned long long* above);

void launch_pcrelate_beta(hipStream_t st, const void* G, int packed, int64_t ldr, const int64_t* krows, int64_t K, int64_t N,
                          const uint8_t* train, const double* Hw, int P, float* betaG, float* beta_rm, unsigned long long* bad);
void launch_pcrelate_isaf(hipStream_t st, const float* betaG, const float* X, int P, int64_t N, int64_t row0, int64_t row1, float* mu);
void launch_pcrelate_inv(hipStream_t st, const void* G, int packed, int64_t ldr, const int64_t* krows, int64_t K, int64_t N,
                         const float* betaG, const float* X, int P, float tau, unsigned* inv);
int launch_pcrelate(hipStream_t st, const void* G, int packed, int64_t ldr, const int64_t* krows, int64_t K, int64_t N, const float* betaG,
                    const float* X, int P, float tau, const int2* tiles, int64_t ntiles, int64_t row0, int64_t row1, double* R, int* Q, int64_t E);
void launch_pcrelate_finish(hipStream_t st, const double* R, const int* Q, const unsigned* inv, int64_t K, int64_t E, int64_t row0,
                            int64_t row1, double* kin, int* nsnp);

int launch_assoc(hipStream_t st, const void* G, int packed, int64_t ldr, const int64_t* krows, int64_t N, const float* Bt,
                 const unsigned* incw, int L, int64_t row0, int64_t row1, double* xb, unsigned* sums, unsigned long long* bad);
void launch_assoc_finish(hipStream_t st, const double* xb, const unsigned* sums, const double* yy, int T, int L, double df, double max_vif,
                         int64_t rows, double* stats, double* info);

int launch_assoc_score_count(hipStream_t st, const void* G, int packed, int64_t ldr, const int64_t* krows, int64_t N, const unsigned* incw,
                             int64_t row0, int64_t row1, unsigned* sums, unsigned long long* bad);
int launch_assoc_score(hipStream_t st, const void* G, int packed, int64_t ldr, const int64_t* krows, int64_t N, const float* Bt,
                       const unsigned* incw, int T, int L, int64_t row0, int64_t row1, const unsigned* sums, double* dv);
void launch_assoc_score_finish(hipStream_t st, const double* dv, const unsigned* sums, int T, int Pc, double max_vif, int64_t rows,
                               double* stats, double* ua, double* info);

void launch_assoc_spa_flag(hipStream_t st, const double* stats, const double* dv, int T, int Pc, int64_t item0, int64_t nitems, double spa_z,
                           double* out, int* list, unsigned* count);
int launch_assoc_spa(hipStream_t st, const void* G, int packed, int64_t ldr, const int64_t* krows, int64_t N, const unsigned* incw,
                     const unsigned* sums, const double* dv, const double* Z, const double* mu, int T, int Pc, int64_t row0, int64_t item0,
                     const int* list, const unsigned* count, double* gws, double* out);

}
```

genomic_pca_amd/csrc/plan_math.h:

```cpp
#pragma once
#include <stdint.h>
#include <algorithm>
#include <initializer_list>
#include <vector>

namespace gpca {

constexpr int64_t kSamplePad = 256;
constexpr int kGQRowsPerWave = 128;
constexpr int kMaxSketchCols = 128;

inline int64_t omega_num_parts(int64_t Mpad) { return (Mpad + 63) / 64; }

constexpr int kSumSlicesMax = 64, kSumSlicesMaxNarrow = 256;
inline int sum_slices(int64_t P, int64_t E) {
    const int64_t cap = E <= 64 ? kSumSlicesMaxNarrow : kSumSlicesMax;
    int64_t s = (P + 63) / 64;
    return (int)(s < 1 ? 1 : (s > cap ? cap : s));
}
inline int64_t sum_scratch_need(int64_t E) { return (E <= 64 ? (int64_t)kSumSlicesMaxNarrow : (int64_t)kSumSlicesMax) * E; }
constexpr int64_t kPostK1Scratch = 256 * 32;
inline int post_k1_slices(int64_t units) { return sum_slices(units, 32); }
inline int64_t sum_scratch_capacity(int Lmax) {
    const int64_t E = (int64_t)Lmax * Lmax;
    const int64_t need = std::max(sum_scratch_need(64), sum_scratch_need(E));
    return std::max<int64_t>(need, (int64_t)(Lmax / 32) * kPostK1Scratch);
}

inline int64_t gram_rows_per_block(int64_t rows) {
    if (rows <= 262144) {
        int64_t parts = rows / 256;
        parts = parts < 32 ? 32 : (parts > 64 ? 64 : parts);
        const int64_t q = (rows + parts - 1) / parts;
        return q < 32 ? 32 : (q + 31) / 32 * 32;
    }
    int64_t r = (rows + 1023) / 1024;
    r = (r + 31) / 32 * 32;
    return r < 32 ? 32 : (r > 2048 ? 2048 : r);
}
inline int64_t gram_num_parts(int64_t rows) { const int64_t rpb = gram_rows_per_block(rows); return (rows + rpb - 1) / rpb; }
inline int64_t gram_max_parts(int64_t rows) {
    if (rows <= 262144) return 64;
    return std::max<int64_t>(1024, (rows + 2047) / 2048);
}

constexpr int kTailRows = 64;
inline int64_t tail_num_parts(int64_t rows_pad) { return (rows_pad + kTailRows - 1) / kTailRows; }
constexpr int64_t kFinishQFoldMax = 512;

constexpr int kScoreParts = 48;
inline int64_t scores_num_parts(int64_t rows) { const int64_t c = (rows + 255) / 256; return c < kScoreParts ? (c < 1 ? 1 : c) : kScoreParts; }
constexpr int kColsumRowsPerBlock = 256;
inline int64_t colsum_num_parts(int64_t rows) { return (rows + kColsumRowsPerBlock - 1) / kColsumRowsPerBlock; }
constexpr int kAbsmaxRowsPerBlock = 1024;
inline int64_t absmax_num_parts(int64_t rows) { return (rows + kAbsmaxRowsPerBlock - 1) / kAbsmaxRowsPerBlock; }

struct GqPlan { int64_t units; int64_t waves; };
inline GqPlan gq_plan(int64_t Mpad, int waves_target) {
    GqPlan p;
    p.units = Mpad / 32;
    int64_t w = waves_target < 4 ? 4 : waves_target;
    if (w > p.units) w = p.units;
    w = (w + 3) / 4 * 4;
    p.waves = w;
    return p;
}
struct GttPlan { int64_t nblocks_n; int W; int64_t rows_per_wave; int64_t grid; };
inline GttPlan gtt_plan(int64_t Mpad, int64_t Npad, int L, int target_waves) {
    GttPlan p;
    p.nblocks_n = Npad / kSamplePad;
    int64_t W = target_waves / p.nblocks_n;
    if (W < 1) W = 1;
    const int64_t maxW = Mpad / 32;
    if (W > maxW) W = maxW;
    int64_t rpw = (Mpad + W - 1) / W;
    rpw = (rpw + 31) / 32 * 32;
    W = (Mpad + rpw - 1) / rpw;
    p.W = (int)W;
    p.rows_per_wave = rpw;
    const int64_t ngroups = (p.nblocks_n + 3) / 4;
    p.grid = ngroups * W;
    (void)L;
    return p;
}
struct Gtt8Plan { int64_t nblocks_n; int W; int64_t rows_per_wave; int64_t grid; int tasks_per_wg; int64_t S; int64_t ngroups; int strided; int64_t C; };
inline Gtt8Plan gtt8_plan(int64_t Mpad, int64_t Npad, int target_waves) {
    Gtt8Plan p{};
    p.nblocks_n = Npad / 128;
    int64_t W = target_waves / p.nblocks_n;
    if (W < 1) W = 1;
    const int64_t minW = (Mpad + ((int64_t)1 << 22) - 1) >> 22;
    if (W < minW) W = minW;
    const int64_t maxW = Mpad / 128;
    if (W > maxW) W = maxW;
    int64_t rpw = (Mpad + W - 1) / W;
    rpw = (rpw + 127) / 128 * 128;
    W = (Mpad + rpw - 1) / rpw;
    p.W = (int)W;
    p.rows_per_wave = rpw;
    p.grid = ((p.nblocks_n + 3) / 4) * W;
    return p;
}
inline Gtt8Plan gtt8_plan_batched(int64_t Mpad, int64_t Npad, int target_waves) {
    Gtt8Plan p{};
    p.nblocks_n = Npad / 128;
    p.ngroups = (p.nblocks_n + 3) / 4;
    p.S = Mpad / 128;
    int64_t grid0 = target_waves / 8;
    if (grid0 < 1) grid0 = 1;
    const int64_t wmin = std::max<int64_t>(1, (p.S + 32767) / 32768), wmax = std::min<int64_t>(p.S, 1024);
    double best = 1e300;
    int64_t bestW = wmin;
    for (int64_t W = wmin; W <= std::max(wmin, wmax); ++W) {
        const int64_t T = W * p.ngroups, k = (T + grid0 - 1) / grid0;
        double f = (double)(k * grid0) / (double)T;
        f *= 1.0 + 3.0 * (double)W / (double)p.S;
        f += (double)W * 256.0 / (double)Mpad;
        if ((double)p.S / (double)W * 16384.0 > 3.0 * 1048576.0) f += 0.02;
        if (f < best - 1e-12) { best = f; bestW = W; }
    }
    p.C = (p.S + bestW - 1) / bestW;
    p.W = (int)((p.S + p.C - 1) / p.C);
    const int64_t T = (int64_t)p.W * p.ngroups;
    p.tasks_per_wg = (int)((T + grid0 - 1) / grid0);
    p.grid = (T + p.tasks_per_wg - 1) / p.tasks_per_wg;
    p.strided = 1;
    p.rows_per_wave = p.C * 128;
    return p;
}
constexpr int64_t kNarrowSamples = 256;
inline Gtt8Plan gtt8_plan_narrow(int64_t Mpad, int64_t N, int target_waves) {
    Gtt8Plan p{};
    p.nblocks_n = (N + 127) / 128;
    int64_t W = target_waves / p.nblocks_n;
    if (W < 1) W = 1;
    const int64_t maxW = Mpad / 128;
    if (W > maxW) W = maxW;
    int64_t rpw = (Mpad + W - 1) / W;
    rpw = (rpw + 127) / 128 * 128;
    W = (Mpad + rpw - 1) / rpw;
    p.W = (int)W;
    p.rows_per_wave = rpw;
    p.grid = (W * p.nblocks_n + 3) / 4;
    return p;
}
struct PrjPlan { int64_t ngroups; int W; int64_t rows_per_wave; int64_t grid; };
inline PrjPlan prj_plan(int64_t Mpad, int64_t Npad, int target_waves) {
    PrjPlan p{};
    const int64_t nblocks = Npad / 64;
    p.ngroups = (nblocks + 3) / 4;
    int64_t W = target_waves / nblocks;
    if (W < 1) W = 1;
    const int64_t minW = (Mpad + ((int64_t)1 << 22) - 1) >> 22;
    if (W < minW) W = minW;
    const int64_t maxW = Mpad / 128;
    if (W > maxW) W = maxW;
    if (W < 1) W = 1;
    int64_t rpw = (Mpad + W - 1) / W;
    rpw = (rpw + 127) / 128 * 128;
    W = (Mpad + rpw - 1) / rpw;
    p.W = (int)W;
    p.rows_per_wave = rpw;
    p.grid = p.ngroups * W;
    return p;
}

inline int64_t part64_capacity(int64_t M, int64_t Mpad, int64_t N, int64_t Npad, int L) {
    return std::max({std::max(gram_num_parts(N), gram_max_parts(std::max(M, N))) * (int64_t)L * L, colsum_num_parts(Npad) * (int64_t)L,
                     absmax_num_parts(Mpad) * (int64_t)32, 2 * tail_num_parts(Npad) * (int64_t)L});
}
inline int64_t cpart_capacity(int64_t gq_waves, int64_t Mpad, int L) {
    return std::max({gq_waves * (int64_t)L, omega_num_parts(Mpad) * (int64_t)L, Mpad * (int64_t)(L / 32)});
}
inline int64_t scores_cand_capacity() { return (int64_t)kScoreParts * kMaxSketchCols; }
inline int64_t project_scratch_capacity(int Lp) { return sum_scratch_need(Lp); }
inline int64_t project_part_capacity(int64_t Mpad, int Lp) { return std::max<int64_t>(absmax_num_parts(Mpad) * 32, 2 * (int64_t)Lp); }
inline int64_t project_cpart_capacity(int64_t Mpad, int Lp) { return omega_num_parts(Mpad) * (int64_t)Lp; }

constexpr int kLdRows = 64, kLdCols = 128, kLdStage = 128, kLdThreads = 256;
constexpr int kLdProducts = 6;
inline int64_t ld_row_blocks(int64_t rows) { return (rows + kLdRows - 1) / kLdRows; }
inline int64_t ld_col_tiles(int64_t weff) { return (kLdRows - 1 + weff) / 32 + 1; }
inline int64_t ld_col_chunks(int64_t weff) { return (ld_col_tiles(weff) + kLdCols / 32 - 1) / (kLdCols / 32); }
inline int64_t ld_stages(int64_t N) { return (N + kLdStage - 1) / kLdStage; }
inline int64_t ld_stages_per_split(int64_t nblocks, int64_t nst) {
    int64_t S = nblocks >= 1024 ? 1 : (1024 + nblocks - 1) / std::max<int64_t>(nblocks, 1);
    if (S > nst) S = nst;
    if (S < 1) S = 1;
    return (nst + S - 1) / S;
}
inline int64_t ld_splits(int64_t nblocks, int64_t nst) { const int64_t per = ld_stages_per_split(nblocks, nst); return (nst + per - 1) / per; }
constexpr int64_t ld_above_words(int64_t wmax) { return (wmax + 63) / 64; }
inline int64_t ld_ws_capacity(int64_t rows, int64_t wmax) { return (int64_t)kLdProducts * rows * wmax; }
inline int64_t ld_stat_capacity(int64_t row0, int64_t hi) { return 3 * (hi - row0); }
inline int64_t ld_r2_capacity(int64_t rows, int64_t wmax) { return rows * wmax; }
inline int64_t ld_counts_capacity(int64_t rows, int64_t wmax) { return 6 * rows * wmax; }
inline int64_t ld_above_capacity(int64_t rows, int64_t wmax) { return rows * ld_above_words(wmax); }

constexpr int kPcrTile = 128, kPcrThreads = 512, kPcrStageRows = 16, kPcrFlushRows = 256, kPcrMaxPcs = 32;
constexpr int kPcrBetaRows = 64;
constexpr int kPcrBetaWaves = 4;
static_assert(kPcrFlushRows % kPcrStageRows == 0 && kPcrBetaRows % kPcrStageRows == 0 && kPcrStageRows % 8 == 0, "stage, flush group, beta block");
inline int64_t pcr_kpad(int64_t K) { return (K + kPcrBetaRows - 1) / kPcrBetaRows * kPcrBetaRows; }
inline int64_t pcr_npad(int64_t N) { return (N + kPcrTile - 1) / kPcrTile * kPcrTile; }
constexpr int64_t pcr_stages(int64_t K) { return (K + kPcrStageRows - 1) / kPcrStageRows; }
inline int pcr_beta_width(int P) {
    const int w = (P + 1 + kPcrBetaWaves - 1) / kPcrBetaWaves;
    for (int c : {1, 2, 3, 4, 6, 9}) if (w <= c) return c;
    return 0;
}
inline int64_t pcr_beta_capacity(int64_t K, int P) { return pcr_kpad(K) * (int64_t)(P + 1); }
inline int64_t pcr_x_capacity(int64_t N, int P) { return pcr_npad(N) * (int64_t)(P + 1); }
inline int64_t pcr_hat_capacity(int64_t N, int P) { return (int64_t)kPcrBetaWaves * N * pcr_beta_width(P); }
inline int64_t pcr_inv_capacity(int64_t N) { return pcr_npad(N); }

constexpr int kGrmTile = 64, kKingTile = 128;
constexpr int64_t band_entries(int64_t row0, int64_t row1, bool diag) {
    return diag ? row1 * (row1 + 1) / 2 - row0 * (row0 + 1) / 2 : row1 * (row1 - 1) / 2 - row0 * (row0 - 1) / 2;
}
constexpr int64_t band_index(int64_t row0, int64_t a, int64_t b, bool diag) {
    return (diag ? a * (a + 1) / 2 - row0 * (row0 + 1) / 2 : a * (a - 1) / 2 - row0 * (row0 - 1) / 2) + b;
}
constexpr int64_t band_tile_count(int64_t row0, int64_t row1, int tile) {
    return ((row1 + tile - 1) / tile) * ((row1 + tile - 1) / tile + 1) / 2 - (row0 / tile) * (row0 / tile + 1) / 2;
}
template <class Tile>
inline void band_tile_list(int64_t row0, int64_t row1, int tile, std::vector<Tile>& tiles) {
    tiles.clear();
    tiles.reserve((size_t)band_tile_count(row0, row1, tile));
    for (int64_t ta = row0 / tile; ta < (row1 + tile - 1) / tile; ++ta)
        for (int64_t tb = 0; tb <= ta; ++tb) { Tile t{}; t.x = (int)ta; t.y = (int)tb; tiles.push_back(t); }
}

constexpr int kAscRows = 128, kAscThreads = 256, kAscStage = 64, kAscFlush = 256, kAscMaxCols = 64;
constexpr int kAscGPitch = kAscStage + 8;
constexpr int kAscBPitch = kAscStage + 4;
static_assert(kAscFlush % kAscStage == 0 && kAscStage % 32 == 0 && kAscThreads * 32 == kAscRows * kAscStage, "stage, flush group, staging map");
constexpr int asc_lpad(int L) { return L <= 32 ? 32 : 64; }
constexpr int64_t asc_npad(int64_t N) { return (N + kAscStage - 1) / kAscStage * kAscStage; }
constexpr int64_t asc_stages(int64_t N) { return (N + kAscStage - 1) / kAscStage; }
constexpr int64_t asc_row_blocks(int64_t rows) { return (rows + kAscRows - 1) / kAscRows; }
constexpr int64_t asc_b_capacity(int64_t N, int L) { return (int64_t)asc_lpad(L) * asc_npad(N); }
constexpr int64_t asc_inc_capacity(int64_t N) { return asc_npad(N) / 32; }
constexpr int64_t asc_xb_capacity(int64_t rows, int L) { return rows * (int64_t)L; }
constexpr int64_t asc_sums_capacity(int64_t rows) { return 3 * rows; }
constexpr int64_t asc_stats_capacity(int64_t rows, int T) { return 3 * rows * (int64_t)T; }
constexpr int64_t asc_info_capacity(int64_t rows) { return 4 * rows; }

constexpr int kAsrMaxCols = 64, kAsrCountRows = 4, kAsrCountThreads = 64 * kAsrCountRows, kAsrChunk = 64 * 32;
static_assert(kAsrMaxCols == kAscMaxCols && kAsrChunk % kAscStage == 0, "the score scan stages its panel as k_assoc does");
constexpr int asr_cols(int T, int Pc) { return T * (Pc + 3); }
constexpr int asr_max_traits(int Pc) { return kAsrMaxCols / (Pc + 3); }
constexpr int asr_col_w(int t) { return t; }
constexpr int asr_col_r(int T, int t) { return T + t; }
constexpr int asr_col_a(int T, int Pc, int t, int j) { return 2 * T + t * (Pc + 1) + j; }
constexpr int64_t asr_count_blocks(int64_t rows) { return (rows + kAsrCountRows - 1) / kAsrCountRows; }
constexpr int64_t asr_count_chunks(int64_t N) { return (asc_npad(N) + kAsrChunk - 1) / kAsrChunk; }
constexpr int64_t asr_dv_capacity(int64_t rows, int L) { return rows * (int64_t)L; }
constexpr int64_t asr_sums_capacity(int64_t rows) { return 3 * rows; }
constexpr int64_t asr_stats_capacity(int64_t rows, int T) { return 5 * rows * (int64_t)T; }
constexpr int64_t asr_ua_capacity(int64_t rows, int T, int Pc) { return rows * (int64_t)asr_cols(T, Pc); }
constexpr int64_t asr_info_capacity(int64_t rows) { return 5 * rows; }

constexpr int kAspThreads = 256, kAspChunk = kAspThreads * 32, kAspMaxSlots = 1024;
constexpr int64_t kAspWsBytes = (int64_t)256 << 20, kAspListItems = (int64_t)1 << 20;
static_assert(kAspChunk % kAscStage == 0, "a chunk is whole stages: a fetch below asc_npad(N) stays inside the row's pitch");
constexpr int64_t asp_gpad(int64_t N) { return asc_npad(N); }
constexpr int64_t asp_chunks(int64_t N) { return (asp_gpad(N) + kAspChunk - 1) / kAspChunk; }
constexpr int64_t asp_slots(int64_t N) {
    const int64_t s = kAspWsBytes / (8 * asp_gpad(N > 0 ? N : 1));
    return s < 1 ? 1 : (s > kAspMaxSlots ? kAspMaxSlots : s);
}
constexpr int64_t asp_ranges(int64_t rows, int T) { return (rows * (int64_t)T + kAspListItems - 1) / kAspListItems; }
constexpr int64_t asp_g_capacity(int64_t N) { return asp_slots(N) * asp_gpad(N); }
constexpr int64_t asp_z_capacity(int64_t N, int T, int Pc) { return (int64_t)T * (Pc + 1) * asp_gpad(N); }
constexpr int64_t asp_mu_capacity(int64_t N, int T) { return (int64_t)T * asp_gpad(N); }
constexpr int64_t asp_list_capacity(int64_t rows, int T) { return rows * (int64_t)T < kAspListItems ? rows * (int64_t)T : kAspListItems; }
constexpr int64_t asp_out_capacity(int64_t rows, int T) { return 4 * rows * (int64_t)T; }

}
```

include/gpca.h:

```cpp
#ifndef GPCA_H
#define GPCA_H

#include <stddef.h>
#include <stdint.h>

#if defined(__GNUC__)
#define GPCA_API __attribute__((visibility("default")))
#else
#define GPCA_API
#endif

#ifdef __cplusplus
extern "C" {
#endif

#define GPCA_VERSION 250
#define GPCA_MISSING_I8 (-127)

typedef struct gpca_handle gpca_handle;

typedef enum gpca_status {
    GPCA_OK = 0,
    GPCA_ERR_BAD_ARG = -1,
    GPCA_ERR_OOM = -2,
    GPCA_ERR_HIP = -3,
    GPCA_ERR_RCCL = -4,
    GPCA_ERR_MISSING_GENOTYPE = -5,
    GPCA_ERR_NOT_CONVERGED = -6,
    GPCA_ERR_STATE = -7,
    GPCA_ERR_NO_DEVICE = -8,
    GPCA_ERR_INVALID_GENOTYPE = -9
} gpca_status;

typedef enum gpca_precision {
    GPCA_PREC_DEFAULT = 0,
    GPCA_PREC_I8_EXACT = 1,
    GPCA_PREC_F32_MFMA = 2
} gpca_precision;

typedef enum gpca_storage {
    GPCA_STORE_AUTO = 0,
    GPCA_STORE_2BIT = 1,
    GPCA_STORE_INT8 = 2
} gpca_storage;

typedef struct gpca_config {
    int32_t device;
    int32_t precision;
    int32_t storage;
    int32_t digit_planes;
    int32_t reserved[4];
} gpca_config;
#define GPCA_CFG_SIMPLE_KERNELS 1
#define GPCA_CFG_NO_COMPACT 2
#define GPCA_CFG_NO_NARROW 4
#define GPCA_CFG_NO_SPIN_SYNC 8
#define GPCA_CFG_ALL 15

typedef struct gpca_qc_config {
    double min_snp_call_rate;
    double min_snp_maf;
    double max_snp_hwe_p_value;
} gpca_qc_config;

GPCA_API int gpca_version(void);
GPCA_API const char* gpca_status_string(int status);
GPCA_API int gpca_create(const gpca_config* cfg, gpca_handle** out);
GPCA_API int gpca_destroy(gpca_handle* h);
GPCA_API const char* gpca_last_error(gpca_handle* h);

GPCA_API int gpca_upload_genotypes_i8(gpca_handle* h, const int8_t* snp_major, int64_t M, int64_t N, int64_t ld);
GPCA_API int gpca_upload_bed2bit(gpca_handle* h, const uint8_t* bed_rows, int64_t M, int64_t N);
GPCA_API int gpca_synth_genotypes(gpca_handle* h, int64_t M, int64_t N, uint64_t seed, const uint32_t* thresh,
                         int32_t P, int64_t snp_offset);
GPCA_API int gpca_download_genotypes_i8(gpca_handle* h, int8_t* out, int64_t ld);

typedef enum gpca_panel_kind {
    GPCA_PANEL_HOST_I8 = 0,
    GPCA_PANEL_HOST_BED = 1,
    GPCA_PANEL_SYNTH = 2,
    GPCA_PANEL_SYNTH16 = 3,
    GPCA_PANEL_MAPPED_I8 = 4,
    GPCA_PANEL_MAPPED_BED = 5
} gpca_panel_kind;
#define GPCA_SOURCE_REGISTER 1
#define GPCA_SOURCE_BENCH_HOLD 2
typedef int (*gpca_panel_fn)(void* user, int64_t row0, int64_t rows, void* dst, int64_t ld);
typedef struct gpca_panel_source {
    int32_t kind;
    int32_t n_pop;
    gpca_panel_fn fill;
    void* user;
    const uint32_t* thresh;
    uint64_t seed;
    int64_t snp_offset;
    int64_t host_ld;
    int64_t flags;
} gpca_panel_source;
GPCA_API int gpca_load_from_source(gpca_handle* h, const gpca_panel_source* src, int64_t M, int64_t N);
GPCA_API int gpca_stream_open(gpca_handle* h, const gpca_panel_source* src, int64_t M, int64_t N, int64_t panel_rows,
                              int32_t ring_slots);
GPCA_API int gpca_stream_set_fused(gpca_handle* h, int32_t fused);
GPCA_API int gpca_stream_set_cache(gpca_handle* h, int64_t max_bytes, int32_t* n_cached);
typedef struct gpca_stream_info {
    int64_t panel_rows;
    int32_t n_panels, ring_slots, n_cached;
    int32_t staging_buffers;
    int32_t zero_staging;
    int32_t copy_threads;
    int64_t fills;
    double fill_host_ms;
    double fill_wait_ms;
    double register_ms;
    int64_t reserved[4];
} gpca_stream_info;
GPCA_API int gpca_stream_get_info(gpca_handle* h, gpca_stream_info* out);
GPCA_API int gpca_dims(gpca_handle* h, int64_t* M, int64_t* N);
GPCA_API int gpca_get_storage(gpca_handle* h, int32_t* storage, int32_t* precision);
GPCA_API int gpca_get_device_memory(gpca_handle* h, int64_t* free_bytes, int64_t* total_bytes);

GPCA_API int gpca_snp_stats(gpca_handle* h, const gpca_qc_config* qc, float* mu, float* sigma, uint8_t* keep);
GPCA_API int gpca_get_snp_qc_detail(gpca_handle* h, uint32_t* counts, uint8_t* reason);
GPCA_API int gpca_set_standardization(gpca_handle* h, const float* mu, const float* sigma, const uint8_t* keep);
GPCA_API int gpca_get_standardization(gpca_handle* h, float* mu, float* sigma, uint8_t* keep);
GPCA_API int gpca_host_eigh_desc(const double* a_sym, int32_t n, double* w, double* v);
GPCA_API int gpca_device_eigh_desc(gpca_handle* h, const double* a_sym, int32_t n, double* w, double* v);
GPCA_API int gpca_device_orth(gpca_handle* h, const double* Y, int32_t l, int32_t rounds, double* Q, double* s, int32_t* pivot_flag);
GPCA_API int gpca_device_tail(gpca_handle* h, const double* Q, const float* B, int32_t l, int32_t k, int32_t zmode);
GPCA_API double gpca_hwe_chi_squared_p_value(uint64_t n_hom1, uint64_t n_het, uint64_t n_hom2);

GPCA_API int gpca_standardize_block(gpca_handle* h, const int64_t* pca_snp_ids, int64_t ns,
                           const int64_t* qc_sample_ids, int64_t nj, float* out);
GPCA_API int64_t gpca_num_pca_snps(gpca_handle* h);
GPCA_API int64_t gpca_num_qc_samples(gpca_handle* h);
GPCA_API int gpca_get_pca_snp_rows(gpca_handle* h, int64_t* rows);

GPCA_API int gpca_rsvd(gpca_handle* h, int32_t k, int32_t oversample, int32_t power_iters, uint64_t seed);
GPCA_API int gpca_get_scores(gpca_handle* h, float* out );
GPCA_API int gpca_get_scores_f64(gpca_handle* h, double* out );
GPCA_API int gpca_get_eigenvalues(gpca_handle* h, double* out );
GPCA_API int gpca_get_singular_values(gpca_handle* h, double* out );
GPCA_API int gpca_get_loadings(gpca_handle* h, float* out );
GPCA_API int gpca_transform(gpca_handle* h, double* out);
GPCA_API int gpca_project(gpca_handle* h, const float* mu, const float* sigma, const float* W, int32_t k, double* scores, int32_t* n_used);

enum { GPCA_GRM_STANDARDIZED = 0, GPCA_GRM_CENTRED = 1 };
GPCA_API int gpca_grm(gpca_handle* h, int32_t scaling, int64_t row0, int64_t row1, double* grm, float* npairs );

GPCA_API int gpca_king(gpca_handle* h, int64_t row0, int64_t row1, double* kinship, int32_t* counts );

GPCA_API int gpca_ld_window(gpca_handle* h, int64_t row0, int64_t row1, const int64_t* win_end , int32_t wmax,
                            double threshold, double* r2 , int32_t* counts ,
                            uint64_t* above );

GPCA_API int gpca_pcrelate_isaf(gpca_handle* h, const double* V , int32_t P, const uint8_t* train , int64_t row0,
                                int64_t row1, float* mu , float* beta );
GPCA_API int gpca_pcrelate(gpca_handle* h, const double* V , int32_t P, const uint8_t* train , double tau,
                           int64_t row0, int64_t row1, double* kinship, int32_t* nsnp );

GPCA_API int gpca_assoc_linear(gpca_handle* h, const double* Y , int32_t T, const double* C , int32_t Pc,
                               const uint8_t* include , double max_vif, int64_t row0, int64_t row1,
                               double* stats , double* xb ,
                               double* rowinfo );
GPCA_API double gpca_student_t_log10p(double t, double df);

GPCA_API int gpca_logistic_null(const double* y , const double* C , int32_t Pc,
                                const uint8_t* include , int64_t N, double* alpha ,
                                double* mu , int32_t* iters );
GPCA_API int gpca_assoc_logistic_score(gpca_handle* h, const double* Y , int32_t T, const double* C ,
                                       int32_t Pc, const uint8_t* include , double max_vif, int64_t row0, int64_t row1,
                                       double* stats , double* ua ,
                                       double* rowinfo );
GPCA_API double gpca_normal_log10p(double z);

GPCA_API int gpca_assoc_logistic_spa(gpca_handle* h, const double* Y , int32_t T, const double* C ,
                                     int32_t Pc, const uint8_t* include , double max_vif, double spa_z, int64_t row0,
                                     int64_t row1, double* stats , double* spa ,
                                     double* ua , double* rowinfo );
GPCA_API int gpca_spa_log10p(const double* gt , const double* mu , int64_t n, double u, double* log10p,
                             double* zeta , int32_t* status );

GPCA_API int gpca_copy_rows(gpca_handle* dst, gpca_handle* src, int64_t row0, int64_t rows);
GPCA_API int gpca_set_sample_mask(gpca_handle* h, const uint8_t* mask );
GPCA_API int gpca_set_condensed_basis(gpca_handle* h, const float* W , const int32_t* feat0 , int32_t cmax, int64_t R);
GPCA_API int gpca_rsvd_condensed(gpca_handle* h, int32_t k, int32_t oversample, int32_t power_iters, uint64_t seed);
GPCA_API int gpca_refine(gpca_handle* h, const double* S0 , int32_t k);

#define GPCA_UNIQUE_ID_BYTES 128
GPCA_API int gpca_comm_get_unique_id(void* out_id );
GPCA_API int gpca_comm_init(gpca_handle* h, int32_t world, int32_t rank, const void* unique_id, int64_t snp_offset);
typedef int (*gpca_allreduce_fn)(void* user, double* host_buf, int64_t count);
GPCA_API int gpca_set_allreduce_hook(gpca_handle* h, gpca_allreduce_fn fn, void* user, int32_t world,
                            int32_t rank, int64_t snp_offset);

GPCA_API int gpca_comm_count_ranks(gpca_handle* h, int32_t* ranks);

typedef struct gpca_kernel_timing {
    char name[32];
    int64_t launches;
    double total_ms;
    double flops;
    double bytes;
} gpca_kernel_timing;
GPCA_API int gpca_get_timings(gpca_handle* h, gpca_kernel_timing* out, int32_t cap, int32_t* n);
GPCA_API int gpca_reset_timings(gpca_handle* h);
GPCA_API int gpca_enable_timings(gpca_handle* h, int32_t on);
GPCA_API int gpca_synchronize(gpca_handle* h);

#ifdef __cplusplus
}
// ... 3 lines not shown
```

Measured before the change: 991.3 billion.

## Process two 32-column sketch halves in one paired GEMM launch

Adds paired kernels (k_gq_d2, k_gtt_d2) that split the grid so workgroups in adjacent groups of 8 handle the two 32-column halves of the sketch in a single launch, instead of looping over halves with separate launches. The pairing interleaves the halves so workgroups reading the same genotype rows run together, which is meant to let the halves share genotype traffic in cache and to cut launch count. Plans, Ypart and apart buffer capacities and the absmax folds are adjusted for per-half strides. It is on by default for i8-exact int8 storage with L>=64 and can be disabled with a new config flag. The cost is more scratch memory and more complex grid indexing.

Measured after the change: 956.2 billion. -3.5%, worse.

```diff
diff --git a/genomic_pca_amd/_lib.py b/genomic_pca_amd/_lib.py
--- a/genomic_pca_amd/_lib.py
+++ b/genomic_pca_amd/_lib.py
@@ -31,6 +31,7 @@
 CFG_NO_COMPACT = 2
 CFG_NO_NARROW = 4
 CFG_NO_SPIN_SYNC = 8
+CFG_NO_PAIRED_HALVES = 16
 
 
 class GpcaLibraryError(RuntimeError):
diff --git a/genomic_pca_amd/csrc/gemm_i8.hip b/genomic_pca_amd/csrc/gemm_i8.hip
--- a/genomic_pca_amd/csrc/gemm_i8.hip
+++ b/genomic_pca_amd/csrc/gemm_i8.hip
@@ -559,22 +559,24 @@
     GQD_STAMP(2 + 2 * round_ix)
 }
 
-template <int NT>
-__global__ __launch_bounds__(256, 1) void k_gq_d(const int8_t* __restrict__ G, int64_t ldg, int64_t units, int64_t nstage,
-                                                  const int8_t* __restrict__ Qd, const double* __restrict__ qscale,
-                                                  const float* __restrict__ rv, const float* __restrict__ bv,
-                                                  const float* __restrict__ sv, float* __restrict__ Tout,
-                                                  float* __restrict__ cpart, double* __restrict__ apart, int scale_out, int64_t ldt,
-                                                  int chain_ok, int phase_mul) {
+template <int NT, bool PAIR>
+__device__ __forceinline__ void gqd_workgroup(const int8_t* __restrict__ G, int64_t ldg, int64_t units, int64_t nstage,
+                                              const int8_t* __restrict__ Qd, const double* __restrict__ qscale,
+                                              const float* __restrict__ rv, const float* __restrict__ bv,
+                                              const float* __restrict__ sv, float* __restrict__ Tout,
+                                              float* __restrict__ cpart, double* __restrict__ apart, int scale_out, int64_t ldt,
+                                              int chain_ok, int phase_mul, const unsigned pwg) {
     extern __shared__ __attribute__((aligned(16))) char gqd_smem[];
     GqdSmem* sm = reinterpret_cast<GqdSmem*>(gqd_smem);
     __builtin_assume(nstage >= 2 && (nstage & 1) == 0);
     const int lane = threadIdx.x & 63;
     const int wv = __builtin_amdgcn_readfirstlane(threadIdx.x >> 6);
     const int c = lane & 31, h = lane >> 5;
-    const uint32_t ph = (uint32_t)(((int64_t)(blockIdx.x & 7) * (phase_mul & 0xffff) + (int64_t)(blockIdx.x >> 3) * (phase_mul >> 16)) % nstage);
-    const int64_t u0 = (units * (int64_t)blockIdx.x) / gridDim.x;
-    const int64_t u1 = (units * ((int64_t)blockIdx.x + 1)) / gridDim.x;
+#define GQD_WG (PAIR ? pwg : blockIdx.x)
+#define GQD_NWG (PAIR ? gridDim.x >> 1 : gridDim.x)
+    const uint32_t ph = (uint32_t)(((int64_t)(GQD_WG & 7) * (phase_mul & 0xffff) + (int64_t)(GQD_WG >> 3) * (phase_mul >> 16)) % nstage);
+    const int64_t u0 = (units * (int64_t)GQD_WG) / GQD_NWG;
+    const int64_t u1 = (units * ((int64_t)GQD_WG + 1)) / GQD_NWG;
     float amax = 0.f;
     const float sj = sv[c];
     const double qs = qscale[c];
@@ -614,7 +616,52 @@
 #endif
     float am_lo, am_hi; halves_pair(amax, am_lo, am_hi);
     const float am = fmaxf(am_lo, am_hi);
-    if (h == 0) apart[((int64_t)blockIdx.x * 4 + wv) * 32 + c] = (double)am;
+    if (h == 0) apart[((int64_t)GQD_WG * 4 + wv) * 32 + c] = (double)am;
+#undef GQD_WG
+#undef GQD_NWG
+}
+
+template <int NT>
+__global__ __launch_bounds__(256, 1) void k_gq_d(const int8_t* __restrict__ G, int64_t ldg, int64_t units, int64_t nstage,
+                                                  const int8_t* __restrict__ Qd, const double* __restrict__ qscale,
+                                                  const float* __restrict__ rv, const float* __restrict__ bv,
+                                                  const float* __restrict__ sv, float* __restrict__ Tout,
+                                                  float* __restrict__ cpart, double* __restrict__ apart, int scale_out, int64_t ldt,
+                                                  int chain_ok, int phase_mul) {
+    gqd_workgroup<NT, false>(G, ldg, units, nstage, Qd, qscale, rv, bv, sv, Tout, cpart, apart, scale_out, ldt, chain_ok, phase_mul, 0u);
+}
+
+template <int NT>
+__global__ __launch_bounds__(256, 1) void k_gq_d2(const int8_t* __restrict__ G, int64_t ldg, int64_t units, int64_t nstage,
+                                                   const int8_t* __restrict__ Qd, const double* __restrict__ qscale,
+                                                   const float* __restrict__ rv, const float* __restrict__ bv,
+                                                   const float* __restrict__ sv, float* __restrict__ Tout,
+                                                   float* __restrict__ cpart, double* __restrict__ apart, int scale_out, int64_t ldt,
+                                                   int chain_ok, int phase_mul, int64_t qd_half, int64_t cpart_half, int64_t apart_half) {
+    const PairId p = pair_id(blockIdx.x, gridDim.x);
+    const unsigned hf = __builtin_amdgcn_readfirstlane(p.half);
+    gqd_workgroup<NT, true>(G, ldg, units, nstage, Qd + hf * qd_half, qscale + 32 * hf, rv, bv, sv + 32 * hf, Tout + 32 * hf, cpart + hf * cpart_half,
+                            apart + hf * apart_half, scale_out, ldt, chain_ok, phase_mul, __builtin_amdgcn_readfirstlane(p.wg));
+}
+
+static inline int gqd_phase(const KernelOpts& ko, int64_t nstage) {
+    int phase = ko.gq_phase;
+    if (phase < 0) phase = (nstage >= 16 && nstage <= 400) ? (int)((nstage / 8) << 16) : 0;
+    return phase;
+}
+
+int launch_gq_d2(hipStream_t st, const int8_t* G, int64_t ldg, const GqPlan& plan, int64_t Npad, const int8_t* Qd, int64_t qd_half,
+                 const double* qscale, const float* r, const float* b, const float* s, float* Tout, float* cpart, int64_t cpart_half,
+                 double* apart, int64_t apart_half, int scale_out, int64_t ldt, const KernelOpts& ko) {
+    if (!dma_shape_ok(Npad, 256, plan.units * 32, 32) || ldg < Npad || plan.waves < 8 || plan.waves % 8 != 0 || ldt < 64) return (int)hipErrorInvalidValue;
+    const dim3 grid((unsigned)(plan.waves / 4)), blk(256);
+    const int64_t nstage = Npad / 128;
+    const int phase = gqd_phase(ko, nstage);
+#if GPCA_STAMP
+    if (!ko.gq_nt) { hipLaunchKernelGGL((k_gq_d2<0>), grid, blk, sizeof(GqdSmem), st, G, ldg, plan.units, nstage, Qd, qscale, r, b, s, Tout, cpart, apart, scale_out, ldt, ko.gq_chain, phase, qd_half, cpart_half, apart_half); return 0; }
+#endif
+    hipLaunchKernelGGL((k_gq_d2<1>), grid, blk, sizeof(GqdSmem), st, G, ldg, plan.units, nstage, Qd, qscale, r, b, s, Tout, cpart, apart, scale_out, ldt, ko.gq_chain, phase, qd_half, cpart_half, apart_half);
+    return 0;
 }
 
 int launch_gq_d(hipStream_t st, const int8_t* G, int64_t ldg, const GqPlan& plan, int64_t Npad, const int8_t* Qd,
@@ -623,8 +670,10 @@
     if (!dma_shape_ok(Npad, 256, plan.units * 32, 32) || ldg < Npad) return (int)hipErrorInvalidValue;
     const dim3 grid((unsigned)(plan.waves / 4)), blk(256);
     const int64_t nstage = Npad / 128;
-    int phase = ko.gq_phase;
-    if (phase < 0) phase = (nstage >= 16 && nstage <= 400) ? (int)((nstage / 8) << 16) : 0;
+#if GPCA_STAMP
+    if (!ko.gq_nt) { hipLaunchKernelGGL((k_gq_d<0>), grid, blk, sizeof(GqdSmem), st, G, ldg, plan.units, nstage, Qd, qscale, r, b, s, Tout, cpart, apart, scale_out, ldt, ko.gq_chain, gqd_phase(ko, nstage)); return 0; }
+#endif
+    const int phase = gqd_phase(ko, nstage);
     hipLaunchKernelGGL((k_gq_d<1>), grid, blk, sizeof(GqdSmem), st, G, ldg, plan.units, nstage, Qd, qscale, r, b, s, Tout, cpart, apart, scale_out, ldt, ko.gq_chain, phase);
     return 0;
 }
@@ -782,9 +831,9 @@
 struct K2Walk {
     int64_t wch, g, wch_step, g_step, ngroups;
     int ntask;
-    __device__ __forceinline__ void init(int64_t vwg, int64_t T, int64_t ngroups_, int tasks_per_wg, int strided) {
+    __device__ __forceinline__ void init(int64_t vwg, int64_t T, int64_t ngroups_, int tasks_per_wg, int strided, int64_t grid = 0) {
         ngroups = ngroups_;
-        const int64_t t_first = strided ? vwg : vwg * tasks_per_wg, t_step = strided ? (int64_t)gridDim.x : 1;
+        const int64_t t_first = strided ? vwg : vwg * tasks_per_wg, t_step = strided ? (grid ? grid : (int64_t)gridDim.x) : 1;
         ntask = 0;
         if (t_first < T) { const int64_t left = (T - 1 - t_first) / t_step + 1; ntask = (int)(left < tasks_per_wg ? left : tasks_per_wg); }
         wch = t_first / ngroups; g = t_first - wch * ngroups;
@@ -793,10 +842,10 @@
     __device__ __forceinline__ void advance() { wch += wch_step; g += g_step; if (g >= ngroups) { g -= ngroups; ++wch; } }
 };
 
-template <int NT, int ABL = 0>
-__global__ __launch_bounds__(256, 1) void k_gtt_d(const uint8_t* __restrict__ Gb, int64_t ldr, int64_t Npad,
-                                                   const int8_t* __restrict__ Td, double* __restrict__ Ypart,
-                                                   int64_t S, int64_t C, int64_t ngroups, int W, int tasks_per_wg, int strided, int xcd_remap) {
+template <int NT, int ABL, bool PAIR>
+__device__ __forceinline__ void gtd_workgroup(const uint8_t* __restrict__ Gb, int64_t ldr, int64_t Npad,
+                                              const int8_t* __restrict__ Td, double* __restrict__ Ypart,
+                                              int64_t S, int64_t C, int64_t ngroups, int W, int tasks_per_wg, int strided, int xcd_remap, int64_t td_half, int64_t yp_half) {
     extern __shared__ __attribute__((aligned(16))) char gqd_smem[];
     GqdSmem* sm = reinterpret_cast<GqdSmem*>(gqd_smem);
     const int lane = threadIdx.x & 63;
@@ -807,7 +856,11 @@
 #endif
     constexpr uint32_t TKB = kDigits * 1024;
     K2Walk cw;
-    cw.init(k2_virtual_wg(xcd_remap), (int64_t)W * ngroups, ngroups, tasks_per_wg, strided);
+    if constexpr (PAIR) {
+        const int64_t v = k2_virtual_wg(xcd_remap), hf = v & 1;
+        Td += hf * td_half; Ypart += hf * yp_half;
+        cw.init(v >> 1, (int64_t)W * ngroups, ngroups, tasks_per_wg, strided, (int64_t)(gridDim.x >> 1));
+    } else cw.init(k2_virtual_wg(xcd_remap), (int64_t)W * ngroups, ngroups, tasks_per_wg, strided);
     const int ntask = cw.ntask;
     if (ntask == 0) return;
     auto task_of = [&](const K2Walk& w) -> GtdTask {
@@ -901,6 +954,21 @@
 #if GPCA_STAMP
     if (threadIdx.x == 0 && blockIdx.x < 4096) g_gtd_stamp[2 * blockIdx.x + 1] = __builtin_amdgcn_s_memrealtime();
 #endif
+}
+
+template <int NT, int ABL = 0>
+__global__ __launch_bounds__(256, 1) void k_gtt_d(const uint8_t* __restrict__ Gb, int64_t ldr, int64_t Npad,
+                                                   const int8_t* __restrict__ Td, double* __restrict__ Ypart,
+                                                   int64_t S, int64_t C, int64_t ngroups, int W, int tasks_per_wg, int strided, int xcd_remap) {
+    gtd_workgroup<NT, ABL, false>(Gb, ldr, Npad, Td, Ypart, S, C, ngroups, W, tasks_per_wg, strided, xcd_remap, 0, 0);
+}
+
+template <int NT>
+__global__ __launch_bounds__(256, 1) void k_gtt_d2(const uint8_t* __restrict__ Gb, int64_t ldr, int64_t Npad,
+                                                    const int8_t* __restrict__ Td, double* __restrict__ Ypart,
+                                                    int64_t S, int64_t C, int64_t ngroups, int W, int tasks_per_wg, int strided, int xcd_remap,
+                                                    int64_t td_half, int64_t yp_half) {
+    gtd_workgroup<NT, 0, true>(Gb, ldr, Npad, Td, Ypart, S, C, ngroups, W, tasks_per_wg, strided, xcd_remap, td_half, yp_half);
 }
 
 struct GtpStage { i32x4 t[4][kDigits][64]; char g[4][4096]; };
@@ -1015,7 +1083,22 @@
     if (plan.tasks_per_wg < 1 || plan.S * 128 != Mpad || !dma_shape_ok(Npad, 256, Mpad, kGQRowsPerWave) || ldg < Npad) return (int)hipErrorInvalidValue;
     const dim3 grid((unsigned)plan.grid), blk(256);
     const int remap = ko.gtt_xcd;
+#if GPCA_STAMP
+    if (!ko.gq_nt) { hipLaunchKernelGGL((k_gtt_d<0>), grid, blk, sizeof(GqdSmem), st, (const uint8_t*)G, ldg, Npad, Td, Ypart, plan.S, plan.C, plan.ngroups, plan.W, plan.tasks_per_wg, plan.strided, remap); return 0; }
+#endif
     hipLaunchKernelGGL((k_gtt_d<1>), grid, blk, sizeof(GqdSmem), st, (const uint8_t*)G, ldg, Npad, Td, Ypart, plan.S, plan.C, plan.ngroups, plan.W, plan.tasks_per_wg, plan.strided, remap);
+    return 0;
+}
+
+int launch_gtt_d2(hipStream_t st, const int8_t* G, int64_t ldg, int64_t Mpad, int64_t Npad, const int8_t* Td, int64_t td_half, double* Ypart,
+                  int64_t yp_half, const Gtt8Plan& plan, const KernelOpts& ko) {
+    if (plan.tasks_per_wg < 1 || plan.S * 128 != Mpad || !dma_shape_ok(Npad, 256, Mpad, kGQRowsPerWave) || ldg < Npad || yp_half < (int64_t)plan.W * Npad * 32) return (int)hipErrorInvalidValue;
+    const dim3 grid((unsigned)(2 * plan.grid)), blk(256);
+    const int remap = ko.gtt_xcd;
+#if GPCA_STAMP
+    if (!ko.gq_nt) { hipLaunchKernelGGL((k_gtt_d2<0>), grid, blk, sizeof(GqdSmem), st, (const uint8_t*)G, ldg, Npad, Td, Ypart, plan.S, plan.C, plan.ngroups, plan.W, plan.tasks_per_wg, plan.strided, remap, td_half, yp_half); return 0; }
+#endif
+    hipLaunchKernelGGL((k_gtt_d2<1>), grid, blk, sizeof(GqdSmem), st, (const uint8_t*)G, ldg, Npad, Td, Ypart, plan.S, plan.C, plan.ngroups, plan.W, plan.tasks_per_wg, plan.strided, remap, td_half, yp_half);
     return 0;
 }
 
@@ -1026,6 +1109,11 @@
     GPCA_OPT_IN((k_gq_d<1>), sizeof(GqdSmem))
     GPCA_OPT_IN((k_gtt_p<kDigits>), sizeof(GtpSmem)) GPCA_OPT_IN((k_gtt_p<3>), sizeof(GtpSmem))
     GPCA_OPT_IN((k_gtt_d<1>), sizeof(GqdSmem))
+    GPCA_OPT_IN((k_gq_d2<1>), sizeof(GqdSmem)) GPCA_OPT_IN((k_gtt_d2<1>), sizeof(GqdSmem))
+#if GPCA_STAMP
+    GPCA_OPT_IN((k_gq_d<0>), sizeof(GqdSmem)) GPCA_OPT_IN((k_gtt_d<0>), sizeof(GqdSmem))
+    GPCA_OPT_IN((k_gq_d2<0>), sizeof(GqdSmem)) GPCA_OPT_IN((k_gtt_d2<0>), sizeof(GqdSmem))
+#endif
 #undef GPCA_OPT_IN
     return e;
 }
diff --git a/genomic_pca_amd/csrc/gpca_api.cpp b/genomic_pca_amd/csrc/gpca_api.cpp
--- a/genomic_pca_amd/csrc/gpca_api.cpp
+++ b/genomic_pca_amd/csrc/gpca_api.cpp
@@ -82,6 +82,7 @@
         h->compact_ok = (flags & GPCA_CFG_NO_COMPACT) == 0;
         h->narrow_ok = (flags & GPCA_CFG_NO_NARROW) == 0;
         h->spin_sync = (flags & GPCA_CFG_NO_SPIN_SYNC) == 0;
+        h->pair_halves = (flags & GPCA_CFG_NO_PAIRED_HALVES) == 0;
         if (gqw) h->gq_waves_target = std::max(4, (int)gqw);
         if (gtw) h->gtt_waves_target = std::max(4, (int)gtw);
     }
diff --git a/genomic_pca_amd/csrc/gpca_internal.h b/genomic_pca_amd/csrc/gpca_internal.h
--- a/genomic_pca_amd/csrc/gpca_internal.h
+++ b/genomic_pca_amd/csrc/gpca_internal.h
@@ -145,6 +145,7 @@
     GttPlan plan{};
     GqPlan gqplan{};
     Gtt8Plan plan8{};
+    Gtt8Plan plan8p{};
     int8_t *dQd = nullptr, *dTd = nullptr;
     bool c_fold_pending = false;
     double* d_apart = nullptr; size_t cap_apart = 0; bool apart_valid = false; int64_t apart_parts = 0;
@@ -181,6 +182,7 @@
     uint64_t gen = 0;
     int simple_kernels = 0;
     int narrow_ok = 1;
+    int pair_halves = 1;
     int gq_waves_target = 1024, gtt_waves_target = 2048;
 
     gpca_handle* child = nullptr;
diff --git a/genomic_pca_amd/csrc/gpca_rsvd.cpp b/genomic_pca_amd/csrc/gpca_rsvd.cpp
--- a/genomic_pca_amd/csrc/gpca_rsvd.cpp
+++ b/genomic_pca_amd/csrc/gpca_rsvd.cpp
@@ -162,6 +162,12 @@
 
 static inline GqPlan k1_plan(const gpca_handle* h, int64_t rows_pad) { return gq_plan(rows_pad, h->gq_waves_target); }
 
+static inline bool paired_halves(const gpca_handle* h) {
+    return h->pair_halves && h->precision == GPCA_PREC_I8_EXACT && h->storage == GPCA_STORE_INT8 && !h->simple_kernels && !narrow_shape(h) && h->L >= 64;
+}
+static inline GqPlan k1_plan_paired(const GqPlan& plan) { return gq_plan_paired(plan); }
+static inline Gtt8Plan k2_plan_paired(const gpca_handle* h, int64_t rows_pad) { return gtt8_plan_paired(rows_pad, h->ldg, h->gtt_waves_target); }
+
 static int k2_panel(gpca_handle* h, const PanelView& pv, const int8_t* Td_half, const Gtt8Plan& plan) {
     const int8_t* Td = Td_half + (size_t)(pv.row0 >> 5) * kPlaneBytesPerBlock;
     const bool packed = h->storage == GPCA_STORE_2BIT;
@@ -199,17 +205,29 @@
         const size_t yint_half = (size_t)h->N * 32;
         {
             const double by = h->storage == GPCA_STORE_2BIT ? elems / 4 : elems;
-            ScopedTimer sweep(h, "gemm_GtT", 2.0 * elems * h->l, by * halves, nullptr, streamed);
+            const bool pair = paired_halves(h);
+            const int per = pair ? 2 : 1;
+            ScopedTimer sweep(h, "gemm_GtT", 2.0 * elems * h->l, by * (halves / per), nullptr, streamed);
             CHK(for_each_panel(h, [&](const PanelView& pv) -> int {
-                const Gtt8Plan plan = streamed ? k2_plan(h, pv.rows_pad) : h->plan8;
-                for (int hf = 0; hf < halves; ++hf) {
+                const Gtt8Plan plan = pair ? (streamed ? k2_plan_paired(h, pv.rows_pad) : h->plan8p) : (streamed ? k2_plan(h, pv.rows_pad) : h->plan8);
+                const size_t yp_half = (size_t)ypart64_half_stride(plan.W, h->ldg);
+                for (int hf = 0; hf < halves; hf += per) {
                     {
-                        ScopedTimer t(h, "gemm_GtT", 2.0 * elems * h->l / halves, by, nullptr, !streamed);
-                        CHK(k2_panel(h, pv, h->dTd + hf * td_half, plan));
+                        ScopedTimer t(h, "gemm_GtT", 2.0 * elems * h->l / halves * per, by, nullptr, !streamed);
+                        if (pair) {
+                            const int e = launch_gtt_d2(h->st, pv.g8, h->ld8, pv.rows_pad, h->ldg, h->dTd + hf * td_half + (size_t)(pv.row0 >> 5) * kPlaneBytesPerBlock, (int64_t)td_half,
+                                                        h->dYpart64, (int64_t)yp_half, plan, h->ko);
+                            if (e != 0) return fail(h, GPCA_ERR_HIP, "k_gtt_d2 launch failed (hip error " + std::to_string(e) + ")");
+                            HIPCHK(hipGetLastError());
+                        }
+                        else CHK(k2_panel(h, pv, h->dTd + hf * td_half, plan));
                     }
-                    if (streamed) launch_accum_y_i8(h->st, h->dYpart64, plan.W, h->ldg, h->N, h->d_yint + hf * yint_half, pv.index == 0);
-                    else launch_reduce_y_i8(h->st, h->dYpart64, plan.W, h->ldg, h->N, h->d_c + 32 * hf, h->d_tscale + 32 * hf, h->dY + 32 * hf, L);
-                    HIPCHK(hipGetLastError());
+                    for (int j = 0; j < per; ++j) {
+                        const double* yp = h->dYpart64 + j * yp_half;
+                        if (streamed) launch_accum_y_i8(h->st, yp, plan.W, h->ldg, h->N, h->d_yint + (hf + j) * yint_half, pv.index == 0);
+                        else launch_reduce_y_i8(h->st, yp, plan.W, h->ldg, h->N, h->d_c + 32 * (hf + j), h->d_tscale + 32 * (hf + j), h->dY + 32 * (hf + j), L);
+                        HIPCHK(hipGetLastError());
+                    }
                 }
                 return GPCA_OK;
             }));
@@ -239,14 +257,18 @@
         const bool packed = h->storage == GPCA_STORE_2BIT, streamed = h->sm.on;
         const size_t qhalf = (size_t)h->ldg * 32 * kDigits;
         const size_t chalf = (size_t)h->Mpad;
-        const size_t ahalf = (size_t)h->gqplan.waves * 32;
+        const size_t ahalf = (size_t)apart_half_stride(h->gqplan.waves);
+        const bool pair = paired_halves(h);
+        const int per = pair ? 2 : 1;
+        const int64_t aparts = pair ? k1_plan_paired(h->gqplan).waves / 2 : h->gqplan.waves;
         if (streamed && scale_out) HIPCHK(hipMemsetAsync(h->d_amax_run, 0, kMaxSketch * 8, h->st));
         {
             const double by = packed ? elems / 4 : elems;
-            ScopedTimer sweep(h, "gemm_GQ", 2.0 * elems * h->l, by * halves, nullptr, streamed);
+            ScopedTimer sweep(h, "gemm_GQ", 2.0 * elems * h->l, by * (halves / per), nullptr, streamed);
             CHK(for_each_panel(h, [&](const PanelView& pv) -> int {
                 const GqPlan plan = streamed ? k1_plan(h, pv.rows_pad) : h->gqplan;
-                for (int hf = 0; hf < halves; ++hf) {
+                const GqPlan pplan = k1_plan_paired(plan);
+                for (int hf = 0; hf < halves; hf += per) {
                     const int8_t* Qd = h->dQd + hf * qhalf;
                     const double* qsc = h->d_qscale + 32 * hf;
                     const float* s32 = h->d_s32 + 32 * hf;
@@ -254,8 +276,12 @@
                     float* Th = h->dT + (size_t)pv.row0 * L + 32 * hf;
                     float* cp = h->d_cpart + hf * chalf + (size_t)pv.row0;
                     double* ap = h->d_apart + hf * ahalf;
-                    ScopedTimer t(h, "gemm_GQ", 2.0 * elems * h->l / halves, by, nullptr, !streamed);
-                    if (packed) launch_gq_2bit(h->st, pv.g2, h->ld2, plan, h->ldg, Qd, qsc, rr, bb, s32, Th, cp, ap, scale_out, h->nd, L);
+                    ScopedTimer t(h, "gemm_GQ", 2.0 * elems * h->l / halves * per, by, nullptr, !streamed);
+                    if (pair) {
+                        const int e = launch_gq_d2(h->st, pv.g8, h->ld8, pplan, h->ldg, Qd, (int64_t)qhalf, qsc, rr, bb, s32, Th, cp, (int64_t)chalf, ap, (int64_t)ahalf, scale_out, L, h->ko);
+                        if (e != 0) return fail(h, GPCA_ERR_HIP, "k_gq_d2 launch failed (hip error " + std::to_string(e) + ")");
+                    }
+                    else if (packed) launch_gq_2bit(h->st, pv.g2, h->ld2, plan, h->ldg, Qd, qsc, rr, bb, s32, Th, cp, ap, scale_out, h->nd, L);
                     else if (narrow_shape(h)) {
                         const int e = launch_gq_n(h->st, pv.g8, h->ld8, plan, h->N, Qd, qsc, rr, bb, s32, Th, cp, ap, scale_out, L);
                         if (e != 0) return fail(h, GPCA_ERR_HIP, "k_gq_n launch failed (hip error " + std::to_string(e) + ")");
@@ -267,8 +293,10 @@
                     else launch_gq_i8(h->st, pv.g8, h->ld8, plan, h->N, Qd, qsc, rr, bb, s32, Th, cp, scale_out, L, h->ko);
                     HIPCHK(hipGetLastError());
                     if (streamed && scale_out && (packed || !h->simple_kernels || narrow_shape(h))) {
-                        launch_absmax_fold(h->st, ap, plan.waves, h->d_amax_run + 32 * hf);
-                        HIPCHK(hipGetLastError());
+                        for (int j = 0; j < per; ++j) {
+                            launch_absmax_fold(h->st, ap + j * ahalf, pair ? pplan.waves / 2 : plan.waves, h->d_amax_run + 32 * (hf + j));
+                            HIPCHK(hipGetLastError());
+                        }
                     }
                 }
                 return GPCA_OK;
@@ -279,13 +307,13 @@
         if (scale_out)
             for (int hf = 0; hf < halves; ++hf) {
                 if (h->c_fold_pending)
-                    launch_post_k1(h->st, h->d_cpart + hf * chalf, h->Mpad / 32, h->d_scratch64 + (size_t)hf * kPostK1Scratch, h->d_apart + hf * ahalf, h->gqplan.waves,
+                    launch_post_k1(h->st, h->d_cpart + hf * chalf, h->Mpad / 32, h->d_scratch64 + (size_t)hf * kPostK1Scratch, h->d_apart + hf * ahalf, aparts,
                                    h->d_tscale + 32 * hf, h->d_tinv + 32 * hf, h->nd);
                 else launch_sum_partials_f32(h->st, h->d_cpart + hf * chalf, h->Mpad / 32, 32, h->d_c + 32 * hf, h->d_scratch64);
                 HIPCHK(hipGetLastError());
             }
         for (int hf = 0; hf < kMaxSketch / 32; ++hf) h->apart_src[hf] = streamed ? h->d_amax_run + 32 * hf : h->d_apart + hf * ahalf;
-        h->apart_parts = streamed ? 1 : h->gqplan.waves;
+        h->apart_parts = streamed ? 1 : aparts;
         return GPCA_OK;
     }
     {
@@ -428,8 +456,14 @@
         CHK(ensure(h, h->dTd, h->cap_Td, (size_t)h->Mpad * 32 * kDigits * (size_t)(L / 32)));
         int64_t yslices = h->plan8.W;
         if (h->sm.on && h->M % h->sm.panel_rows) yslices = std::max<int64_t>(yslices, k2_plan(h, round_up(h->M % h->sm.panel_rows, kGQRowsPerWave)).W);
-        CHK(ensure(h, h->dYpart64, h->cap_Ypart64, (size_t)yslices * (size_t)Npad * 32));
-        CHK(ensure(h, h->d_apart, h->cap_apart, (size_t)h->gqplan.waves * 32 * (size_t)(L / 32)));
+        int64_t yslices_paired = 0;
+        if (paired_halves(h)) {
+            h->plan8p = k2_plan_paired(h, gemm_rows);
+            yslices_paired = h->plan8p.W;
+            if (h->sm.on && h->M % h->sm.panel_rows) yslices_paired = std::max<int64_t>(yslices_paired, k2_plan_paired(h, round_up(h->M % h->sm.panel_rows, kGQRowsPerWave)).W);
+        }
+        CHK(ensure(h, h->dYpart64, h->cap_Ypart64, (size_t)ypart64_capacity(yslices, yslices_paired, Npad)));
+        CHK(ensure(h, h->d_apart, h->cap_apart, (size_t)apart_capacity(h->gqplan.waves, L)));
         if (h->sm.on) CHK(ensure(h, h->d_yint, h->cap_yint, (size_t)N * 32 * (size_t)(L / 32)));
         if (!h->d_qscale) {
             HIPCHK(hipMalloc((void**)&h->d_qscale, kMaxSketch * 8)); HIPCHK(hipMalloc((void**)&h->d_qinv, kMaxSketch * 8));
@@ -578,7 +612,7 @@
     c->is_child = true; c->compact_ok = 0;
     c->device = h->device; c->precision = h->precision; c->storage = h->storage; c->nd = h->nd; c->ko = h->ko;
     c->st = h->st;
-    c->simple_kernels = h->simple_kernels; c->narrow_ok = h->narrow_ok; c->spin_sync = h->spin_sync;
+    c->simple_kernels = h->simple_kernels; c->narrow_ok = h->narrow_ok; c->spin_sync = h->spin_sync; c->pair_halves = h->pair_halves;
     c->gq_waves_target = h->gq_waves_target; c->gtt_waves_target = h->gtt_waves_target;
     c->timing_on = h->timing_on;
     c->M = n; c->N = h->N; c->Mpad = npad; c->ldg = h->ldg; c->ld8 = h->ld8; c->ld2 = h->ld2; c->cap_rows_pad = npad; c->pack_flags = h->pack_flags;
diff --git a/genomic_pca_amd/csrc/kernels.h b/genomic_pca_amd/csrc/kernels.h
--- a/genomic_pca_amd/csrc/kernels.h
+++ b/genomic_pca_amd/csrc/kernels.h
@@ -12,6 +12,7 @@
     int gq_phase = -1;
     int gq_chain = 1;
     int gtt_xcd = 1;
+    int gq_nt = 1;
 };
 int init_device_kernels_i8();
 int init_device_kernels_common();
@@ -178,6 +179,11 @@
 int launch_gq_d(hipStream_t st, const int8_t* G, int64_t ldg, const GqPlan& plan, int64_t Npad, const int8_t* Qd,
                 const double* qscale, const float* r, const float* b, const float* s, float* Tout, float* cpart, double* apart,
                 int scale_out, int64_t ldt = 32, const KernelOpts& ko = KernelOpts());
+int launch_gq_d2(hipStream_t st, const int8_t* G, int64_t ldg, const GqPlan& plan, int64_t Npad, const int8_t* Qd, int64_t qd_half,
+                 const double* qscale, const float* r, const float* b, const float* s, float* Tout, float* cpart, int64_t cpart_half,
+                 double* apart, int64_t apart_half, int scale_out, int64_t ldt, const KernelOpts& ko = KernelOpts());
+int launch_gtt_d2(hipStream_t st, const int8_t* G, int64_t ldg, int64_t Mpad, int64_t Npad, const int8_t* Td, int64_t td_half, double* Ypart,
+                  int64_t yp_half, const Gtt8Plan& plan, const KernelOpts& ko = KernelOpts());
 void launch_gtt_2bit(hipStream_t st, const uint8_t* G2, int64_t ld2, int64_t Mpad, int64_t Npad, const int8_t* Td,
                      double* Ypart, const Gtt8Plan& plan, int nd = 4);
 
diff --git a/genomic_pca_amd/csrc/plan_math.h b/genomic_pca_amd/csrc/plan_math.h
--- a/genomic_pca_amd/csrc/plan_math.h
+++ b/genomic_pca_amd/csrc/plan_math.h
@@ -65,6 +65,20 @@
     p.waves = w;
     return p;
 }
+#ifdef __HIPCC__
+#define GPCA_PLAN_HD __host__ __device__
+#else
+#define GPCA_PLAN_HD
+#endif
+struct PairId { unsigned wg, half; };
+GPCA_PLAN_HD inline PairId pair_id(unsigned b, unsigned grid) {
+    const unsigned full = grid & ~15u;
+    PairId p;
+    if (b < full) { p.half = (b >> 3) & 1u; p.wg = (b & 7u) | ((b >> 4) << 3); }
+    else { const unsigned r2 = (grid - full) >> 1, j = b - full; p.half = j >= r2 ? 1u : 0u; p.wg = (full >> 1) + (p.half ? j - r2 : j); }
+    return p;
+}
+inline GqPlan gq_plan_paired(GqPlan plan) { plan.waves = (plan.waves + 7) / 8 * 8; return plan; }
 struct GttPlan { int64_t nblocks_n; int W; int64_t rows_per_wave; int64_t grid; };
 inline GttPlan gtt_plan(int64_t Mpad, int64_t Npad, int L, int target_waves) {
     GttPlan p;
@@ -101,12 +115,11 @@
     p.grid = ((p.nblocks_n + 3) / 4) * W;
     return p;
 }
-inline Gtt8Plan gtt8_plan_batched(int64_t Mpad, int64_t Npad, int target_waves) {
+inline Gtt8Plan gtt8_plan_for_grid(int64_t Mpad, int64_t Npad, int64_t grid0) {
     Gtt8Plan p{};
     p.nblocks_n = Npad / 128;
     p.ngroups = (p.nblocks_n + 3) / 4;
     p.S = Mpad / 128;
-    int64_t grid0 = target_waves / 8;
     if (grid0 < 1) grid0 = 1;
     const int64_t wmin = std::max<int64_t>(1, (p.S + 32767) / 32768), wmax = std::min<int64_t>(p.S, 1024);
     double best = 1e300;
@@ -128,6 +141,12 @@
     p.rows_per_wave = p.C * 128;
     return p;
 }
+inline Gtt8Plan gtt8_plan_batched(int64_t Mpad, int64_t Npad, int target_waves) {
+    return gtt8_plan_for_grid(Mpad, Npad, target_waves / 8);
+}
+inline Gtt8Plan gtt8_plan_paired(int64_t Mpad, int64_t Npad, int target_waves) {
+    return gtt8_plan_for_grid(Mpad, Npad, target_waves / 16);
+}
 constexpr int64_t kNarrowSamples = 256;
 inline Gtt8Plan gtt8_plan_narrow(int64_t Mpad, int64_t N, int target_waves) {
     Gtt8Plan p{};
@@ -172,6 +191,12 @@
 inline int64_t cpart_capacity(int64_t gq_waves, int64_t Mpad, int L) {
     return std::max({gq_waves * (int64_t)L, omega_num_parts(Mpad) * (int64_t)L, Mpad * (int64_t)(L / 32)});
 }
+inline int64_t ypart64_half_stride(int64_t slices, int64_t Npad) { return slices * Npad * 32; }
+inline int64_t ypart64_capacity(int64_t slices, int64_t slices_paired, int64_t Npad) {
+    return std::max(ypart64_half_stride(slices, Npad), 2 * ypart64_half_stride(slices_paired, Npad));
+}
+inline int64_t apart_half_stride(int64_t gq_waves) { return gq_waves * 32; }
+inline int64_t apart_capacity(int64_t gq_waves, int L) { return apart_half_stride(gq_waves) * (int64_t)(L / 32); }
 inline int64_t scores_cand_capacity() { return (int64_t)kScoreParts * kMaxSketchCols; }
 inline int64_t project_scratch_capacity(int Lp) { return sum_scratch_need(Lp); }
 inline int64_t project_part_capacity(int64_t Mpad, int Lp) { return std::max<int64_t>(absmax_num_parts(Mpad) * 32, 2 * (int64_t)Lp); }
diff --git a/include/gpca.h b/include/gpca.h
--- a/include/gpca.h
+++ b/include/gpca.h
@@ -55,7 +55,8 @@
 #define GPCA_CFG_NO_COMPACT 2
 #define GPCA_CFG_NO_NARROW 4
 #define GPCA_CFG_NO_SPIN_SYNC 8
-#define GPCA_CFG_ALL 15
+#define GPCA_CFG_NO_PAIRED_HALVES 16
+#define GPCA_CFG_ALL 31
 
 typedef struct gpca_qc_config {
     double min_snp_call_rate;
```
